# jinggqu/NextGen-UIA

Hardware: AMD Instinct MI355X
Metric: images/sec fwd+bwd BiomedCLIP+Mona bs=256 (higher is better)
Workload: dtype bf16

## Files before the change

include/uia_hip.h:

```cpp
#ifndef UIA_HIP_H
#define UIA_HIP_H
#include <stddef.h>
#include <stdint.h>

#ifdef __cplusplus
extern "C" {
#endif

enum { UIA_F32 = 0, UIA_BF16 = 1 };
enum { UIA_ACT_NONE = 0, UIA_ACT_GELU = 1, UIA_ACT_QUICKGELU = 2, UIA_ACT_RELU = 3 };
enum { UIA_MASK_NONE = 0, UIA_MASK_CAUSAL = 1, UIA_MASK_KEYPAD = 2 };
enum { UIA_MONA_BASELINE = 0, UIA_MONA_NOISE_AWARE = 1, UIA_MONA_FREQ_ENHANCED = 2, UIA_MONA_HYBRID = 3 };

const char* uia_last_error(void);
int uia_version(void);

typedef struct uia_gemm_desc {
    const void* A; int64_t lda;
    const void* W; int64_t ldw;
    int32_t M, N, K;
    float alpha;
    const float* bias;
    int32_t act;
    int32_t dact;
    const void* aux_in; int64_t ldaux_in;
    void* aux_out; int64_t ldaux_out;
    const float* resid; int64_t ldr;
    int32_t resid_mod, resid_row_off;
    const void* residT; int64_t ldrT;
    int32_t out_group;
    void* outT; int64_t ldo;
    float* out32; int64_t ldo32;
    int32_t w_kblocked;
    const void* resid_ln_stats;
    const float* resid_ln_w;
    const float* resid_ln_b;
    int64_t* rowsum_out;
    const int64_t* lnfold_sums;
    const float* lnfold_colsum;
    int32_t lnfold_dim; float lnfold_eps;
    int32_t resid_ln_dim; float resid_ln_eps;
    int64_t a_kb_rows;
    int64_t outT_kb_rows;
    int32_t* ln_flag;
    float ln_flag_limit;
    int32_t drop_where;
    float drop_p;
    uint64_t drop_seed;
    void* a_drop_out;
    float* splitk_ws;
    const void* A2;
    int64_t lda2;
    int32_t K2;
    int32_t a2_group_cols;
    int64_t a2_group_stride;
    const int8_t* resid_lo8;
    int64_t ld_resid_lo;
    int64_t residT_kb_rows;
    int8_t* out_lo8;
    int64_t ld_out_lo;
    int64_t resid_lo_kb_rows;
    int64_t out_lo_kb_rows;
} uia_gemm_desc;
int uia_gemm(void* stream, int dtype, const uia_gemm_desc* d, int tile_cfg );

int uia_wgrad(void* stream, int dtype, int M, int I, int J, const void* A, int64_t lda, const void* B, int64_t ldb,
              float alpha, float* dW, float* dbias_A);
int uia_wgrad_ex(void* stream, int dtype, int M, int I, int J, const void* A, int64_t lda, const void* B, int64_t ldb,
                 float alpha, float* dW, int64_t ldw, int i_valid, int j_valid, float* dbias_A);
int uia_wgrad_drop(void* stream, int dtype, int M, int I, int J, const void* A, int64_t lda, const void* B, int64_t ldb,
                   float alpha, float* dW, int64_t ldw, int i_valid, int j_valid, float drop_p, uint64_t seed, int64_t drop_ld, int drop_col0);
typedef struct uia_wgrad_group_desc {
    int32_t n, M, I, J;
    const void* A[4];
    const void* B[4];
    float* dW[4];
    float* dbias_A[4];
    int64_t lda, ldb, ldw;
    int32_t i_valid, j_valid;
    float alpha, drop_p;
    uint64_t drop_seed[4];
    int64_t drop_ld;
    int32_t drop_col0, reserved;
} uia_wgrad_group_desc;
int uia_wgrad_group(void* stream, int dtype, const uia_wgrad_group_desc* d);

typedef struct uia_attn_desc {
    const void *q, *k, *v; int64_t ld_qkv;
    void* out; int64_t ldo;
    float* lse;
    const int32_t* keylen;
    int32_t B, H, L, dh;
    int32_t mask_kind;
    float scale;
    const void* dout; int64_t lddo;
    void *dq, *dk, *dv; int64_t ld_dqkv;
    const int32_t* cu_seqlens;
    int64_t out_kb_rows;
    int64_t dqkv_kb_rows;
} uia_attn_desc;
int uia_attn_fwd(void* stream, int dtype, const uia_attn_desc* d);
int uia_attn_bwd(void* stream, int dtype, const uia_attn_desc* d);
int uia_attn_bwd_cfg(void* stream, int dtype, const uia_attn_desc* d, int cfg);

int uia_attn_fwd_long(void* stream, int dtype, const uia_attn_desc* d);

int uia_attn_bwd_cls(void* stream, int dtype, const uia_attn_desc* d);

int uia_attn_fwd_cls(void* stream, int dtype, const uia_attn_desc* d);
int uia_attn_bwd_cls_rows(void* stream, int dtype, const uia_attn_desc* d);

int uia_layernorm_fwd(void* stream, int dtype, int M, int D, int64_t ldx, const float* x, const float* gamma, const float* beta,
                      float eps, void* yT, float* y32);
int uia_layernorm_fwd_stats(void* stream, int dtype, int M, int D, int64_t ldx, const float* x, const float* gamma, const float* beta,
                            float eps, void* yT, float* y32, float* stats);
#define UIA_POOL_SLICES 32
int uia_ln_mean_rows(void* stream, int B, int L, int row0, int n, int D, int64_t ldx, const float* x, const float* gamma, const float* beta,
                     float eps, float* ws, float* out, int64_t ldo);
int uia_layernorm_bwd(void* stream, int dtype, int M, int D, int64_t ldx, const void* dy, const float* x, const float* gamma,
                      float eps, const float* dres, float* dx32, void* dxT);
int uia_layernorm_bwd3(void* stream, int dtype, int M, int D, int64_t ldx, const void* dy, const float* x, const void* x_hi, const int8_t* x_lo, int64_t x_kb_rows,
                       const float* gamma, float eps, const float* dres, const void* dres_hi, const int8_t* dres_lo, int64_t dres_kb_rows, float* dx32, void* dxT,
                       int8_t* dx_lo);
int uia_layernorm_bwd_periodic(void* stream, int dtype, int M, int D, const void* dy, const float* x, const void* x_hi, const int8_t* x_lo, int64_t x_kb_rows,
                               const float* gamma, float eps, const float* dres_rows, int period, float* dx32, void* dxT, int8_t* dx_lo);

typedef struct uia_mona_spatial_desc {
    int32_t variant, B, h, w, bott;
    const void* t;
    void* d;
    const float *conv1_w, *conv1_b, *conv2_w, *conv2_b, *conv3_w, *conv3_b;
    const float *proj_w, *proj_b;
    const float* freq;
    const float *ne1_w, *ne1_b, *ne3_w, *ne3_b;
    float p_drop; uint64_t seed; const uint8_t* keep_mask;
    const void* dd;
    void* dt;
    float *g_conv1_w, *g_conv1_b, *g_conv2_w, *g_conv2_b, *g_conv3_w, *g_conv3_b, *g_proj_w, *g_proj_b, *g_freq,
          *g_ne1_w, *g_ne1_b, *g_ne3_w, *g_ne3_b;
    float* ws;
} uia_mona_spatial_desc;
size_t uia_mona_spatial_workspace_bytes(int B);
int uia_mona_pre_fwd(void* stream, int dtype, int M, int D, const float* x, const float* norm_w, const float* norm_b,
                     const float* gamma, const float* gammax, float eps, void* u);
int uia_mona_pre_fwd_t(void* stream, int dtype, int M, int D, const float* x, const float* norm_w, const float* norm_b, const float* gamma, const float* gammax,
                       float eps, void* u, const void* w1, int64_t ldw1, const float* b1, void* t, int64_t ldt);
int uia_mona_pre_bwd(void* stream, int dtype, int M, int D, const void* du, const float* x, const float* dy,
                     const float* norm_w, const float* norm_b, const float* gamma, const float* gammax, float eps,
                     float* dx32, void* dxT, float* g_gamma, float* g_gammax, float* g_norm_w, float* g_norm_b, float* ws,
                     int64_t dxT_kb_rows);
int uia_mona_pre_bwd_du(void* stream, int dtype, int M, int D, const void* dt, int64_t ldt, const void* w1t, int64_t ldw1, const float* x, const float* dy,
                        const float* norm_w, const float* norm_b, const float* gamma, const float* gammax, float eps,
                        float* dx32, void* dxT, float* g_gamma, float* g_gammax, float* g_norm_w, float* g_norm_b, float* ws, int64_t dxT_kb_rows);
int uia_mona_pre_bwd_du3(void* stream, int dtype, int M, int D, const void* dt, int64_t ldt, const void* w1t, int64_t ldw1, const float* x, const void* dy_hi, const int8_t* dy_lo,
                         const float* norm_w, const float* norm_b, const float* gamma, const float* gammax, float eps, void* dxT, int8_t* dx_lo, float* g_gamma,
                         float* g_gammax, float* g_norm_w, float* g_norm_b, float* ws, int64_t dxT_kb_rows);
size_t uia_mona_pre_bwd_workspace_bytes(int M, int D);
int uia_mona_spatial_fwd(void* stream, int dtype, const uia_mona_spatial_desc* d);
int uia_mona_spatial_bwd(void* stream, int dtype, const uia_mona_spatial_desc* d);
int uia_mona_cls_bwd(void* stream, int dtype, int B, int ntok, const void* dd, const void* t, int64_t ldt, void* dt, float p_drop, uint64_t seed,
                     const uint8_t* keep_mask);
int uia_mona_cls_fwd(void* stream, int dtype, int B, int ntok, const void* t, int64_t ldt, void* d, float p_drop, uint64_t seed, const uint8_t* keep_mask);

typedef struct uia_mona_fused_desc {
    uia_mona_spatial_desc sp;
    int32_t D; float eps;
    const float* x;
    const float *norm_w, *norm_b, *gamma, *gammax;
    const void* w1; const float* b1;
    const void* w2; const float* b2;
    float* y32;
    void* yT; int64_t yT_kb_rows;
    int64_t* rowsum_out;
    int32_t* ln_flag;
    void* u_out;
    void* t_out;
} uia_mona_fused_desc;
int uia_mona_fused_supported(int dtype, int D, int h, int w, int bott);
int uia_mona_fused_fwd(void* stream, int dtype, const uia_mona_fused_desc* d);

typedef struct uia_lora_rank_desc {
    int32_t M, N, nsrc;
    float alpha;
    const void* Q; int64_t ldq, q_stride;
    const void* W[3]; int64_t ldw;
    void* out; int64_t ldo;
    float drop_p;
    uint64_t seed[3];
} uia_lora_rank_desc;
int uia_lora_rank_update(void* stream, int dtype, const uia_lora_rank_desc* d);

typedef struct uia_ln_lora_desc {
    int32_t M, D, nsrc;
    float eps;
    const float* x; int64_t ldx;
    const float *gamma, *beta;
    void* h;
    const void* A[3]; int64_t lda;
    void* T; int64_t t_stride;
    float drop_p;
    uint64_t seed[3];
} uia_ln_lora_desc;
int uia_ln_lora_down(void* stream, int dtype, const uia_ln_lora_desc* d);

int uia_upsample_bilinear_fwd(void* stream, int B, int C, int h, int w, int H, int W, const float* src, int64_t ld, float* dst);
int uia_upsample_bilinear_bwd(void* stream, int B, int C, int h, int w, int H, int W, const float* ddst, float* dsrc, int64_t ld);
int uia_segment_mean_fwd(void* stream, int B, int n, int C, const float* x, int64_t ld, float* out);
int uia_segment_mean_bwd(void* stream, int B, int n, int C, const float* dout, float* dx, int64_t ld);
size_t uia_dicece_workspace_bytes(int B);
int uia_dicece_fwd_bwd(void* stream, int B, int C, int HW, const float* logits, const float* label, float smooth_nr, float smooth_dr,
                       float* ws, float* loss, float* dlogits);
size_t uia_focal_workspace_bytes(int N, int C);
int uia_focal_fwd_bwd(void* stream, int N, int C, const float* logits, const int64_t* labels, float gamma, float alpha, void* ws, size_t ws_bytes,
                      float* loss, float* dlogits);
size_t uia_binary_cls_stats_workspace_bytes(int N);
int uia_binary_cls_stats(void* stream, int N, const float* p1, const int64_t* labels, const int64_t* perm, void* ws, size_t ws_bytes, double* record);
size_t uia_surface_distances_workspace_bytes(int B, int H, int W);
int uia_surface_distances(void* stream, int B, int H, int W, const float* logits, const float* label, float percentile, void* ws, size_t ws_bytes,
                          double* hd, double* asd);
enum { UIA_SEG_LABEL_U8 = 0, UIA_SEG_LABEL_F32 = 1 };
int uia_seg_viz_form(int S, int label_dtype, const void* logits, const void* images, const void* labels, const void* mask_rgb, const void* overlay_rgb,
                     const void* pred);
int uia_seg_viz(void* stream, int B, int C, int Ci, int S, const float* logits, const float* images, const void* labels, int label_dtype,
                uint8_t* mask_rgb, uint8_t* overlay_rgb, uint8_t* pred);
size_t uia_retrieval_workspace_bytes(int N, int E);
int uia_retrieval_ranks(void* stream, int N, int E, const float* img, const float* txt, int normalize, void* ws, size_t ws_bytes,
                        int32_t* gt_i2t, int32_t* eq_i2t, int32_t* gt_t2i, int32_t* eq_t2i);
size_t uia_retrieval_stats_workspace_bytes(int N);
int uia_retrieval_stats(void* stream, int N, const int32_t* gt, int nk, const int32_t* k_values, void* ws, size_t ws_bytes, double* record);
size_t uia_retrieval_topk_workspace_bytes(int Q, int N, int E, int K);
int uia_retrieval_topk_splits(int Q, int N);
int uia_retrieval_topk(void* stream, int Q, int N, int E, int K, const float* queries, const float* gallery, int normalize, int splits, void* ws,
                       size_t ws_bytes, int32_t* idx, float* score);
int uia_zero_shot_score(void* stream, int N, int T, int E, int C, const int32_t* class_off, const float* img, const float* prompts, float* logits, int64_t ld,
                        int64_t row, float* probs, float* img_n);
size_t uia_binary_roc_curve_workspace_bytes(int N);
int uia_binary_roc_curve(void* stream, int N, const float* p1, const int64_t* labels, const int64_t* perm, void* ws, size_t ws_bytes, int32_t* count,
                         double* fpr, double* tpr, float* thr);

size_t uia_augment_workspace_bytes(int B, int S);
int uia_augment_batch(void* stream, int B, int S, const float* images, const uint8_t* masks, const int32_t* programs, void* ws, size_t ws_bytes,
                      float* out_images, uint8_t* out_masks);

int uia_augment_gather(void* stream, int N, int B, int S, int src_dtype, const void* images, const uint8_t* masks, const int32_t* programs, void* ws,
                       size_t ws_bytes, float* out_images, uint8_t* out_masks);

int uia_cast(void* stream, int dtype, size_t n, const float* src, void* dst, float scale);
int uia_transpose_cast(void* stream, int dtype, int rows, int cols, const float* src, void* dst);

typedef struct uia_pack_desc {
    const float* src;
    void* row;
    void* row_kb;
    void* tr;
    void* tr_kb;
    int32_t rows, cols;
    int32_t rows_pad, cols_pad;
    float scale;
    int32_t reserved_;
} uia_pack_desc;
int uia_pack_weights(void* stream, int dtype, int n, const uia_pack_desc* descs_device, int max_elems);
int uia_im2col(void* stream, int dtype, int B, int C, int H, int W, int P, const float* img, void* out);
int uia_im2col_padded(void* stream, int dtype, int B, int C, int H, int W, int P, const float* img, void* cols, int64_t ldo);
int uia_fill_cls(void* stream, int B, int N, int D, const float* cls, const float* pos0, float* x);
// ... 94 lines not shown
```

nextgen-uia_amd/csrc/capi.cpp:

```cpp
#include "uia_kernels.h"

void uia_set_error(const char* fmt, ...);
#define NEED(ptr, name) do { if (!(ptr)) { uia_set_error("%s: null descriptor", name); return -1; } } while (0)

extern "C" {

int uia_version(void) { return 100; }

int uia_gemm(void* stream, int dtype, const uia_gemm_desc* d, int tile_cfg) {
    NEED(d, "uia_gemm");
    return uia_gemm_launch((hipStream_t)stream, dtype, *d, tile_cfg);
}
int uia_lora_rank_update(void* stream, int dtype, const uia_lora_rank_desc* d) {
    NEED(d, "uia_lora_rank_update");
    return uia_lora_rank_update_launch((hipStream_t)stream, dtype, *d);
}
int uia_ln_lora_down(void* stream, int dtype, const uia_ln_lora_desc* d) {
    NEED(d, "uia_ln_lora_down");
    return uia_ln_lora_down_launch((hipStream_t)stream, dtype, *d);
}
int uia_wgrad(void* stream, int dtype, int M, int I, int J, const void* A, int64_t lda, const void* B, int64_t ldb, float alpha, float* dW, float* dbias_A) {
    return uia_wgrad_launch((hipStream_t)stream, dtype, M, I, J, A, lda, B, ldb, alpha, dW, dbias_A);
}
int uia_wgrad_ex(void* stream, int dtype, int M, int I, int J, const void* A, int64_t lda, const void* B, int64_t ldb, float alpha, float* dW, int64_t ldw,
                 int i_valid, int j_valid, float* dbias_A) {
    if (ldw <= 0) { uia_set_error("uia_wgrad_ex: ldw=%lld must be positive", (long long)ldw); return -1; }
    return uia_wgrad_launch((hipStream_t)stream, dtype, M, I, J, A, lda, B, ldb, alpha, dW, dbias_A, ldw, i_valid, j_valid);
}
int uia_wgrad_group(void* stream, int dtype, const uia_wgrad_group_desc* d) {
    if (!d) { uia_set_error("uia_wgrad_group: null descriptor"); return -1; }
    if (d->n < 1 || d->n > 4) { uia_set_error("uia_wgrad_group: n=%d outside 1..4", d->n); return -1; }
    if (d->ldw <= 0) { uia_set_error("uia_wgrad_group: ldw=%lld must be positive", (long long)d->ldw); return -1; }
    float* dW[4];
    float* db[4];
    for (int g = 0; g < 4; ++g) { dW[g] = d->dW[g]; db[g] = d->dbias_A[g]; }
    if (d->drop_p > 0.f) for (int g = 0; g < d->n; ++g) if (db[g]) { uia_set_error("uia_wgrad_group: dbias with dropout on B is not a form of the kernel"); return -1; }
    return uia_wgrad_group_launch((hipStream_t)stream, dtype, d->n, d->M, d->I, d->J, d->A, (long)d->lda, d->B, (long)d->ldb, d->alpha, dW, db, (long)d->ldw, d->i_valid, d->j_valid,
                                  d->drop_p, d->drop_seed, (long)d->drop_ld, d->drop_col0);
}
int uia_wgrad_drop(void* stream, int dtype, int M, int I, int J, const void* A, int64_t lda, const void* B, int64_t ldb, float alpha, float* dW, int64_t ldw,
                   int i_valid, int j_valid, float drop_p, uint64_t seed, int64_t drop_ld, int drop_col0) {
    if (ldw <= 0) { uia_set_error("uia_wgrad_drop: ldw=%lld must be positive", (long long)ldw); return -1; }
    if (!(drop_p > 0.f)) { uia_set_error("uia_wgrad_drop: drop_p=%f must be in (0, 1); uia_wgrad_ex is the form without dropout", (double)drop_p); return -1; }
    return uia_wgrad_launch((hipStream_t)stream, dtype, M, I, J, A, lda, B, ldb, alpha, dW, nullptr, ldw, i_valid, j_valid, drop_p, seed, drop_ld, drop_col0);
}
int uia_attn_fwd(void* stream, int dtype, const uia_attn_desc* d) {
    NEED(d, "uia_attn_fwd");
    return uia_attn_fwd_launch((hipStream_t)stream, dtype, *d);
}
int uia_attn_fwd_long(void* stream, int dtype, const uia_attn_desc* d) {
    NEED(d, "uia_attn_fwd_long");
    return uia_attn_fwd_long_launch((hipStream_t)stream, dtype, *d);
}
int uia_attn_bwd(void* stream, int dtype, const uia_attn_desc* d) {
    NEED(d, "uia_attn_bwd");
    return uia_attn_bwd_launch((hipStream_t)stream, dtype, *d, 0);
}
int uia_attn_bwd_cfg(void* stream, int dtype, const uia_attn_desc* d, int cfg) {
    NEED(d, "uia_attn_bwd_cfg");
    return uia_attn_bwd_launch((hipStream_t)stream, dtype, *d, cfg);
}
int uia_layernorm_fwd(void* stream, int dtype, int M, int D, int64_t ldx, const float* x, const float* gamma, const float* beta, float eps, void* yT, float* y32) {
    return uia_layernorm_fwd_launch((hipStream_t)stream, dtype, M, D, ldx, x, gamma, beta, eps, yT, y32, nullptr);
}
int uia_layernorm_fwd_stats(void* stream, int dtype, int M, int D, int64_t ldx, const float* x, const float* gamma, const float* beta, float eps, void* yT, float* y32,
                            float* stats) {
    return uia_layernorm_fwd_launch((hipStream_t)stream, dtype, M, D, ldx, x, gamma, beta, eps, yT, y32, stats);
}
int uia_layernorm_bwd(void* stream, int dtype, int M, int D, int64_t ldx, const void* dy, const float* x, const float* gamma, float eps, const float* dres, float* dx32, void* dxT) {
    return uia_layernorm_bwd_launch((hipStream_t)stream, dtype, M, D, ldx, dy, x, gamma, eps, dres, dx32, dxT);
}
int uia_layernorm_bwd3(void* stream, int dtype, int M, int D, int64_t ldx, const void* dy, const float* x, const void* x_hi, const int8_t* x_lo, int64_t x_kb_rows,
                       const float* gamma, float eps, const float* dres, const void* dres_hi, const int8_t* dres_lo, int64_t dres_kb_rows, float* dx32, void* dxT,
                       int8_t* dx_lo) {
    return uia_layernorm_bwd3_launch((hipStream_t)stream, dtype, M, D, ldx, dy, x, x_hi, x_lo, (long)x_kb_rows, gamma, eps, dres, dres_hi, dres_lo, (long)dres_kb_rows, dx32, dxT,
                                     dx_lo);
}
int uia_layernorm_bwd_periodic(void* stream, int dtype, int M, int D, const void* dy, const float* x, const void* x_hi, const int8_t* x_lo, int64_t x_kb_rows,
                               const float* gamma, float eps, const float* dres_rows, int period, float* dx32, void* dxT, int8_t* dx_lo) {
    return uia_layernorm_bwd_periodic_launch((hipStream_t)stream, dtype, M, D, dy, x, x_hi, x_lo, (long)x_kb_rows, gamma, eps, dres_rows, period, dx32, dxT, dx_lo);
}
int uia_attn_bwd_cls(void* stream, int dtype, const uia_attn_desc* d) {
    NEED(d, "uia_attn_bwd_cls");
    return uia_attn_bwd_cls_launch((hipStream_t)stream, dtype, *d);
}
int uia_attn_bwd_cls_rows(void* stream, int dtype, const uia_attn_desc* d) {
    NEED(d, "uia_attn_bwd_cls_rows");
    return uia_attn_bwd_cls_launch((hipStream_t)stream, dtype, *d, true);
}
int uia_attn_fwd_cls(void* stream, int dtype, const uia_attn_desc* d) {
    NEED(d, "uia_attn_fwd_cls");
    return uia_attn_fwd_cls_launch((hipStream_t)stream, dtype, *d);
}
int uia_mona_cls_fwd(void* stream, int dtype, int B, int ntok, const void* t, int64_t ldt, void* d, float p_drop, uint64_t seed, const uint8_t* keep_mask) {
    return uia_mona_cls_fwd_launch((hipStream_t)stream, dtype, B, ntok, t, (long)ldt, d, p_drop, seed, keep_mask);
}
int uia_rows3_to_f32(void* stream, int rows, int D, int64_t stride_rows, const void* hi, int64_t ldhi, int64_t hi_kb_rows, const int8_t* lo, int64_t ldlo, float* dst) {
    return uia_rows3_to_f32_launch((hipStream_t)stream, rows, D, (long)stride_rows, hi, (long)ldhi, (long)hi_kb_rows, lo, (long)ldlo, dst);
}
int uia_mona_cls_bwd(void* stream, int dtype, int B, int ntok, const void* dd, const void* t, int64_t ldt, void* dt, float p_drop, uint64_t seed, const uint8_t* keep_mask) {
    return uia_mona_cls_bwd_launch((hipStream_t)stream, dtype, B, ntok, dd, t, (long)ldt, dt, p_drop, seed, keep_mask);
}
int uia_copy_rows(void* stream, int rows, int64_t row_bytes, const void* src, int64_t src_stride_bytes, void* dst) {
    return uia_copy_rows_launch((hipStream_t)stream, rows, (long)row_bytes, src, (long)src_stride_bytes, dst);
}
int uia_cast(void* stream, int dtype, size_t n, const float* src, void* dst, float scale) { return uia_cast_launch((hipStream_t)stream, dtype, n, src, dst, scale); }
int uia_transpose_cast(void* stream, int dtype, int rows, int cols, const float* src, void* dst) { return uia_transpose_cast_launch((hipStream_t)stream, dtype, rows, cols, src, dst); }
int uia_pack_weights(void* stream, int dtype, int n, const uia_pack_desc* descs_device, int max_elems) { return uia_pack_weights_launch((hipStream_t)stream, dtype, n, descs_device, max_elems); }
int uia_im2col(void* stream, int dtype, int B, int C, int H, int W, int P, const float* img, void* out) { return uia_im2col_launch((hipStream_t)stream, dtype, B, C, H, W, P, img, out); }
int uia_fill_cls(void* stream, int B, int N, int D, const float* cls, const float* pos0, float* x) { return uia_fill_cls_launch((hipStream_t)stream, B, N, D, cls, pos0, x); }
int uia_embed(void* stream, int rows, int L, int D, int vocab, int max_pos, const int64_t* ids, const float* table, const float* pos, const float* type0, float* out) {
    return uia_embed_launch((hipStream_t)stream, rows, L, D, vocab, max_pos, ids, table, pos, type0, out);
}
int uia_gather_rows(void* stream, int n, int D, const float* src, const int64_t* idx, float* dst) { return uia_gather_rows_launch((hipStream_t)stream, n, D, src, idx, dst); }

int uia_mona_pre_fwd(void* stream, int dtype, int M, int D, const float* x, const float* norm_w, const float* norm_b, const float* gamma,
                     const float* gammax, float eps, void* u) {
    return uia_mona_pre_fwd_launch((hipStream_t)stream, dtype, M, D, x, norm_w, norm_b, gamma, gammax, eps, u);
}
int uia_mona_pre_bwd(void* stream, int dtype, int M, int D, const void* du, const float* x, const float* dy, const float* norm_w,
                     const float* norm_b, const float* gamma, const float* gammax, float eps, float* dx32, void* dxT, float* g_gamma,
                     float* g_gammax, float* g_norm_w, float* g_norm_b, float* ws, int64_t dxT_kb_rows) {
    return uia_mona_pre_bwd_launch((hipStream_t)stream, dtype, M, D, du, x, dy, norm_w, norm_b, gamma, gammax, eps, dx32, dxT, g_gamma, g_gammax,
                                   g_norm_w, g_norm_b, ws, (long)dxT_kb_rows);
}
int uia_mona_pre_fwd_t(void* stream, int dtype, int M, int D, const float* x, const float* norm_w, const float* norm_b, const float* gamma, const float* gammax,
                       float eps, void* u, const void* w1, int64_t ldw1, const float* b1, void* t, int64_t ldt) {
    return uia_mona_pre_fwd_t_launch((hipStream_t)stream, dtype, M, D, x, norm_w, norm_b, gamma, gammax, eps, u, w1, (long)ldw1, b1, t, (long)ldt);
}
int uia_mona_pre_bwd_du(void* stream, int dtype, int M, int D, const void* dt, int64_t ldt, const void* w1t, int64_t ldw1, const float* x, const float* dy,
                        const float* norm_w, const float* norm_b, const float* gamma, const float* gammax, float eps, float* dx32, void* dxT, float* g_gamma,
                        float* g_gammax, float* g_norm_w, float* g_norm_b, float* ws, int64_t dxT_kb_rows) {
    if (!dt || !w1t) { uia_set_error("uia_mona_pre_bwd_du: null dt / w1t"); return -1; }
    return uia_mona_pre_bwd_launch((hipStream_t)stream, dtype, M, D, nullptr, x, dy, norm_w, norm_b, gamma, gammax, eps, dx32, dxT, g_gamma, g_gammax,
                                   g_norm_w, g_norm_b, ws, (long)dxT_kb_rows, dt, (long)ldt, w1t, (long)ldw1);
}
int uia_mona_pre_bwd_du3(void* stream, int dtype, int M, int D, const void* dt, int64_t ldt, const void* w1t, int64_t ldw1, const float* x, const void* dy_hi, const int8_t* dy_lo,
                         const float* norm_w, const float* norm_b, const float* gamma, const float* gammax, float eps, void* dxT, int8_t* dx_lo, float* g_gamma,
                         float* g_gammax, float* g_norm_w, float* g_norm_b, float* ws, int64_t dxT_kb_rows) {
    if (!dt || !w1t || !dy_hi || !dy_lo || !dx_lo) { uia_set_error("uia_mona_pre_bwd_du3: null dt / w1t / dy_hi / dy_lo / dx_lo"); return -1; }
    return uia_mona_pre_bwd_launch((hipStream_t)stream, dtype, M, D, nullptr, x, nullptr, norm_w, norm_b, gamma, gammax, eps, nullptr, dxT, g_gamma, g_gammax,
                                   g_norm_w, g_norm_b, ws, (long)dxT_kb_rows, dt, (long)ldt, w1t, (long)ldw1, dy_hi, dy_lo, dx_lo);
}
size_t uia_mona_pre_bwd_workspace_bytes(int M, int D) { return uia_mona_pre_bwd_ws_floats(M, D) * sizeof(float); }
int uia_mona_spatial_fwd(void* stream, int dtype, const uia_mona_spatial_desc* d) {
    NEED(d, "uia_mona_spatial_fwd");
    return uia_mona_spatial_fwd_launch((hipStream_t)stream, dtype, *d);
}
int uia_mona_spatial_bwd(void* stream, int dtype, const uia_mona_spatial_desc* d) {
    NEED(d, "uia_mona_spatial_bwd");
    return uia_mona_spatial_bwd_launch((hipStream_t)stream, dtype, *d);
}
int uia_mona_fused_fwd(void* stream, int dtype, const uia_mona_fused_desc* d) {
    NEED(d, "uia_mona_fused_fwd");
    return uia_mona_fused_fwd_launch((hipStream_t)stream, dtype, *d);
}

size_t uia_infonce_workspace_bytes(int B, int E) { return uia_infonce_workspace_floats(B, E) * sizeof(float); }
int uia_infonce_fwd_bwd(void* stream, int B, int E, const float* img, const float* txt, float inv_temp, float grad_scale, float* loss,
                        float* dimg, float* dtxt, void* workspace, size_t workspace_bytes) {
    return uia_infonce_launch((hipStream_t)stream, B, E, img, txt, inv_temp, grad_scale, loss, dimg, dtxt, (float*)workspace, workspace_bytes / sizeof(float));
}
int uia_adamw_clip_step(void* stream, size_t n, float* p, const float* g, float* m, float* v, float lr, float beta1, float beta2, float eps,
                        float weight_decay, float max_norm, int step, float grad_scale, float* ws2) {
    return uia_adamw_clip_launch((hipStream_t)stream, n, p, g, m, v, lr, beta1, beta2, eps, weight_decay, max_norm, step, grad_scale, ws2);
}
int uia_grad_accum_guarded(void* stream, size_t n, float* acc, float* mb, const float* loss, float* stats, int32_t* ctl, uint8_t* ok_log, int64_t log_index) {
    return uia_grad_accum_guarded_launch((hipStream_t)stream, n, acc, mb, loss, stats, (int*)ctl, ok_log, (long)log_index);
}
int uia_adamw_clip_step_guarded(void* stream, size_t n, float* p, float* acc, float* m, float* v, float lr, float lr_min, int t_max, float beta1, float beta2,
                                float eps, float weight_decay, float max_norm, float grad_scale, float skip_scale, float* ws8, int32_t* ctl) {
    return uia_adamw_clip_guarded_launch((hipStream_t)stream, n, p, acc, m, v, lr, lr_min, t_max, beta1, beta2, eps, weight_decay, max_norm, grad_scale, skip_scale, ws8, (int*)ctl);
}

int uia_dropout(void* stream, int dtype, size_t n, const void* src, void* dst, float p, uint64_t seed, int accumulate) {
    return uia_dropout_launch((hipStream_t)stream, dtype, n, src, dst, p, seed, accumulate);
}
int uia_colsum(void* stream, int dtype, int M, int N, const void* A, int64_t lda, float* out) {
    return uia_colsum_launch((hipStream_t)stream, dtype, M, N, A, lda, out);
}

int uia_layernorm_bwd_affine(void* stream, int dtype, int M, int D, const void* dy, const float* x, const float* gamma, float eps, const float* dres,
                             float* dx32, float* g_gamma, float* g_beta) {
    return uia_layernorm_bwd_affine_launch((hipStream_t)stream, dtype, M, D, dy, x, gamma, eps, dres, dx32, g_gamma, g_beta);
}
int uia_film_fwd(void* stream, int B, int N, int C, const float* x, const float* mul, const float* add, float* y) { return uia_film_fwd_launch((hipStream_t)stream, B, N, C, x, mul, add, y); }
int uia_film_bwd(void* stream, int B, int N, int C, const float* dy, const float* x, const float* mul, float* dx, float* dmul, float* dadd) {
    return uia_film_bwd_launch((hipStream_t)stream, B, N, C, dy, x, mul, dx, dmul, dadd);
}
int uia_im2col3x3(void* stream, int dtype, int B, int h, int w, int C, int ntok, int tok_off, const float* x, void* cols) {
    return uia_im2col3x3_launch((hipStream_t)stream, dtype, B, h, w, C, ntok, tok_off, x, cols);
}
int uia_col2im3x3(void* stream, int dtype, int B, int h, int w, int C, int ntok, int tok_off, const void* dcols, float* dx) {
    return uia_col2im3x3_launch((hipStream_t)stream, dtype, B, h, w, C, ntok, tok_off, dcols, dx);
}
int uia_unshuffle(void* stream, int dtype, int B, int h, int w, int k1, int k2, const void* tmp, int64_t ld, float bias, float* out) {
    return uia_unshuffle_launch((hipStream_t)stream, dtype, B, h, w, k1, k2, tmp, ld, bias, out);
}
int uia_shuffle(void* stream, int dtype, int B, int h, int w, int k1, int k2, const float* dout, void* dtmp, int64_t ld) {
    return uia_shuffle_launch((hipStream_t)stream, dtype, B, h, w, k1, k2, dout, dtmp, ld);
}
int uia_act_bwd(void* stream, int dtype, size_t n, const void* dy, const void* y, int act, void* out) { return uia_act_bwd_launch((hipStream_t)stream, dtype, n, dy, y, act, out); }

size_t uia_mona_spatial_workspace_bytes(int B) { return uia_mona_spatial_ws_floats(B) * sizeof(float); }

int uia_upsample_bilinear_fwd(void* stream, int B, int C, int h, int w, int H, int W, const float* src, int64_t ld, float* dst) {
    return uia_upsample_bilinear_launch((hipStream_t)stream, false, B, C, h, w, H, W, src, dst, (long)ld);
}
int uia_upsample_bilinear_bwd(void* stream, int B, int C, int h, int w, int H, int W, const float* ddst, float* dsrc, int64_t ld) {
    return uia_upsample_bilinear_launch((hipStream_t)stream, true, B, C, h, w, H, W, ddst, dsrc, (long)ld);
}
int uia_segment_mean_fwd(void* stream, int B, int n, int C, const float* x, int64_t ld, float* out) {
    return uia_segment_mean_launch((hipStream_t)stream, false, B, n, C, x, out, (long)ld);
}
int uia_segment_mean_bwd(void* stream, int B, int n, int C, const float* dout, float* dx, int64_t ld) {
    return uia_segment_mean_launch((hipStream_t)stream, true, B, n, C, dout, dx, (long)ld);
}

size_t uia_dicece_workspace_bytes(int B) { return uia_dicece_ws_floats(B) * sizeof(float); }
int uia_dicece_fwd_bwd(void* stream, int B, int C, int HW, const float* logits, const float* label, float smooth_nr, float smooth_dr,
                       float* ws, float* loss, float* dlogits) {
    return uia_dicece_launch((hipStream_t)stream, B, C, HW, logits, label, smooth_nr, smooth_dr, ws, loss, dlogits);
}

size_t uia_focal_workspace_bytes(int N, int C) { return uia_focal_ws_bytes(N, C); }
int uia_focal_fwd_bwd(void* stream, int N, int C, const float* logits, const int64_t* labels, float gamma, float alpha, void* ws, size_t ws_bytes,
                      float* loss, float* dlogits) {
    return uia_focal_launch((hipStream_t)stream, N, C, logits, labels, gamma, alpha, ws, ws_bytes, loss, dlogits);
}
size_t uia_binary_cls_stats_workspace_bytes(int N) { return uia_binary_cls_stats_ws_bytes(N); }
int uia_binary_cls_stats(void* stream, int N, const float* p1, const int64_t* labels, const int64_t* perm, void* ws, size_t ws_bytes, double* record) {
    return uia_binary_cls_stats_launch((hipStream_t)stream, N, p1, labels, perm, ws, ws_bytes, record);
}

size_t uia_surface_distances_workspace_bytes(int B, int H, int W) { return uia_surface_ws_bytes(B, H, W); }
int uia_surface_distances(void* stream, int B, int H, int W, const float* logits, const float* label, float percentile, void* ws, size_t ws_bytes,
                          double* hd, double* asd) {
    return uia_surface_launch((hipStream_t)stream, B, H, W, logits, label, percentile, ws, ws_bytes, hd, asd);
}

int uia_seg_viz(void* stream, int B, int C, int Ci, int S, const float* logits, const float* images, const void* labels, int label_dtype,
                uint8_t* mask_rgb, uint8_t* overlay_rgb, uint8_t* pred) {
    return uia_seg_viz_launch((hipStream_t)stream, B, C, Ci, S, logits, images, labels, label_dtype, mask_rgb, overlay_rgb, pred);
}

size_t uia_retrieval_workspace_bytes(int N, int E) { return uia_retrieval_ranks_ws_bytes(N, E); }
// ... 138 lines not shown
```

nextgen-uia_amd/csrc/uia_kernels.h:

```cpp
#pragma once
#include <hip/hip_runtime.h>
#include <stddef.h>
#include <stdint.h>

#include "../../include/uia_hip.h"

typedef uia_gemm_desc UiaGemmParams;
typedef uia_attn_desc UiaAttnParams;

int uia_gemm_launch(hipStream_t stream, int dtype, const UiaGemmParams& p, int cfg);
int uia_attn_fwd_launch(hipStream_t stream, int dtype, const UiaAttnParams& p);
int uia_attn_fwd_long_launch(hipStream_t stream, int dtype, const UiaAttnParams& p);
int uia_attn_bwd_launch(hipStream_t stream, int dtype, const UiaAttnParams& p, int cfg = 0);
int uia_layernorm_fwd_launch(hipStream_t stream, int dtype, int M, int D, long ldx, const float* x, const float* gamma, const float* beta,
                             float eps, void* yT, float* y32, float* stats);
int uia_layernorm_bwd_launch(hipStream_t stream, int dtype, int M, int D, long ldx, const void* dy, const float* x, const float* gamma, float eps,
                             const float* dres, float* dx32, void* dxT);
int uia_layernorm_bwd3_launch(hipStream_t stream, int dtype, int M, int D, long ldx, const void* dy, const float* x, const void* x_hi, const int8_t* x_lo,
                              long x_kb_rows, const float* gamma, float eps, const float* dres, const void* dres_hi, const int8_t* dres_lo, long dres_kb_rows,
                              float* dx32, void* dxT, int8_t* dx_lo);
int uia_layernorm_bwd_periodic_launch(hipStream_t stream, int dtype, int M, int D, const void* dy, const float* x, const void* x_hi, const int8_t* x_lo, long x_kb_rows,
                                      const float* gamma, float eps, const float* dres_rows, int period, float* dx32, void* dxT, int8_t* dx_lo);
int uia_attn_bwd_cls_launch(hipStream_t stream, int dtype, const UiaAttnParams& p, bool compact = false);
int uia_attn_fwd_cls_launch(hipStream_t stream, int dtype, const UiaAttnParams& p);
int uia_mona_cls_fwd_launch(hipStream_t stream, int dtype, int B, int ntok, const void* t, long ldt, void* d, float p_drop, uint64_t seed, const uint8_t* keep_mask);
int uia_rows3_to_f32_launch(hipStream_t stream, int rows, int D, long stride_rows, const void* hi, long ldhi, long hi_kb_rows, const int8_t* lo, long ldlo, float* dst);
int uia_mona_cls_bwd_launch(hipStream_t stream, int dtype, int B, int ntok, const void* dd, const void* t, long ldt, void* dt, float p_drop, uint64_t seed,
                            const uint8_t* keep_mask);
int uia_copy_rows_launch(hipStream_t stream, int rows, long row_bytes, const void* src, long src_stride_bytes, void* dst);
int uia_lora_rank_update_launch(hipStream_t stream, int dtype, const uia_lora_rank_desc& p);
int uia_ln_lora_down_launch(hipStream_t stream, int dtype, const uia_ln_lora_desc& p);
int uia_cast_launch(hipStream_t stream, int dtype, size_t n, const float* src, void* dst, float scale);
int uia_transpose_cast_launch(hipStream_t stream, int dtype, int rows, int cols, const float* src, void* dst);
int uia_pack_weights_launch(hipStream_t stream, int dtype, int n, const uia_pack_desc* descs_device, int max_elems);
int uia_im2col_launch(hipStream_t stream, int dtype, int B, int C, int H, int W, int P, const float* img, void* out);
int uia_fill_cls_launch(hipStream_t stream, int B, int N, int D, const float* cls, const float* pos0, float* x);
int uia_embed_launch(hipStream_t stream, int rows, int L, int D, int vocab, int max_pos, const int64_t* ids, const float* table, const float* pos, const float* type0, float* out);
int uia_gather_rows_launch(hipStream_t stream, int n, int D, const float* src, const int64_t* idx, float* dst);
int uia_wgrad_group_launch(hipStream_t stream, int dtype, int n, int M, int I, int J, const void* const* A, long lda, const void* const* B, long ldb, float alpha,
                            float* const* dW, float* const* dbias, long ldw, int i_valid, int j_valid, float drop_p, const uint64_t* drop_seed, long drop_ld, int drop_col0);
int uia_wgrad_launch(hipStream_t stream, int dtype, int M, int I, int J, const void* A, long lda, const void* B, long ldb, float alpha, float* dW, float* dbias,
                     long ldw = 0, int i_valid = 0, int j_valid = 0, float drop_p = 0.f, uint64_t drop_seed = 0, long drop_ld = 0, int drop_col0 = 0);
int uia_mona_pre_fwd_launch(hipStream_t stream, int dtype, int M, int D, const float* x, const float* nw, const float* nb, const float* gamma,
                            const float* gammax, float eps, void* u);
int uia_mona_pre_fwd_t_launch(hipStream_t stream, int dtype, int M, int D, const float* x, const float* nw, const float* nb, const float* gamma,
                              const float* gammax, float eps, void* u, const void* w1, long ldw1, const float* b1, void* t, long ldt);
int uia_mona_pre_bwd_launch(hipStream_t stream, int dtype, int M, int D, const void* du, const float* x, const float* dy, const float* nw,
                            const float* nb, const float* gamma, const float* gammax, float eps, float* dx32, void* dxT, float* g_gamma,
                            float* g_gammax, float* g_nw, float* g_nb, float* ws, long dxT_kb_rows, const void* dt = nullptr, long ldt = 0,
                            const void* w1t = nullptr, long ldw1 = 0, const void* dy_hi = nullptr, const int8_t* dy_lo = nullptr, int8_t* dx_lo = nullptr);
size_t uia_mona_pre_bwd_ws_floats(int M, int D);
int uia_mona_spatial_fwd_launch(hipStream_t stream, int dtype, const uia_mona_spatial_desc& p);
int uia_mona_spatial_bwd_launch(hipStream_t stream, int dtype, const uia_mona_spatial_desc& p);
int uia_mona_fused_fwd_launch(hipStream_t stream, int dtype, const uia_mona_fused_desc& q);
size_t uia_infonce_workspace_floats(int B, int E);
int uia_infonce_launch(hipStream_t stream, int B, int E, const float* img, const float* txt, float inv_temp, float grad_scale, float* loss,
                       float* dimg, float* dtxt, float* ws, size_t ws_floats);
int uia_adamw_clip_launch(hipStream_t stream, size_t n, float* p, const float* g, float* m, float* v, float lr, float beta1, float beta2,
                          float eps, float weight_decay, float max_norm, int step, float grad_scale, float* ws);
int uia_grad_accum_guarded_launch(hipStream_t stream, size_t n, float* acc, float* mb, const float* loss, float* stats, int* ctl, unsigned char* ok_log, long log_index);
int uia_adamw_clip_guarded_launch(hipStream_t stream, size_t n, float* p, float* acc, float* m, float* v, float lr, float lr_min, int t_max, float beta1,
                                  float beta2, float eps, float weight_decay, float max_norm, float grad_scale, float skip_scale, float* ws8, int* ctl);
int uia_dropout_launch(hipStream_t stream, int dtype, size_t n, const void* src, void* dst, float p, uint64_t seed, int accumulate);
int uia_colsum_launch(hipStream_t stream, int dtype, int M, int N, const void* A, long lda, float* out);
int uia_attn_small_launch(hipStream_t stream, int dtype, const UiaAttnParams& p, bool bwd);
bool uia_attn_dh16_ok(int dtype, const UiaAttnParams& p);
int uia_attn_dh16_launch(hipStream_t stream, const UiaAttnParams& p, bool bwd);
int uia_layernorm_bwd_affine_launch(hipStream_t stream, int dtype, int M, int D, const void* dy, const float* x, const float* gamma, float eps,
                                    const float* dres, float* dx32, float* g_gamma, float* g_beta);
int uia_film_fwd_launch(hipStream_t stream, int B, int N, int C, const float* x, const float* mul, const float* add, float* y);
int uia_film_bwd_launch(hipStream_t stream, int B, int N, int C, const float* dy, const float* x, const float* mul, float* dx, float* dmul, float* dadd);
int uia_im2col3x3_launch(hipStream_t stream, int dtype, int B, int h, int w, int C, int ntok, int tok_off, const float* x, void* cols);
int uia_col2im3x3_launch(hipStream_t stream, int dtype, int B, int h, int w, int C, int ntok, int tok_off, const void* dcols, float* dx);
int uia_unshuffle_launch(hipStream_t stream, int dtype, int B, int h, int w, int k1, int k2, const void* tmp, long ld, float bias, float* out);
int uia_shuffle_launch(hipStream_t stream, int dtype, int B, int h, int w, int k1, int k2, const float* dout, void* dtmp, long ld);
int uia_act_bwd_launch(hipStream_t stream, int dtype, size_t n, const void* dy, const void* y, int act, void* out);
size_t uia_mona_spatial_ws_floats(int B);
int uia_upsample_bilinear_launch(hipStream_t stream, bool bwd, int B, int C, int h, int w, int H, int W, const float* in, float* out, long ld);
int uia_segment_mean_launch(hipStream_t stream, bool bwd, int B, int n, int C, const float* in, float* out, long ld);
size_t uia_dicece_ws_floats(int B);
int uia_dicece_launch(hipStream_t stream, int B, int C, int HW, const float* logits, const float* label, float nr, float dr, float* ws, float* loss, float* dlogits);
size_t uia_focal_ws_bytes(int N, int C);
int uia_focal_launch(hipStream_t stream, int N, int C, const float* logits, const int64_t* labels, float gamma, float alpha, void* ws, size_t ws_bytes,
                     float* loss, float* dlogits);
size_t uia_binary_cls_stats_ws_bytes(int N);
int uia_binary_cls_stats_launch(hipStream_t stream, int N, const float* p1, const int64_t* labels, const int64_t* perm, void* ws, size_t ws_bytes,
                                double* record);
size_t uia_surface_ws_bytes(int B, int H, int W);
int uia_surface_launch(hipStream_t stream, int B, int H, int W, const float* logits, const float* label, float percentile, void* ws, size_t ws_bytes,
                       double* hd, double* asd);
int uia_seg_viz_launch(hipStream_t stream, int B, int C, int Ci, int S, const float* logits, const float* images, const void* labels, int label_dtype,
                       uint8_t* mask_rgb, uint8_t* overlay_rgb, uint8_t* pred);
size_t uia_retrieval_ranks_ws_bytes(int N, int E);
int uia_retrieval_ranks_launch(hipStream_t stream, int N, int E, const float* img, const float* txt, int normalize, void* ws, size_t ws_bytes,
                               int32_t* gt_i2t, int32_t* eq_i2t, int32_t* gt_t2i, int32_t* eq_t2i);
size_t uia_retrieval_stats_ws_bytes(int N);
int uia_retrieval_stats_launch(hipStream_t stream, int N, const int32_t* gt, int nk, const int32_t* k_values, void* ws, size_t ws_bytes, double* record);
size_t uia_retrieval_topk_ws_bytes(int Q, int N, int E, int K);
int uia_retrieval_topk_rule(int Q, int N);
int uia_retrieval_topk_launch(hipStream_t stream, int Q, int N, int E, int K, const float* queries, const float* gallery, int normalize, int splits, void* ws,
                              size_t ws_bytes, int32_t* idx, float* score);
int uia_zero_shot_score_launch(hipStream_t stream, int N, int T, int E, int C, const int32_t* class_off, const float* img, const float* prompts, float* logits,
                               long ld, long row, float* probs, float* img_n);
size_t uia_binary_roc_curve_ws_bytes(int N);
int uia_binary_roc_curve_launch(hipStream_t stream, int N, const float* p1, const int64_t* labels, const int64_t* perm, void* ws, size_t ws_bytes,
                                int32_t* count, double* fpr, double* tpr, float* thr);
size_t uia_augment_ws_bytes(int B, int S);
int uia_augment_batch_launch(hipStream_t stream, int B, int S, const float* images, const uint8_t* masks, const int32_t* programs, void* ws, size_t ws_bytes,
                             float* out_images, uint8_t* out_masks);
int uia_augment_gather_launch(hipStream_t stream, int N, int B, int S, int src_dtype, const void* images, const uint8_t* masks, const int32_t* programs,
                              void* ws, size_t ws_bytes, float* out_images, uint8_t* out_masks);
int uia_im2col_padded_launch(hipStream_t stream, int dtype, int B, int C, int H, int W, int P, const float* img, void* out, long ldo);
int uia_embed_bwd_launch(hipStream_t stream, int rows, int D, int vocab, const int64_t* ids, const float* dx, float* dtable, long pad_id);
int uia_embed_packed_launch(hipStream_t stream, int rows, int D, int vocab, int max_pos, const int64_t* ids, const int64_t* pos_idx, const float* table, const float* pos, const float* type0, float* out);
int uia_ln_mean_rows_launch(hipStream_t stream, int B, int L, int row0, int n, int D, long ldx, const float* x, const float* gamma, const float* beta,
                            float eps, float* ws, float* out, long ldo);
int uia_conv_igemm_launch(hipStream_t stream, int dtype, int mode, int B, int H, int W, int C1, int C2, const void* x1, const void* x2, int N, int N1,
                          const void* w, const float* bias, void* y1, void* y2);
int uia_conv_wgrad_splits(int mode, int B, int H, int W, int C1, int C2, int N);
int uia_conv_wgrad_launch(hipStream_t stream, int dtype, int mode, int B, int H, int W, int C1, int C2, const void* x1, const void* x2, int N,
                          const void* dy, float* ws, float* dw);
int uia_bn_fwd_launch(hipStream_t stream, int dtype, int training, long M, int C, const void* y, const float* gamma, const float* beta,
                      float* run_mean, float* run_var, int64_t* nbt, float momentum, float eps, float* ws, float* mean, float* invstd,
                      float* scale, float* shift, int relu, void* out);
int uia_bn_relu_bwd_launch(hipStream_t stream, int dtype, long M, int C, const void* y, const void* dout, const float* scale, const float* shift,
                           const float* mean, const float* invstd, const float* gamma, float* ws, float* dgamma, float* dbeta, void* dy);
int uia_colsum_ordered_launch(hipStream_t stream, int dtype, long M, int C, const void* y, float* ws, float* out);
int uia_conv_igemm_form(int mode, int C1, int C2, int N, int N1);
int uia_conv_wgrad_form(int mode, int C1, int C2, int N);
int uia_bn_act_fwd_launch(hipStream_t stream, int dtype, int training, long M, int C, const void* y, const float* gamma, const float* beta,
                          float* run_mean, float* run_var, int64_t* nbt, float momentum, float eps, float* ws, float* mean, float* invstd,
                          float* scale, float* shift, float slope, void* out, float drop_p, uint64_t seed, const uint8_t* keep_mask);
int uia_bn_act_bwd_launch(hipStream_t stream, int dtype, long M, int C, const void* y, const void* dout, const float* scale, const float* shift,
                          const float* mean, const float* invstd, const float* gamma, float* ws, float* dgamma, float* dbeta, void* dy,
                          float slope, float drop_p, uint64_t seed, const uint8_t* keep_mask);
int uia_maxpool2_launch(hipStream_t stream, int dtype, int backward, int B, int H, int W, int C, const void* x, const void* dy, void* out);
int uia_conv_strided_launch(hipStream_t stream, int dtype, int dgrad, int B, int H, int W, int C, int k, int s, const void* x, int N, const void* w,
                            void* y);
int uia_conv_strided_wgrad_splits(int B, int H, int W, int C, int k, int s, int N);
int uia_conv_strided_form(int dgrad, int C, int N, int k, int s);
int uia_conv_strided_wgrad_form(int C, int N, int k, int s);
int uia_conv_strided_wgrad_launch(hipStream_t stream, int dtype, int B, int H, int W, int C, int k, int s, const void* x, int N, const void* dy,
                                  float* ws, float* dw);
int uia_maxpool3s2_launch(hipStream_t stream, int dtype, int backward, int B, int H, int W, int C, const void* x, const void* dy, void* out);
int uia_avgpool_launch(hipStream_t stream, int dtype, int backward, int B, int H, int W, int C, const void* x, float* pooled, void* dx);
int uia_nchw_to_nhwc_launch(hipStream_t stream, int dtype, int B, int Cin, int H, int W, int Cout, int rep, const float* x, void* out);
int uia_add2_launch(hipStream_t stream, int dtype, long n, const void* a, const void* b, void* out);
int uia_bn_add_relu_fwd_launch(hipStream_t stream, int dtype, int training, long M, int C, const void* y, const void* r, const float* gamma,
                               const float* beta, float* run_mean, float* run_var, int64_t* nbt, float momentum, float eps, float* ws, float* mean,
                               float* invstd, float* scale, float* shift, void* out);
int uia_bn_add_relu_bwd_launch(hipStream_t stream, int dtype, long M, int C, const void* y, const void* out, const void* dout, const float* mean,
                               const float* invstd, const float* gamma, float* ws, float* dgamma, float* dbeta, void* dy, void* dr);
int uia_upsample_ac_launch(hipStream_t stream, int dtype, int backward, int B, int H, int W, int C, int f, const void* in, void* out);
int uia_resize_aa_launch(hipStream_t stream, int dtype, int backward, int B, int C, int Hi, int Wi, int Ho, int Wo, const void* x, float* tmp, float* out,
                         const float* dout, void* dx);
```

nextgen-uia_amd/uia_hip/_lib.py:

```python
import ctypes as C
import os
import re

import torch

_HERE = os.path.dirname(os.path.abspath(__file__))
LIB_PATH = os.environ.get("UIA_HIP_LIB") or os.path.join(_HERE, "libuia_hip.so")

F32, BF16 = 0, 1
ACT_NONE, ACT_GELU, ACT_QUICKGELU, ACT_RELU = 0, 1, 2, 3
MASK_NONE, MASK_CAUSAL, MASK_KEYPAD = 0, 1, 2
MONA_VARIANTS = {"baseline": 0, "noise_aware": 1, "freq_enhanced": 2, "hybrid": 3}

vp, i32, i64, f32, sz = C.c_void_p, C.c_int32, C.c_int64, C.c_float, C.c_size_t


class PackDesc(C.Structure):
    _fields_ = [("src", vp), ("row", vp), ("row_kb", vp), ("tr", vp), ("tr_kb", vp), ("rows", i32), ("cols", i32),
                ("rows_pad", i32), ("cols_pad", i32), ("scale", f32), ("reserved_", i32)]


class GemmDesc(C.Structure):
    _fields_ = [("A", vp), ("lda", i64), ("W", vp), ("ldw", i64), ("M", i32), ("N", i32), ("K", i32), ("alpha", f32),
                ("bias", vp), ("act", i32), ("dact", i32), ("aux_in", vp), ("ldaux_in", i64), ("aux_out", vp), ("ldaux_out", i64),
                ("resid", vp), ("ldr", i64), ("resid_mod", i32), ("resid_row_off", i32), ("residT", vp), ("ldrT", i64),
                ("out_group", i32), ("outT", vp), ("ldo", i64), ("out32", vp), ("ldo32", i64), ("w_kblocked", i32),
                ("resid_ln_stats", vp), ("resid_ln_w", vp), ("resid_ln_b", vp),
                ("rowsum_out", vp), ("lnfold_sums", vp), ("lnfold_colsum", vp), ("lnfold_dim", i32), ("lnfold_eps", f32),
                ("resid_ln_dim", i32), ("resid_ln_eps", f32), ("a_kb_rows", i64), ("outT_kb_rows", i64), ("ln_flag", vp), ("ln_flag_limit", f32),
                ("drop_where", i32), ("drop_p", f32), ("drop_seed", C.c_uint64), ("a_drop_out", vp), ("splitk_ws", vp),
                ("A2", vp), ("lda2", i64), ("K2", i32), ("a2_group_cols", i32), ("a2_group_stride", i64),
                ("resid_lo8", vp), ("ld_resid_lo", i64), ("residT_kb_rows", i64), ("out_lo8", vp), ("ld_out_lo", i64),
                ("resid_lo_kb_rows", i64), ("out_lo_kb_rows", i64)]


class AttnDesc(C.Structure):
    _fields_ = [("q", vp), ("k", vp), ("v", vp), ("ld_qkv", i64), ("out", vp), ("ldo", i64), ("lse", vp), ("keylen", vp),
                ("B", i32), ("H", i32), ("L", i32), ("dh", i32), ("mask_kind", i32), ("scale", f32),
                ("dout", vp), ("lddo", i64), ("dq", vp), ("dk", vp), ("dv", vp), ("ld_dqkv", i64), ("cu_seqlens", vp),
                ("out_kb_rows", i64), ("dqkv_kb_rows", i64)]


class MonaSpatialDesc(C.Structure):
    _fields_ = [("variant", i32), ("B", i32), ("h", i32), ("w", i32), ("bott", i32),
                ("t", vp), ("d", vp),
                ("conv1_w", vp), ("conv1_b", vp), ("conv2_w", vp), ("conv2_b", vp), ("conv3_w", vp), ("conv3_b", vp),
                ("proj_w", vp), ("proj_b", vp), ("freq", vp), ("ne1_w", vp), ("ne1_b", vp), ("ne3_w", vp), ("ne3_b", vp),
                ("p_drop", f32), ("seed", C.c_uint64), ("keep_mask", vp),
                ("dd", vp), ("dt", vp),
                ("g_conv1_w", vp), ("g_conv1_b", vp), ("g_conv2_w", vp), ("g_conv2_b", vp), ("g_conv3_w", vp), ("g_conv3_b", vp),
                ("g_proj_w", vp), ("g_proj_b", vp), ("g_freq", vp), ("g_ne1_w", vp), ("g_ne1_b", vp), ("g_ne3_w", vp), ("g_ne3_b", vp), ("ws", vp)]


class WgradGroupDesc(C.Structure):
    _fields_ = [("n", C.c_int32), ("M", C.c_int32), ("I", C.c_int32), ("J", C.c_int32), ("A", C.c_void_p * 4), ("B", C.c_void_p * 4), ("dW", C.c_void_p * 4),
                ("dbias_A", C.c_void_p * 4), ("lda", C.c_int64), ("ldb", C.c_int64), ("ldw", C.c_int64), ("i_valid", C.c_int32), ("j_valid", C.c_int32),
                ("alpha", C.c_float), ("drop_p", C.c_float), ("drop_seed", C.c_uint64 * 4), ("drop_ld", C.c_int64), ("drop_col0", C.c_int32), ("reserved", C.c_int32)]


class LoraRankDesc(C.Structure):
    _fields_ = [("M", i32), ("N", i32), ("nsrc", i32), ("alpha", f32), ("Q", vp), ("ldq", i64), ("q_stride", i64), ("W", vp * 3), ("ldw", i64),
                ("out", vp), ("ldo", i64), ("drop_p", f32), ("seed", C.c_uint64 * 3)]


class LnLoraDesc(C.Structure):
    _fields_ = [("M", i32), ("D", i32), ("nsrc", i32), ("eps", f32), ("x", vp), ("ldx", i64), ("gamma", vp), ("beta", vp), ("h", vp), ("A", vp * 3), ("lda", i64),
                ("T", vp), ("t_stride", i64), ("drop_p", f32), ("seed", C.c_uint64 * 3)]


class MonaFusedDesc(C.Structure):
    _fields_ = [("sp", MonaSpatialDesc), ("D", i32), ("eps", f32), ("x", vp), ("norm_w", vp), ("norm_b", vp), ("gamma", vp), ("gammax", vp),
                ("w1", vp), ("b1", vp), ("w2", vp), ("b2", vp), ("y32", vp), ("yT", vp), ("yT_kb_rows", i64), ("rowsum_out", vp), ("ln_flag", vp),
                ("u_out", vp), ("t_out", vp)]


PROTOTYPES = {
    "uia_last_error": (C.c_char_p, []),
    "uia_version": (C.c_int, []),
    "uia_gemm": (C.c_int, [vp, C.c_int, C.POINTER(GemmDesc), C.c_int]),
    "uia_wgrad": (C.c_int, [vp, C.c_int, C.c_int, C.c_int, C.c_int, vp, i64, vp, i64, f32, vp, vp]),
    "uia_wgrad_drop": (C.c_int, [vp, C.c_int, C.c_int, C.c_int, C.c_int, vp, i64, vp, i64, f32, vp, i64, C.c_int, C.c_int, f32, C.c_uint64, i64, C.c_int]),
    "uia_wgrad_group": (C.c_int, [vp, C.c_int, vp]),
    "uia_wgrad_ex": (C.c_int, [vp, C.c_int, C.c_int, C.c_int, C.c_int, vp, i64, vp, i64, f32, vp, i64, C.c_int, C.c_int, vp]),
    "uia_attn_fwd": (C.c_int, [vp, C.c_int, C.POINTER(AttnDesc)]),
    "uia_attn_fwd_long": (C.c_int, [vp, C.c_int, C.POINTER(AttnDesc)]),
    "uia_attn_bwd": (C.c_int, [vp, C.c_int, C.POINTER(AttnDesc)]),
    "uia_attn_bwd_cfg": (C.c_int, [vp, C.c_int, C.POINTER(AttnDesc), C.c_int]),
    "uia_layernorm_fwd": (C.c_int, [vp, C.c_int, C.c_int, C.c_int, i64, vp, vp, vp, f32, vp, vp]),
    "uia_layernorm_fwd_stats": (C.c_int, [vp, C.c_int, C.c_int, C.c_int, i64, vp, vp, vp, f32, vp, vp, vp]),
    "uia_ln_mean_rows": (C.c_int, [vp, C.c_int, C.c_int, C.c_int, C.c_int, C.c_int, i64, vp, vp, vp, f32, vp, vp, i64]),
    "uia_conv_igemm": (C.c_int, [vp, C.c_int, C.c_int, C.c_int, C.c_int, C.c_int, C.c_int, C.c_int, vp, vp, C.c_int, C.c_int, vp, vp, vp, vp]),
    "uia_conv_wgrad_splits": (C.c_int, [C.c_int, C.c_int, C.c_int, C.c_int, C.c_int, C.c_int, C.c_int]),
    "uia_conv_wgrad": (C.c_int, [vp, C.c_int, C.c_int, C.c_int, C.c_int, C.c_int, C.c_int, C.c_int, vp, vp, C.c_int, vp, vp, vp]),
    "uia_conv_igemm_form": (C.c_int, [C.c_int, C.c_int, C.c_int, C.c_int, C.c_int]),
    "uia_conv_wgrad_form": (C.c_int, [C.c_int, C.c_int, C.c_int, C.c_int]),
    "uia_bn_act_fwd": (C.c_int, [vp, C.c_int, C.c_int, i64, C.c_int, vp, vp, vp, vp, vp, vp, f32, f32, vp, vp, vp, vp, vp, f32, vp, f32, C.c_uint64, vp]),
    "uia_bn_act_bwd": (C.c_int, [vp, C.c_int, i64, C.c_int, vp, vp, vp, vp, vp, vp, vp, vp, vp, vp, vp, f32, f32, C.c_uint64, vp]),
    "uia_maxpool2_fwd": (C.c_int, [vp, C.c_int, C.c_int, C.c_int, C.c_int, C.c_int, vp, vp]),
    "uia_maxpool2_bwd": (C.c_int, [vp, C.c_int, C.c_int, C.c_int, C.c_int, C.c_int, vp, vp, vp]),
    "uia_conv_strided": (C.c_int, [vp, C.c_int, C.c_int, C.c_int, C.c_int, C.c_int, C.c_int, C.c_int, C.c_int, vp, C.c_int, vp, vp]),
    "uia_conv_strided_wgrad_splits": (C.c_int, [C.c_int, C.c_int, C.c_int, C.c_int, C.c_int, C.c_int, C.c_int]),
    "uia_conv_strided_form": (C.c_int, [C.c_int, C.c_int, C.c_int, C.c_int, C.c_int]),
    "uia_conv_strided_wgrad_form": (C.c_int, [C.c_int, C.c_int, C.c_int, C.c_int]),
    "uia_conv_strided_wgrad": (C.c_int, [vp, C.c_int, C.c_int, C.c_int, C.c_int, C.c_int, C.c_int, C.c_int, vp, C.c_int, vp, vp, vp]),
    "uia_maxpool3s2_fwd": (C.c_int, [vp, C.c_int, C.c_int, C.c_int, C.c_int, C.c_int, vp, vp]),
    "uia_maxpool3s2_bwd": (C.c_int, [vp, C.c_int, C.c_int, C.c_int, C.c_int, C.c_int, vp, vp, vp]),
    "uia_bn_add_relu_fwd": (C.c_int, [vp, C.c_int, C.c_int, i64, C.c_int, vp, vp, vp, vp, vp, vp, vp, f32, f32, vp, vp, vp, vp, vp, vp]),
    "uia_bn_add_relu_bwd": (C.c_int, [vp, C.c_int, i64, C.c_int, vp, vp, vp, vp, vp, vp, vp, vp, vp, vp, vp]),
    "uia_avgpool_fwd": (C.c_int, [vp, C.c_int, C.c_int, C.c_int, C.c_int, C.c_int, vp, vp]),
    "uia_avgpool_bwd": (C.c_int, [vp, C.c_int, C.c_int, C.c_int, C.c_int, C.c_int, vp, vp]),
    "uia_nchw_to_nhwc": (C.c_int, [vp, C.c_int, C.c_int, C.c_int, C.c_int, C.c_int, C.c_int, C.c_int, vp, vp]),
    "uia_add2": (C.c_int, [vp, C.c_int, i64, vp, vp, vp]),
    "uia_bn_fwd": (C.c_int, [vp, C.c_int, C.c_int, i64, C.c_int, vp, vp, vp, vp, vp, vp, f32, f32, vp, vp, vp, vp, vp, C.c_int, vp]),
    "uia_bn_relu_bwd": (C.c_int, [vp, C.c_int, i64, C.c_int, vp, vp, vp, vp, vp, vp, vp, vp, vp, vp, vp]),
    "uia_colsum_ordered": (C.c_int, [vp, C.c_int, i64, C.c_int, vp, vp, vp]),
    "uia_upsample_ac": (C.c_int, [vp, C.c_int, C.c_int, C.c_int, C.c_int, C.c_int, C.c_int, C.c_int, vp, vp]),
    "uia_resize_aa": (C.c_int, [vp, C.c_int, C.c_int, C.c_int, C.c_int, C.c_int, C.c_int, C.c_int, C.c_int, vp, vp, vp, vp, vp]),
    "uia_layernorm_bwd": (C.c_int, [vp, C.c_int, C.c_int, C.c_int, i64, vp, vp, vp, f32, vp, vp, vp]),
    "uia_ln_lora_down": (C.c_int, [vp, C.c_int, C.POINTER(LnLoraDesc)]),
    "uia_lora_rank_update": (C.c_int, [vp, C.c_int, C.POINTER(LoraRankDesc)]),
    "uia_layernorm_bwd3": (C.c_int, [vp, C.c_int, C.c_int, C.c_int, i64, vp, vp, vp, vp, i64, vp, f32, vp, vp, vp, i64, vp, vp, vp]),
    "uia_mona_pre_fwd": (C.c_int, [vp, C.c_int, C.c_int, C.c_int, vp, vp, vp, vp, vp, f32, vp]),
    "uia_mona_pre_bwd": (C.c_int, [vp, C.c_int, C.c_int, C.c_int, vp, vp, vp, vp, vp, vp, vp, f32, vp, vp, vp, vp, vp, vp, vp, i64]),
    "uia_mona_pre_fwd_t": (C.c_int, [vp, C.c_int, C.c_int, C.c_int, vp, vp, vp, vp, vp, f32, vp, vp, i64, vp, vp, i64]),
    "uia_mona_pre_bwd_du": (C.c_int, [vp, C.c_int, C.c_int, C.c_int, vp, i64, vp, i64, vp, vp, vp, vp, vp, vp, f32, vp, vp, vp, vp, vp, vp, vp, i64]),
    "uia_mona_pre_bwd_du3": (C.c_int, [vp, C.c_int, C.c_int, C.c_int, vp, i64, vp, i64, vp, vp, vp, vp, vp, vp, vp, f32, vp, vp, vp, vp, vp, vp, vp, i64]),
    "uia_mona_pre_bwd_workspace_bytes": (sz, [C.c_int, C.c_int]),
    "uia_mona_spatial_fwd": (C.c_int, [vp, C.c_int, C.POINTER(MonaSpatialDesc)]),
    "uia_mona_spatial_bwd": (C.c_int, [vp, C.c_int, C.POINTER(MonaSpatialDesc)]),
    "uia_mona_spatial_workspace_bytes": (sz, [C.c_int]),
    "uia_mona_fused_supported": (C.c_int, [C.c_int, C.c_int, C.c_int, C.c_int, C.c_int]),
    "uia_mona_fused_fwd": (C.c_int, [vp, C.c_int, C.POINTER(MonaFusedDesc)]),
    "uia_upsample_bilinear_fwd": (C.c_int, [vp, C.c_int, C.c_int, C.c_int, C.c_int, C.c_int, C.c_int, vp, C.c_int64, vp]),
    "uia_upsample_bilinear_bwd": (C.c_int, [vp, C.c_int, C.c_int, C.c_int, C.c_int, C.c_int, C.c_int, vp, vp, C.c_int64]),
    "uia_segment_mean_fwd": (C.c_int, [vp, C.c_int, C.c_int, C.c_int, vp, C.c_int64, vp]),
    "uia_segment_mean_bwd": (C.c_int, [vp, C.c_int, C.c_int, C.c_int, vp, vp, C.c_int64]),
    "uia_dicece_workspace_bytes": (sz, [C.c_int]),
    "uia_dicece_fwd_bwd": (C.c_int, [vp, C.c_int, C.c_int, C.c_int, vp, vp, C.c_float, C.c_float, vp, vp, vp]),
    "uia_focal_workspace_bytes": (sz, [C.c_int, C.c_int]),
    "uia_focal_fwd_bwd": (C.c_int, [vp, C.c_int, C.c_int, vp, vp, f32, f32, vp, sz, vp, vp]),
    "uia_binary_cls_stats_workspace_bytes": (sz, [C.c_int]),
    "uia_binary_cls_stats": (C.c_int, [vp, C.c_int, vp, vp, vp, vp, sz, vp]),
    "uia_surface_distances_workspace_bytes": (sz, [C.c_int, C.c_int, C.c_int]),
    "uia_surface_distances": (C.c_int, [vp, C.c_int, C.c_int, C.c_int, vp, vp, f32, vp, sz, vp, vp]),
    "uia_seg_viz_form": (C.c_int, [C.c_int, C.c_int, vp, vp, vp, vp, vp, vp]),
    "uia_seg_viz": (C.c_int, [vp, C.c_int, C.c_int, C.c_int, C.c_int, vp, vp, vp, C.c_int, vp, vp, vp]),
    "uia_retrieval_workspace_bytes": (sz, [C.c_int, C.c_int]),
    "uia_retrieval_ranks": (C.c_int, [vp, C.c_int, C.c_int, vp, vp, C.c_int, vp, sz, vp, vp, vp, vp]),
    "uia_retrieval_stats_workspace_bytes": (sz, [C.c_int]),
    "uia_retrieval_stats": (C.c_int, [vp, C.c_int, vp, C.c_int, vp, vp, sz, vp]),
    "uia_retrieval_topk_workspace_bytes": (sz, [C.c_int, C.c_int, C.c_int, C.c_int]),
    "uia_retrieval_topk_splits": (C.c_int, [C.c_int, C.c_int]),
    "uia_retrieval_topk": (C.c_int, [vp, C.c_int, C.c_int, C.c_int, C.c_int, vp, vp, C.c_int, C.c_int, vp, sz, vp, vp]),
    "uia_zero_shot_score": (C.c_int, [vp, C.c_int, C.c_int, C.c_int, C.c_int, vp, vp, vp, vp, C.c_int64, C.c_int64, vp, vp]),
    "uia_binary_roc_curve_workspace_bytes": (sz, [C.c_int]),
    "uia_binary_roc_curve": (C.c_int, [vp, C.c_int, vp, vp, vp, vp, sz, vp, vp, vp, vp]),
    "uia_augment_workspace_bytes": (sz, [C.c_int, C.c_int]),
    "uia_augment_batch": (C.c_int, [vp, C.c_int, C.c_int, vp, vp, vp, vp, sz, vp, vp]),
    "uia_augment_gather": (C.c_int, [vp, C.c_int, C.c_int, C.c_int, C.c_int, vp, vp, vp, vp, sz, vp, vp]),
    "uia_infonce_workspace_bytes": (sz, [C.c_int, C.c_int]),
    "uia_infonce_fwd_bwd": (C.c_int, [vp, C.c_int, C.c_int, vp, vp, f32, f32, vp, vp, vp, vp, sz]),
    "uia_adamw_clip_step": (C.c_int, [vp, sz, vp, vp, vp, vp, f32, f32, f32, f32, f32, f32, C.c_int, f32, vp]),
    "uia_grad_accum_guarded": (C.c_int, [vp, sz, vp, vp, vp, vp, vp, vp, i64]),
    "uia_adamw_clip_step_guarded": (C.c_int, [vp, sz, vp, vp, vp, vp, f32, f32, C.c_int, f32, f32, f32, f32, f32, f32, f32, vp, vp]),
    "uia_comm_unique_id_bytes": (C.c_int, []),
    "uia_comm_get_unique_id": (C.c_int, [vp, C.c_int]),
    "uia_comm_init": (C.c_int, [C.c_int, C.c_int, vp, C.c_int]),
    "uia_comm_world": (C.c_int, []),
    "uia_comm_initialised": (C.c_int, []),
    "uia_allreduce_sum": (C.c_int, [vp, C.c_int, vp, sz]),
    "uia_allgather": (C.c_int, [vp, C.c_int, vp, vp, sz]),
    "uia_comm_destroy": (C.c_int, []),
    "uia_dropout": (C.c_int, [vp, C.c_int, sz, vp, vp, f32, C.c_uint64, C.c_int]),
    "uia_colsum": (C.c_int, [vp, C.c_int, C.c_int, C.c_int, vp, i64, vp]),
    "uia_layernorm_bwd_affine": (C.c_int, [vp, C.c_int, C.c_int, C.c_int, vp, vp, vp, f32, vp, vp, vp, vp]),
    "uia_film_fwd": (C.c_int, [vp, C.c_int, C.c_int, C.c_int, vp, vp, vp, vp]),
    "uia_film_bwd": (C.c_int, [vp, C.c_int, C.c_int, C.c_int, vp, vp, vp, vp, vp, vp]),
    "uia_im2col3x3": (C.c_int, [vp, C.c_int, C.c_int, C.c_int, C.c_int, C.c_int, C.c_int, C.c_int, vp, vp]),
    "uia_col2im3x3": (C.c_int, [vp, C.c_int, C.c_int, C.c_int, C.c_int, C.c_int, C.c_int, C.c_int, vp, vp]),
    "uia_unshuffle": (C.c_int, [vp, C.c_int, C.c_int, C.c_int, C.c_int, C.c_int, C.c_int, vp, i64, f32, vp]),
    "uia_shuffle": (C.c_int, [vp, C.c_int, C.c_int, C.c_int, C.c_int, C.c_int, C.c_int, vp, vp, i64]),
    "uia_act_bwd": (C.c_int, [vp, C.c_int, sz, vp, vp, C.c_int, vp]),
    "uia_cast": (C.c_int, [vp, C.c_int, sz, vp, vp, f32]),
    "uia_transpose_cast": (C.c_int, [vp, C.c_int, C.c_int, C.c_int, vp, vp]),
    "uia_pack_weights": (C.c_int, [vp, C.c_int, C.c_int, vp, C.c_int]),
    "uia_im2col": (C.c_int, [vp, C.c_int, C.c_int, C.c_int, C.c_int, C.c_int, C.c_int, vp, vp]),
    "uia_im2col_padded": (C.c_int, [vp, C.c_int, C.c_int, C.c_int, C.c_int, C.c_int, C.c_int, vp, vp, C.c_int64]),
    "uia_fill_cls": (C.c_int, [vp, C.c_int, C.c_int, C.c_int, vp, vp, vp]),
    "uia_embed": (C.c_int, [vp, C.c_int, C.c_int, C.c_int, C.c_int, C.c_int, vp, vp, vp, vp, vp]),
    "uia_embed_bwd": (C.c_int, [vp, C.c_int, C.c_int, C.c_int, vp, vp, vp, C.c_int64]),
    "uia_embed_packed": (C.c_int, [vp, C.c_int, C.c_int, C.c_int, C.c_int, vp, vp, vp, vp, vp, vp]),
    "uia_gather_rows": (C.c_int, [vp, C.c_int, C.c_int, vp, vp, vp]),
    "uia_copy_rows": (C.c_int, [vp, C.c_int, i64, vp, i64, vp]),
    "uia_attn_bwd_cls": (C.c_int, [vp, C.c_int, C.POINTER(AttnDesc)]),
    "uia_mona_cls_bwd": (C.c_int, [vp, C.c_int, C.c_int, C.c_int, vp, vp, i64, vp, f32, C.c_uint64, vp]),
    "uia_attn_fwd_cls": (C.c_int, [vp, C.c_int, C.POINTER(AttnDesc)]),
    "uia_attn_bwd_cls_rows": (C.c_int, [vp, C.c_int, C.POINTER(AttnDesc)]),
    "uia_mona_cls_fwd": (C.c_int, [vp, C.c_int, C.c_int, C.c_int, vp, i64, vp, f32, C.c_uint64, vp]),
    "uia_rows3_to_f32": (C.c_int, [vp, C.c_int, C.c_int, i64, vp, i64, i64, vp, i64, vp]),
    "uia_layernorm_bwd_periodic": (C.c_int, [vp, C.c_int, C.c_int, C.c_int, vp, vp, vp, vp, i64, vp, f32, vp, C.c_int, vp, vp, vp]),
}

_lib = None
_BLOCKING = ("uia_comm_init", "uia_comm_destroy", "uia_comm_get_unique_id")


class UiaError(RuntimeError):
    pass


def lib():
    global _lib
    if _lib is None:
        if not os.path.exists(LIB_PATH):
            raise UiaError(f"{LIB_PATH} not built: run `make -C nextgen-uia_amd/csrc` (hipcc --offload-arch=gfx950). "
                           "There is no CPU fallback for the uia hot path.")
        release = os.environ.get("UIA_CTYPES_RELEASE_GIL", "0") == "1"
        handle = (C.CDLL if release else C.PyDLL)(LIB_PATH)
        blocking = C.CDLL(LIB_PATH)
        _one_copy_of("librccl")
        _one_copy_of("libamdhip64")
        for name, (res, args) in PROTOTYPES.items():
            fn = getattr(blocking if name in _BLOCKING else handle, name)
            fn.restype, fn.argtypes = res, args
            if name in _BLOCKING:
                setattr(handle, name, fn)
        _lib = handle
    return _lib


def _one_copy_of(stem):
    try:
        pat = re.compile(r"^" + re.escape(stem) + r"\.so(\.\d+)*$")
        paths = {line.split()[-1] for line in open("/proc/self/maps") if pat.match(os.path.basename(line.split()[-1]) if line.split() else "")}
    except OSError:
        return
    real = {os.path.realpath(p) for p in paths}
    if len(real) > 1:
        raise UiaError(f"two copies of {stem} are loaded ({sorted(real)}): import torch before uia_hip so that libuia_hip.so binds to PyTorch's runtime")


def check(rc, what=""):
    if rc != 0:
        raise UiaError(f"{what} failed (rc={rc}): {lib().uia_last_error().decode()}")
```

nextgen-uia_amd/uia_hip/functional.py:

```python
import math
import os
import weakref

import time

import torch

from . import handoff, ops
from ._lib import UiaError
from .handoff import (ClsGrad, Resid3, _g3_partner_feeds, cls_grad_of, fwd3_of, grad3_decode, grad3_of, grad_resid3_enabled, hook_free, linear_chain,
                      publish_cls_grad, publish_fwd3, publish_grad3, publish_rows, publish_t_copy, set_cls_grad, set_grad_resid3, t_copy_of, take_rows, zero_sums,
                      cls_only, set_cls_forward, take_cls_forward)
from .handoff import clear as clear_t_copies

_STATE = {"dtype": torch.bfloat16, "seed": 0x5EED, "calls": 0, "fwd_resid3": os.environ.get("UIA_FWD_RESID3", "1") != "0"}


def set_compute_dtype(dt):
    assert dt in (torch.bfloat16, torch.float32)
    _STATE["dtype"] = dt


def compute_dtype():
    return _STATE["dtype"]


def set_deferred_text_ln(flag):
    _STATE["text_ln_deferred"] = bool(flag)


def set_block_resid3(flag):
    _STATE["block_resid3"] = bool(flag)


def set_fwd_resid3(flag):
    _STATE["fwd_resid3"] = bool(flag)


def set_text_resid3(flag):
    _STATE["text_resid3"] = bool(flag)


def set_ln_fold(flag):
    _STATE["ln_fold"] = bool(flag)


def set_deterministic(flag):
    _STATE["deterministic"] = bool(flag)
    ops.TAIL_SPLIT_K = not flag


def ln_fold_enabled(dt, rows=None):
    return dt != torch.float32 and _STATE.get("ln_fold", True) and (rows is None or rows > _STATE.get("ln_fold_min_rows", 2048))


class LnFoldRangeError(FloatingPointError):
    """A GEMM that left row sums for a folded LayerNorm saw a non-finite or out-of-range partial sum: the LayerNorm statistics of that
    row — and everything downstream of it — are wrong."""


_FOLD_POLL = {}
_FOLD_REPORTED = {}


POLL_LAG = max(1, int(os.environ.get("UIA_POLL_LAG", "2")))


def reset_ln_flag(device=None):
    dev = torch.device("cuda", torch.cuda.current_device()) if device is None else torch.device(device)
    key = dev.index if dev.index is not None else torch.cuda.current_device()
    _FOLD_POLL.pop(key, None)
    _FOLD_REPORTED.pop(key, None)
    if key in ops._LN_FLAG:
        ops._LN_FLAG[key].zero_()


def poll_ln_flag(device=None, sync=False):
    dev = torch.device("cuda", torch.cuda.current_device()) if device is None else torch.device(device)
    key = dev.index if dev.index is not None else torch.cuda.current_device()
    flag = ops._LN_FLAG.get(key)
    if flag is None:
        return 0
    seen = 0
    pending = _FOLD_POLL.setdefault(key, [])
    while pending and (sync or len(pending) >= POLL_LAG):
        prev = pending.pop(0)
        t0 = time.perf_counter()
        prev[1].synchronize()
        _STATE["gpu_wait_s"] = _STATE.get("gpu_wait_s", 0.0) + time.perf_counter() - t0
        seen |= int(prev[0][0])
    host = torch.empty(1, dtype=torch.int32, pin_memory=True)
    host.copy_(flag, non_blocking=True)
    ev = torch.cuda.Event()
    ev.record()
    if sync:
        ev.synchronize()
        seen |= int(host[0])
    else:
        pending.append((host, ev))
    seen &= ~_FOLD_REPORTED.get(key, 0) | 2
    _FOLD_REPORTED[key] = _FOLD_REPORTED.get(key, 0) | (seen & 1)
    if seen & 2:
        raise LnFoldRangeError("uia_hip: a LayerNorm row sum was non-finite or out of the fixed-point range (|Σ| or Σ² >= 5e8 in one column "
                               "block): the activations have diverged; the statistics of that row are not valid")
    if seen & 1 and _STATE.get("ln_fold", True):
        import warnings
        warnings.warn(f"uia_hip: LayerNorm fold switched off: a row with |mean| / std > {ops.LN_FLAG_LIMIT} would lose bf16 precision as a raw "
                      "GEMM operand; the LayerNorm kernels are used from the next forward on")
        set_ln_fold(False)
    return seen


def set_fp32_heads(flag):
    _STATE["fp32_heads"] = bool(flag)


def head_dtype():
    return torch.float32 if _STATE.get("fp32_heads", True) else compute_dtype()


def set_unpad_text(flag):
    _STATE["unpad_text"] = bool(flag)


def set_dropout_seed(seed):
    _STATE["seed"], _STATE["calls"] = int(seed), 0


def _next_seed():
    _STATE["calls"] += 1
    return (_STATE["seed"] * 0x9E3779B97F4A7C15 + _STATE["calls"] * 0xD1B54A32D192ED03) & 0xFFFFFFFFFFFFFFFF


class _PackedParam:
    __slots__ = ("ref", "version", "epoch", "dt", "row", "row_kb", "tr", "tr_kb", "fwd", "bwd", "src_ptr", "pads", "extra")

    def __init__(self, p, dt, pads=None):
        R, Cc = p.shape
        RP, CP = pads if pads is not None else (R, Cc)
        g = 64 // torch.empty(0, dtype=dt).element_size()
        mk = (lambda *shape: torch.zeros(shape, device=p.device, dtype=dt)) if pads is not None else (lambda *shape: torch.empty(shape, device=p.device, dtype=dt))
        self.ref, self.version, self.epoch, self.dt, self.src_ptr, self.pads = weakref.ref(p), -1, -1, dt, 0, pads
        self.extra = []
        self.row, self.tr = mk(RP, CP), mk(CP, RP)
        self.row_kb = mk(CP // g, RP, g) if CP % g == 0 else None
        self.tr_kb = mk(RP // g, CP, g) if RP % g == 0 else None
        self.fwd, self.bwd = ops.PackedW(self.row, self.row_kb), ops.PackedW(self.tr, self.tr_kb)

    def entries(self):
        src = self.ref().detach()
        ent = (src, self.row, self.row_kb, self.tr, self.tr_kb)
        out = [ent if self.pads is None else ent + ((self.pads[0], self.pads[1], 1.0),)]
        for view, rp, cp, scale in self.extra:
            out.append((src, None, ops.RawDest(view), None, None, (rp, cp, scale)))
        return out


class WeightCache:
    PACK_MAX_ELEMS = 1 << 20

    def __init__(self):
        self._c = {}
        self.epoch = 0
        self._packed = {}
        self._ext_of = {}
# ... 272 lines not shown
        P = dict(zip(names, params))
        B, N, D = x.shape
        dt, bott = u.dtype, t.shape[1]
        dy = cg.rows32
        dy_t = dy if dt == torch.float32 else (cg.rows_t if cg.rows_t is not None else t_copy_of(dy, dt))
        direct = ctx.direct_params is not None and all(_is_flat_grad(p) for p in ctx.direct_params)
        G = ({k: p.grad for k, p in zip(names, ctx.direct_params)} if direct
             else {k: torch.zeros_like(v, dtype=torch.float32) for k, v in P.items()})
        cls_rows = lambda a: a.view(B, N * a.shape[1])[:, :a.shape[1]]
        side = _wgrad_side_stream(x.device) if _STATE.get("wgrad_side_stream", False) else None
        w2t = WEIGHTS.get(P["project2.weight"], dt, transpose=True)
        dd = _empty((B, bott), dt, x)
        _wgrad_beside(side, lambda: ops.gemm(dy_t, w2t, out_t=dd), dy_t, cls_rows(d), G["project2.weight"], G["project2.bias"])
        dtt = _empty((B, bott), dt, x)
        ops.mona_cls_bwd(B, ntok or N, dd, t, dtt, p_drop=p_drop, seed=seed, keep_mask=keep_mask, t_rows=bool(ntok))
        w1t = WEIGHTS.get(P["project1.weight"], dt, transpose=True)
        fuse_du = x.is_cuda and ops.mona_pre_bwd_du_ok(B, D, bott, dt)
        du = None if fuse_du else _empty((B, D), dt, x)
        _wgrad_beside(side, None if fuse_du else (lambda: ops.gemm(dtt, w1t, out_t=du)), dtt, cls_rows(u), G["project1.weight"], G["project1.bias"])
        need_dx = ctx.needs_input_grad[0]
        x_cls = x.view(B, D) if ntok else ops.copy_rows(x.view(B * N, D), N, _empty((B, D), torch.float32, x))
        dx = _empty((B, D), torch.float32, x) if need_dx else None
        dx_t = _empty((B, D), dt, x) if (need_dx and dt != torch.float32) else None
        w1t_rows = (dtt, w1t.row if isinstance(w1t, ops.PackedW) else w1t) if fuse_du else None
        ops.mona_pre_bwd(du, x_cls, dy if need_dx else None, P["norm.weight"], P["norm.bias"], P["gamma"], P["gammax"], dx, dx_t,
                         G["gamma"], G["gammax"], G["norm.weight"], G["norm.bias"], dt_w1t=w1t_rows)
        if need_dx and ntok:
            dx = dx.view(B, 1, D)
            publish_t_copy(dx, dx_t.view(B, 1, D) if dx_t is not None else None)
        elif need_dx:
            dx = publish_cls_grad(x.shape, x.device, dx, dx_t) if ctx.cls_ok else ClsGrad(dx, dx_t, N).decode()
        grads = tuple(None if direct else (G[k] if ctx.needs_input_grad[7 + i] else None) for i, k in enumerate(names))
        return (dx, None, None, None, None, None, None) + grads

    @staticmethod
    def backward(ctx, dy):
        if getattr(ctx, "rows_ntok", 0):
            dy = dy.contiguous()
            B, _, D = dy.shape
            dt = ctx.saved_tensors[1].dtype
            return MonaFn.backward_cls(ctx, ClsGrad(dy.view(B, D), t_copy_of(dy, dt).view(B, D) if dt != torch.float32 else None, ctx.rows_ntok))
        cg = cls_grad_of(dy)
        if cg is not None:
            return MonaFn.backward_cls(ctx, cg)
        variant, hw, p_drop, seed, names, has_mask = ctx.meta
        x, u, t, d, keep_mask, *params = ctx.saved_tensors
        keep_mask = keep_mask if has_mask else None
        P = dict(zip(names, params))
        B, N, D = x.shape
        h, w = hw
        M, dt = B * N, u.dtype
        bott = t.shape[1]
        g3 = grad3_of(dy)
        fuse_du = x.is_cuda and ops.mona_pre_bwd_du_ok(M, D, bott, dt)
        if g3 is not None and ops.is_kb(g3.hi):
            dy, g3 = g3.decode().view(B, N, D), None
        if g3 is not None:
            dy_t = g3.hi.view(M, D)
        else:
            dy = dy.contiguous()
            dy_t = t_copy_of(dy, dt).view(M, D)
        direct = ctx.direct_params is not None and all(_is_flat_grad(p) for p in ctx.direct_params)
        G = ({k: p.grad for k, p in zip(names, ctx.direct_params)} if direct
             else {k: torch.zeros_like(v, dtype=torch.float32) for k, v in P.items()})
        w2t = WEIGHTS.get(P["project2.weight"], dt, transpose=True)
        dd = _empty((M, bott), dt, x)
        side = _wgrad_side_stream(x.device) if _STATE.get("wgrad_side_stream", False) else None
        _wgrad_beside(side, lambda: ops.gemm(dy_t, w2t, out_t=dd), dy_t, d, G["project2.weight"], G["project2.bias"])
        sp = {_SPATIAL_MAP[k]: v.detach().contiguous() for k, v in P.items() if k in _SPATIAL_MAP}
        sg = {_SPATIAL_MAP[k]: G[k] for k in P if k in _SPATIAL_MAP}
        dtt = _empty((M, bott), dt, x)
        ops.mona_spatial_bwd(variant, B, h, w, t, sp, dd, dtt, sg, p_drop=p_drop, seed=seed, keep_mask=keep_mask)
        w1t = WEIGHTS.get(P["project1.weight"], dt, transpose=True)
        du = None if fuse_du else _empty((M, D), dt, x)
        _wgrad_beside(side, None if fuse_du else (lambda: ops.gemm(dtt, w1t, out_t=du)), dtt, u, G["project1.weight"], G["project1.bias"])
        need_dx = ctx.needs_input_grad[0]
        dx_t = _act(M, D, dt, x, 4 * D) if (need_dx and dt != torch.float32) else None
        w1t_rows = (dtt, w1t.row if isinstance(w1t, ops.PackedW) else w1t) if fuse_du else None
        if need_dx and g3 is not None and fuse_du and getattr(ctx, "g3_out", False):
            dlo = torch.empty(M, D, device=x.device, dtype=torch.int8)
            ops.mona_pre_bwd(None, x, g3, P["norm.weight"], P["norm.bias"], P["gamma"], P["gammax"], None, dx_t,
                             G["gamma"], G["gammax"], G["norm.weight"], G["norm.bias"], dt_w1t=w1t_rows, dx_lo=dlo)
            dx = publish_grad3(x.shape, x.device, dx_t, dlo)
        else:
            if need_dx and g3 is not None:
                dy = g3.decode().view(B, N, D)
            dx = torch.empty_like(x) if need_dx else None
            ops.mona_pre_bwd(du, x, dy if need_dx else None, P["norm.weight"], P["norm.bias"], P["gamma"], P["gammax"], dx, dx_t,
                             G["gamma"], G["gammax"], G["norm.weight"], G["norm.bias"], dt_w1t=w1t_rows)
            if need_dx:
                publish_t_copy(dx, dx_t)
        grads = tuple(None if direct else (G[k] if ctx.needs_input_grad[7 + i] else None) for i, k in enumerate(names))
        return (dx, None, None, None, None, None, None) + grads


def _wgrad_beside(side, dgrad, a, b, dw, db):
    if side is not None:
        side.wait_stream(torch.cuda.current_stream())
        with torch.cuda.stream(side):
            ops.wgrad(a, b, dw, db)
        a.record_stream(side)
        b.record_stream(side)
    if dgrad is not None:
        dgrad()
    if side is None:
        ops.wgrad(a, b, dw, db)


_WGRAD_SIDE = {}


def _wgrad_side_stream(device):
    key = device.index if device.index is not None else torch.cuda.current_device()
    if key not in _WGRAD_SIDE:
        _WGRAD_SIDE[key] = torch.cuda.Stream(device=device)
    return _WGRAD_SIDE[key]


def set_wgrad_side_stream(flag):
    _STATE["wgrad_side_stream"] = bool(flag)


def join_side_streams():
    cur = torch.cuda.current_stream()
    for st in _WGRAD_SIDE.values():
        cur.wait_stream(st)


DIRECT_TRAIN = True


def _is_flat_grad(p):
    g = p.grad
    return (getattr(p, "_uia_flat_grad", False) and g is not None and g.dtype == torch.float32 and g.is_contiguous() and g.shape == p.shape
            and g.device == p.device)


def mona_apply(x_bnd, module_params, variant, hw, p_drop, training, keep_mask=None):
    names = tuple(k for k in MONA_PARAM_ORDER if k in module_params)
    pd = p_drop if (training or keep_mask is not None) else 0.0
    params = [module_params[k] for k in names]
    direct = torch.is_grad_enabled() and all(p.requires_grad and _is_flat_grad(p) for p in params)
    return MonaFn.apply(x_bnd, variant, tuple(hw), pd, keep_mask, names, direct, *params)


class BlockSpec:

    def __init__(self, heads, eps, act, ln1, qkv, proj, ln2, fc1, fc2, mask=None, publish_out=False):
        self.heads, self.eps, self.act, self.mask = heads, eps, act, mask
        self.publish_out = publish_out
        self.ln1, self.qkv, self.proj, self.ln2, self.fc1, self.fc2 = ln1, qkv, proj, ln2, fc1, fc2


ATTN_SINGLE_PASS_MAX = 272


class VitBlockFn(torch.autograd.Function):

    @staticmethod
    def forward(ctx, x, spec):
        B, N, D = x.shape
        M, dt = B * N, compute_dtype()
        if N > ATTN_SINGLE_PASS_MAX and (ctx.needs_input_grad[0] or spec.mask is not None):
            raise UiaError(f"vit_block: {N} tokens exceed the {ATTN_SINGLE_PASS_MAX} of the attention backward; sequences this long run forward-only "
                           "(frozen tower under torch.no_grad()), unmasked" if ctx.needs_input_grad[0] else
                           f"vit_block: {N} tokens with a mask: the long attention forward takes no mask")
        x3 = fwd3_of(x)
        like = x3.lo if x3 is not None else x
        if x3 is None:
            x = x.contiguous()
            x2d = x.view(M, D)
        train = ctx.needs_input_grad[0]
        fold = ln_fold_enabled(dt, M)
        if x3 is not None:
            assert fold and dt == torch.bfloat16, "a three-byte forward token reached a block that cannot take it"
            rows = (x3.hi, x3.sums)
        else:
            rows = take_rows(x, dt) if fold else None
        qkv = _empty((M, 3 * D), dt, like)
        if rows is not None:
            wq, cq, bq = WEIGHTS.get_lnfold(spec.qkv[0], spec.qkv[1], spec.ln1[0], spec.ln1[1], dt)
            xin_t, sums0 = rows
            if not ops.is_kb(xin_t):
                xin_t = xin_t.view(M, D)
            ops.gemm(xin_t, wq, bias=bq, out_t=qkv, lnfold=(sums0, cq, D, spec.eps))
            h1 = _act(M, D, dt, like, spec.fc1[0].shape[0]) if x3 is not None else xin_t
        else:
            h1 = _empty((M, D), dt, x)
            ops.layernorm_fwd(x2d, spec.ln1[0], spec.ln1[1], spec.eps, y_t=h1)
            ops.gemm(h1, WEIGHTS.get(spec.qkv[0], dt), bias=spec.qkv[1], out_t=qkv)
        if handoff.take_last_block_cls() and spec.mask is None and 1 < N <= ATTN_SINGLE_PASS_MAX and D == 64 * spec.heads and like.is_cuda:
            return VitBlockFn._forward_cls(ctx, x, x3, qkv, spec, (B, N, D), dt, train)
        if N > ATTN_SINGLE_PASS_MAX:
            a = _empty((M, D), dt, like)
            ops.attn_fwd_long(qkv[:, :D], qkv[:, D:2 * D], qkv[:, 2 * D:], a, B, spec.heads, N)
            lse = None
        else:
            a = _attn_act(M, D, dt, like, D) if D == 64 * spec.heads else _empty((M, D), dt, like)
            lse = torch.empty(B, spec.heads, N, device=like.device, dtype=torch.float32) if train else None
            ops.attn_fwd(qkv[:, :D], qkv[:, D:2 * D], qkv[:, 2 * D:], a, B, spec.heads, N, lse=lse, mask=spec.mask)
        F = spec.fc1[0].shape[0]
        f = _act(M, F, dt, like, D)
        pre = _empty((M, F), dt, like) if train else None
        r3 = fold and _STATE.get("block_resid3", False) and dt == torch.bfloat16 and M > 2048
        x1 = None if r3 else torch.empty(M, D, device=like.device, dtype=torch.float32)
        lo1 = torch.empty(M, D, device=like.device, dtype=torch.int8) if r3 else None
        if fold:
            sums1 = zero_sums(M, like.device)
            h1 = _as_act(h1, M, D, dt, F) if x3 is None else h1
            resx = dict(resid3=x3.resid3) if x3 is not None else dict(resid=x2d)
            ops.gemm(a, WEIGHTS.get(spec.proj[0], dt), bias=spec.proj[1], out32=x1, out_t=h1, out_lo=lo1, rowsum=sums1, **resx)
            w1, c1, b1 = WEIGHTS.get_lnfold(spec.fc1[0], spec.fc1[1], spec.ln2[0], spec.ln2[1], dt)
            ops.gemm(h1, w1, bias=b1, act=spec.act, aux_out=pre, out_t=f, lnfold=(sums1, c1, D, spec.eps))
        else:
            ops.gemm(a, WEIGHTS.get(spec.proj[0], dt), bias=spec.proj[1], resid=x2d, out32=x1)
            h1 = _as_act(h1, M, D, dt, 0)
            ops.layernorm_fwd(x1, spec.ln2[0], spec.ln2[1], spec.eps, y_t=h1)
            ops.gemm(h1, WEIGHTS.get(spec.fc1[0], dt), bias=spec.fc1[1], act=spec.act, aux_out=pre, out_t=f)
        x2 = torch.empty(B, N, D, device=like.device, dtype=torch.float32)
        res1 = dict(resid3=Resid3(h1, lo1)) if r3 else dict(resid=x1)
        if fold and spec.publish_out:
            sums2 = zero_sums(M, like.device)
            h2 = _act(M, D, dt, like, 3 * D) if r3 else _as_act(h1, M, D, dt, 3 * D)
            ops.gemm(f, WEIGHTS.get(spec.fc2[0], dt), bias=spec.fc2[1], out32=x2.view(M, D), out_t=h2, rowsum=sums2, **res1)
            publish_rows(x2, h2, sums2)
        else:
            ops.gemm(f, WEIGHTS.get(spec.fc2[0], dt), bias=spec.fc2[1], out32=x2.view(M, D), **res1)
        if train:
            saved, ctx.layout = handoff.save_layout(x3.resid3 if x3 is not None else x, qkv, a, lse, Resid3(h1, lo1) if r3 else x1, pre)
            ctx.save_for_backward(*saved)
            ctx.xshape = (B, N, D)
            ctx.spec = spec
            ctx.g3_out = dt == torch.bfloat16 and _g3_partner_feeds(x)
            ctx.cls_ok = spec.mask is None and N <= ATTN_SINGLE_PASS_MAX and D == 64 * spec.heads and not r3 and handoff.cls_grad_enabled()
        return x2

    @staticmethod
    def _forward_cls(ctx, x, x3, qkv, spec, shape, dt, train):
        B, N, D = shape
        like = qkv
        a = _empty((B, D), dt, like)
        lse = torch.empty(B, spec.heads, device=like.device, dtype=torch.float32) if train else None
        ops.attn_fwd_cls(qkv[:, :D], qkv[:, D:2 * D], qkv[:, 2 * D:], a, B, spec.heads, N, lse=lse)
        x_cls = torch.empty(B, D, device=like.device, dtype=torch.float32)
        if x3 is not None:
            ops.rows3_to_f32(x3.hi, x3.lo, N, x_cls)
        else:
            ops.copy_rows(x.view(B * N, D), N, x_cls)
        x1 = torch.empty(B, D, device=like.device, dtype=torch.float32)
        M = B * N
        wp = WEIGHTS.get(spec.proj[0], dt)
        ops.gemm(a, wp, bias=spec.proj[1], resid=x_cls, out32=x1, tile_cfg=_rows_tile_cfg(M, wp, like, dt, out32=True, resid=True))
        h2 = _empty((B, D), dt, like)
        ops.layernorm_fwd(x1, spec.ln2[0], spec.ln2[1], spec.eps, y_t=h2)
        F = spec.fc1[0].shape[0]
        f = _empty((B, F), dt, like)
        pre = _empty((B, F), dt, like) if train else None
        w1, w2 = WEIGHTS.get(spec.fc1[0], dt), WEIGHTS.get(spec.fc2[0], dt)
        ops.gemm(h2, w1, bias=spec.fc1[1], act=spec.act, aux_out=pre, out_t=f, tile_cfg=_rows_tile_cfg(M, w1, like, dt, act=True, aux_out=train, out_t=True))
        x2 = torch.empty(B, 1, D, device=like.device, dtype=torch.float32)
        ops.gemm(f, w2, bias=spec.fc2[1], resid=x1, out32=x2.view(B, D), tile_cfg=_rows_tile_cfg(M, w2, like, dt, out32=True, resid=True))
        if train:
            saved, ctx.layout = handoff.save_layout(x3.resid3 if x3 is not None else x, qkv, a, lse, x1, pre)
            ctx.save_for_backward(*saved)
            ctx.xshape = (B, N, D)
            ctx.spec = spec
            ctx.g3_out = dt == torch.bfloat16 and _g3_partner_feeds(x)
            ctx.cls_ok = False
            ctx.cls_fwd = True
        handoff.cls_rows_out(True)
        return x2

    @staticmethod
    def backward_cls(ctx, cg):
        compact = getattr(ctx, "cls_fwd", False)
        xin, qkv, a, lse, x1, pre = handoff.restore_layout(ctx.saved_tensors, ctx.layout)
        x3_in = isinstance(xin, Resid3)
        x = xin.lo if x3_in else xin
        spec = ctx.spec
        B, N, D = ctx.xshape
        M, dt = B * N, qkv.dtype
        F = pre.shape[1]
        dy = cg.rows32
        dy_t = dy if dt == torch.float32 else (cg.rows_t if cg.rows_t is not None else t_copy_of(dy, dt))
        pre_cls = pre if compact else ops.copy_rows(pre, N, _empty((B, F), dt, x))
        dpre = _empty((B, F), dt, x)
        ops.gemm(dy_t, WEIGHTS.get(spec.fc2[0], dt, transpose=True), dact=spec.act, aux_in=pre_cls, out_t=dpre)
        dh = _empty((B, D), dt, x)
        ops.gemm(dpre, WEIGHTS.get(spec.fc1[0], dt, transpose=True), out_t=dh)
        x1_cls = x1 if compact else ops.copy_rows(x1, N, _empty((B, D), torch.float32, x))
        dx1 = _empty((B, D), torch.float32, x)
        dx1_t = _empty((B, D), dt, x) if dt != torch.float32 else dx1
        ops.layernorm_bwd(dh, x1_cls, spec.ln2[0], spec.eps, dres=dy, dx32=dx1, dx_t=dx1_t if dt != torch.float32 else None)
        da = dh
        ops.gemm(dx1_t, WEIGHTS.get(spec.proj[0], dt, transpose=True), out_t=da)
        dqkv = _attn_act(M, 3 * D, dt, x, D)
        if ops.is_kb(dqkv):
            ops.attn_bwd_cls(qkv[:, :D], qkv[:, D:2 * D], qkv[:, 2 * D:], a, da, lse, dqkv, None, None, B, spec.heads, N, rows=compact)
        else:
            ops.attn_bwd_cls(qkv[:, :D], qkv[:, D:2 * D], qkv[:, 2 * D:], a, da, lse, dqkv[:, :D], dqkv[:, D:2 * D], dqkv[:, 2 * D:], B, spec.heads, N, rows=compact)
        dh1 = _empty((M, D), dt, x)
        ops.gemm(dqkv, WEIGHTS.get(spec.qkv[0], dt, transpose=True), out_t=dh1)
        xrows = xin if x3_in else x.view(M, D)
        if getattr(ctx, "g3_out", False):
            dx_t = _empty((M, D), dt, x)
            dlo = torch.empty(M, D, device=x.device, dtype=torch.int8)
            ops.layernorm_bwd_periodic(dh1, xrows, spec.ln1[0], spec.eps, dx1, N, dx_t=dx_t, dx_lo=dlo)
            return publish_grad3((B, N, D), x.device, dx_t, dlo), None
        dx = torch.empty(B, N, D, device=x.device, dtype=torch.float32)
        if dt == torch.float32:
            ops.layernorm_bwd_periodic(dh1, xrows, spec.ln1[0], spec.eps, dx1, N, dx32=dx.view(M, D))
            return dx, None
        dx_t = _empty((M, D), dt, x)
        ops.layernorm_bwd(dh1, xrows, spec.ln1[0], spec.eps, dres=ClsGrad(dx1, None, N).decode().view(M, D), dx32=dx.view(M, D), dx_t=dx_t)
        publish_t_copy(dx, dx_t)
        return dx, None

    @staticmethod
    def backward(ctx, dx2):
        if getattr(ctx, "cls_fwd", False):
            dx2 = dx2.contiguous()
            B, N, D = ctx.xshape
            dt = ctx.saved_tensors[-1].dtype
            return VitBlockFn.backward_cls(ctx, ClsGrad(dx2.view(B, D), t_copy_of(dx2, dt).view(B, D) if dt != torch.float32 else None, N))
        cg = cls_grad_of(dx2)
        if cg is not None:
            if getattr(ctx, "cls_ok", False):
                return VitBlockFn.backward_cls(ctx, cg)
            dx2 = cg.decode()
        g3 = grad3_of(dx2)
        xin, qkv, a, lse, x1, pre = handoff.restore_layout(ctx.saved_tensors, ctx.layout)
        x3_in, r3 = isinstance(xin, Resid3), isinstance(x1, Resid3)
        x = xin.lo if x3_in else xin
        spec = ctx.spec
        B, N, D = ctx.xshape
        M, dt = B * N, qkv.dtype
        F = pre.shape[1]
        if g3 is not None:
            dx2_t = g3.hi if ops.is_kb(g3.hi) else g3.hi.view(M, D)
            dres2 = Resid3(dx2_t, g3.lo)
        else:
            dx2 = dx2.contiguous()
            dx2_t = t_copy_of(dx2, dt, allow_kb=True)
            if not ops.is_kb(dx2_t):
                dx2_t = dx2_t.view(M, D)
            dres2 = dx2.view(M, D)
        g3_mode = g3 is not None or getattr(ctx, "g3_out", False)
        dpre = _act(M, F, dt, x, D)
        ops.gemm(dx2_t, WEIGHTS.get(spec.fc2[0], dt, transpose=True), dact=spec.act, aux_in=pre, out_t=dpre)
        dh = _empty((M, D), dt, x)
        ops.gemm(dpre, WEIGHTS.get(spec.fc1[0], dt, transpose=True), out_t=dh)
        del dpre
        if r3 or g3_mode:
            dx1_t = _empty((M, D), dt, x)
            dlo1 = torch.empty(M, D, device=x.device, dtype=torch.int8)
            ops.layernorm_bwd(dh, x1, spec.ln2[0], spec.eps, dres=dres2, dx_t=dx1_t, dx_lo=dlo1)
            dx1 = Resid3(dx1_t, dlo1)
        else:
            dx1 = torch.empty_like(x1)
            dx1_t = _empty((M, D), dt, x) if dt != torch.float32 else dx1
            ops.layernorm_bwd(dh, x1, spec.ln2[0], spec.eps, dres=dres2, dx32=dx1, dx_t=dx1_t if dt != torch.float32 else None)
        da = dh
        ops.gemm(dx1_t, WEIGHTS.get(spec.proj[0], dt, transpose=True), out_t=da)
        dqkv = _attn_act(M, 3 * D, dt, x, D) if D == 64 * spec.heads else _empty((M, 3 * D), dt, x)
        if ops.is_kb(dqkv):
            ops.attn_bwd(qkv[:, :D], qkv[:, D:2 * D], qkv[:, 2 * D:], a, da, lse, dqkv, None, None, B, spec.heads, N, mask=spec.mask)
        else:
            ops.attn_bwd(qkv[:, :D], qkv[:, D:2 * D], qkv[:, 2 * D:], a, da, lse, dqkv[:, :D], dqkv[:, D:2 * D], dqkv[:, 2 * D:], B, spec.heads, N, mask=spec.mask)
        ops.gemm(dqkv, WEIGHTS.get(spec.qkv[0], dt, transpose=True), out_t=da)
        dx_t = _empty((M, D), dt, x) if dt != torch.float32 else None
        xrows = xin if x3_in else x.view(M, D)
        if getattr(ctx, "g3_out", False):
            dlo = torch.empty(M, D, device=x.device, dtype=torch.int8)
            ops.layernorm_bwd(da, xrows, spec.ln1[0], spec.eps, dres=dx1, dx_t=dx_t, dx_lo=dlo)
            return publish_grad3((B, N, D), x.device, dx_t, dlo), None
        dx = torch.empty(B, N, D, device=x.device, dtype=torch.float32)
        ops.layernorm_bwd(da, xrows, spec.ln1[0], spec.eps, dres=dx1, dx32=dx.view(M, D), dx_t=dx_t)
        publish_t_copy(dx, dx_t)
        return dx, None


def vit_block(x, spec):
    return VitBlockFn.apply(x, spec)


class LnResidual:
    __slots__ = ("raw", "stats", "w", "b", "dim", "eps", "hi", "lo")

    def __init__(self, raw, stats, w, b, dim=None, eps=None, hi=None, lo=None):
        self.raw, self.stats, self.w, self.b = raw, stats, w, b
        self.dim, self.eps = dim, eps
        self.hi, self.lo = hi, lo

    def gemm_kw(self):
        if self.lo is not None:
            return dict(resid3=Resid3(self.hi, self.lo), resid_ln=(self.stats, self.w, self.b, self.dim, self.eps))
        if self.stats is None:
            return dict(resid=self.raw)
        if self.dim is None:
            return dict(resid=self.raw, resid_ln=(self.stats, self.w, self.b))
        return dict(resid=self.raw, resid_ln=(self.stats, self.w, self.b, self.dim, self.eps))


def _post_ln(raw, w, b, eps, x_t, stats_buf=None):
    if _STATE.get("text_ln_deferred", True):
        stats = stats_buf if stats_buf is not None else torch.empty(raw.shape[0], 2, device=raw.device, dtype=torch.float32)
        ops.layernorm_fwd(raw, w, b, eps, y_t=x_t, stats=stats)
        return LnResidual(raw, stats, w, b)
    ops.layernorm_fwd(raw, w, b, eps, y_t=x_t, y32=raw)
    return LnResidual(raw, None, w, b)


def post_ln_embed(e32, ln, x_t):
    return _post_ln(e32, ln.weight, ln.bias, ln.eps, x_t)


def _res_cls_rows(res, L, B, D, eps):
    rows = torch.empty(B, D, device=res.w.device, dtype=torch.float32)
    if res.lo is not None:
        ops.rows3_to_f32(res.hi, res.lo, L, rows)
    else:
        ops.copy_rows(res.raw.view(-1, D), L, rows)
        if res.stats is None:
            return rows
    ops.layernorm_fwd(rows, res.w, res.b, res.eps if res.eps is not None else eps, y32=rows)
    return rows


def post_ln_layer_cls_ok(x_t, heads, L, cu_seqlens=None):
    D = x_t.cols if ops.is_kb(x_t) else x_t.shape[1]
    return cu_seqlens is None and D == 64 * heads and 1 < L <= 288 and x_t.is_cuda and not (x_t.dtype != torch.float32 and _STATE.get("text_resid_t", False))


def _post_ln_layer_cls(res, qkv, L, B, heads, P, keylen, eps, D, dt):
    a = _empty((B, D), dt, qkv)
    ops.attn_fwd_cls(qkv[:, :D], qkv[:, D:2 * D], qkv[:, 2 * D:], a, B, heads, L, mask="keypad", keylen=keylen)
    r = _res_cls_rows(res, L, B, D, eps)
    s_a = torch.empty(B, D, device=qkv.device, dtype=torch.float32)
    M = B * L
    wo = WEIGHTS.get(P["attention.output.dense.weight"], dt)
    ops.gemm(a, wo, bias=P["attention.output.dense.bias"], resid=r, out32=s_a, tile_cfg=_rows_tile_cfg(M, wo, qkv, dt, out32=True, resid=True))
    h = _empty((B, D), dt, qkv)
    ops.layernorm_fwd(s_a, P["attention.output.LayerNorm.weight"], P["attention.output.LayerNorm.bias"], eps, y_t=h, y32=s_a)
    F = P["intermediate.dense.weight"].shape[0]
    f = _empty((B, F), dt, qkv)
    w1, w2 = WEIGHTS.get(P["intermediate.dense.weight"], dt), WEIGHTS.get(P["output.dense.weight"], dt)
    ops.gemm(h, w1, bias=P["intermediate.dense.bias"], act="gelu", out_t=f, tile_cfg=_rows_tile_cfg(M, w1, qkv, dt, act=True, out_t=True))
    ops.gemm(f, w2, bias=P["output.dense.bias"], resid=s_a, out32=r, tile_cfg=_rows_tile_cfg(M, w2, qkv, dt, out32=True, resid=True))
    ops.layernorm_fwd(r, P["output.LayerNorm.weight"], P["output.LayerNorm.bias"], eps, y_t=h, y32=r)
    return LnResidual(r, None, P["output.LayerNorm.weight"], P["output.LayerNorm.bias"]), h


def post_ln_layer(res, x_t, L, B, heads, P, keylen, eps=1e-12, cu_seqlens=None, fold_sums=None, fold_out=False, cls_only=False):
    kb_in = ops.is_kb(x_t)
    M, D = (x_t.rows, x_t.cols) if kb_in else x_t.shape
    dt = x_t.dtype
    t_resid = dt != torch.float32 and _STATE.get("text_resid_t", False)
    fold = fold_sums is not None and ln_fold_enabled(dt, M) and not t_resid
    qkv = _empty((M, 3 * D), dt, x_t)
    if res.dim is not None:
        wq, cq, bq = WEIGHTS.get_lnfold(P["_qkv_raw"][0], P["_qkv_raw"][1], res.w, res.b, dt)
        ops.gemm(x_t, wq, bias=bq, out_t=qkv, lnfold=(res.stats, cq, D, res.eps))
    else:
        ops.gemm(x_t, P["_qkv_w"](dt), bias=P["_qkv_b"], out_t=qkv)
    if cls_only:
        return _post_ln_layer_cls(res, qkv, L, B, heads, P, keylen, eps, D, dt)
    a = _attn_act(M, D, dt, x_t, D) if (D == 64 * heads and cu_seqlens is None) else _empty((M, D), dt, x_t)
    if cu_seqlens is not None:
        ops.attn_fwd(qkv[:, :D], qkv[:, D:2 * D], qkv[:, 2 * D:], a, B, heads, L, cu_seqlens=cu_seqlens)
    else:
        ops.attn_fwd(qkv[:, :D], qkv[:, D:2 * D], qkv[:, 2 * D:], a, B, heads, L, mask="keypad", keylen=keylen)
    del qkv
    F = P["intermediate.dense.weight"].shape[0]
    f = _act(M, F, dt, x_t, D)
    r3 = fold and _STATE.get("text_resid3", True) and dt == torch.bfloat16 and M > 2048
    if fold:
        lw_a, lb_a = P["attention.output.LayerNorm.weight"], P["attention.output.LayerNorm.bias"]
        s_a_t = _act(M, D, dt, x_t, F)
        if r3:
            lo_a = torch.empty(M, D, device=x_t.device, dtype=torch.int8)
            ops.gemm(a, WEIGHTS.get(P["attention.output.dense.weight"], dt), bias=P["attention.output.dense.bias"], out_t=s_a_t, out_lo=lo_a,
                     rowsum=fold_sums[0], **res.gemm_kw())
            res_a = LnResidual(None, fold_sums[0], lw_a, lb_a, D, eps, hi=s_a_t, lo=lo_a)
        else:
            s_a = torch.empty(M, D, device=x_t.device, dtype=torch.float32)
            ops.gemm(a, WEIGHTS.get(P["attention.output.dense.weight"], dt), bias=P["attention.output.dense.bias"], out32=s_a, out_t=s_a_t,
                     rowsum=fold_sums[0], **res.gemm_kw())
            res_a = LnResidual(s_a, fold_sums[0], lw_a, lb_a, D, eps)
        w1, c1, b1 = WEIGHTS.get_lnfold(P["intermediate.dense.weight"], P["intermediate.dense.bias"], lw_a, lb_a, dt)
        ops.gemm(s_a_t, w1, bias=b1, act="gelu", out_t=f, lnfold=(fold_sums[0], c1, D, eps))
        if not r3:
            del s_a_t
    else:
        s_a = torch.empty(M, D, device=x_t.device, dtype=torch.float32)
        ops.gemm(a, WEIGHTS.get(P["attention.output.dense.weight"], dt), bias=P["attention.output.dense.bias"], out32=s_a,
                 **(dict(resid_t=x_t) if t_resid else res.gemm_kw()))
        x_t = _as_act(x_t, M, D, dt, 0)
        res_a = _post_ln(s_a, P["attention.output.LayerNorm.weight"], P["attention.output.LayerNorm.bias"], eps, x_t)
        ops.gemm(x_t, WEIGHTS.get(P["intermediate.dense.weight"], dt), bias=P["intermediate.dense.bias"], act="gelu", out_t=f)
    s_o = res.raw if res.raw is not None else torch.empty(M, D, device=x_t.device, dtype=torch.float32)
    if fold and fold_out:
        x_t = _as_act(x_t, M, D, dt, 3 * D)
        if r3:
            lo_o = res.lo if res.lo is not None else torch.empty(M, D, device=x_t.device, dtype=torch.int8)
            ops.gemm(f, WEIGHTS.get(P["output.dense.weight"], dt), bias=P["output.dense.bias"], out_t=x_t, out_lo=lo_o, rowsum=fold_sums[1],
                     **res_a.gemm_kw())
            return LnResidual(None, fold_sums[1], P["output.LayerNorm.weight"], P["output.LayerNorm.bias"], D, eps, hi=x_t, lo=lo_o), x_t
        ops.gemm(f, WEIGHTS.get(P["output.dense.weight"], dt), bias=P["output.dense.bias"], out32=s_o, out_t=x_t, rowsum=fold_sums[1],
                 **res_a.gemm_kw())
        return LnResidual(s_o, fold_sums[1], P["output.LayerNorm.weight"], P["output.LayerNorm.bias"], D, eps), x_t
    ops.gemm(f, WEIGHTS.get(P["output.dense.weight"], dt), bias=P["output.dense.bias"], out32=s_o,
             **(dict(resid_t=x_t) if t_resid else res_a.gemm_kw()))
    stats_buf = res.stats if (res.dim is None and res.stats is not None) else None
    x_t = _as_act(x_t, M, D, dt, 0)
    return _post_ln(s_o, P["output.LayerNorm.weight"], P["output.LayerNorm.bias"], eps, x_t, stats_buf=stats_buf), x_t


_GRAY_W = {}


def gray_conv_weight(conv_w):
    if conv_w.requires_grad:
        raise NotImplementedError("one-channel input through a TRAINABLE patch embedding: widen the batch instead (src.datasets.segmentation.as_model_input)")
    key = id(conv_w)
    hit = _GRAY_W.get(key)
    sig = (conv_w._version, conv_w.data_ptr(), conv_w.dtype, conv_w.device)
    if hit is None or hit[0] != sig or hit[2]() is not conv_w:
        import weakref
        hit = _GRAY_W[key] = (sig, conv_w.detach().float().sum(dim=1, keepdim=True).contiguous(), weakref.ref(conv_w))
    return hit[1]


class PatchEmbedFn(torch.autograd.Function):

    @staticmethod
    def forward(ctx, images, conv_w, conv_b, cls, pos, patch):
        dt = compute_dtype()
        B, C, H, W = images.shape
        G = (H // patch) * (W // patch)
        D = conv_w.shape[0]
        K = C * patch * patch
        gran = 64 if dt == torch.bfloat16 else 32
        Kp = (K + gran - 1) // gran * gran
        cols = _empty((B * G, Kp), dt, images)
        ops.im2col(images.contiguous().float(), cols, patch)
        x = torch.empty(B, G + 1, D, device=images.device, dtype=torch.float32)
        pos2d = pos.detach().reshape(G + 1, D).contiguous()
        ops.gemm(cols, WEIGHTS.get(conv_w, dt, pad_cols_to=Kp), bias=conv_b, resid=pos2d, resid_mod=G, resid_row_off=1, out_group=G, out32=x.view(-1, D))
        ops.fill_cls(x, cls.detach().reshape(D).contiguous(), pos2d[0])
        return x

    @staticmethod
    def backward(ctx, g):
        return None, None, None, None, None, None


class ClsHeadFn(torch.autograd.Function):

    @staticmethod
    def forward(ctx, x, ln_w, ln_b, eps, w, w_is_in_out=False):
        B, N, D = x.shape
        dt = head_dtype()
        x = x.contiguous()
        h = _empty((B, D), dt, x)
        ops.layernorm_fwd(x, ln_w, ln_b, eps, y_t=h, rows=B, ldx=N * D)
        E = w.shape[1] if w_is_in_out else w.shape[0]
        feat = torch.empty(B, E, device=x.device, dtype=torch.float32)
        ops.gemm(h, WEIGHTS.get(w, dt, transpose=w_is_in_out), out32=feat)
        ctx.save_for_backward(x, ln_w)
        ctx.meta = (eps, w, w_is_in_out, dt)
        ctx.cls_out = handoff.takes_cls_grad(x, in_chain=False)
        return feat

    @staticmethod
    def backward(ctx, dfeat):
        x, ln_w = ctx.saved_tensors
        eps, w, w_is_in_out, hdt = ctx.meta
        B, N, D = x.shape
        dt = compute_dtype()
        df = t_copy_of(dfeat.contiguous(), hdt)
        dh = _empty((B, D), hdt, x)
        E = df.shape[1]
        if E % 64:
            Ep = (E + 63) // 64 * 64
            dfp = df.new_zeros(B, Ep)
            dfp[:, :E] = df
            df = dfp
            wt = WEIGHTS.get(w, hdt, transpose=not w_is_in_out, **({"pad_cols_to": Ep} if w_is_in_out else {"pad_rows_to": Ep}))
        else:
            wt = WEIGHTS.get(w, hdt, transpose=not w_is_in_out)
        ops.gemm(df, wt, out_t=dh)
        if hdt != dt:
            dh_t = _empty((B, D), dt, x)
            ops.cast(dh, dh_t)
            dh = dh_t
        if getattr(ctx, "cls_out", False):
            x_cls = ops.copy_rows(x.view(B * N, D), N, _empty((B, D), torch.float32, x))
            rows32 = _empty((B, D), torch.float32, x)
            rows_t = _empty((B, D), dt, x) if dt != torch.float32 else None
            ops.layernorm_bwd(dh, x_cls, ln_w, eps, dx32=rows32, dx_t=rows_t)
            return publish_cls_grad(x.shape, x.device, rows32, rows_t), None, None, None, None, None
        dx = torch.zeros_like(x)
        dx_t = torch.zeros(B * N, D, device=x.device, dtype=dt) if dt != torch.float32 else None
        ops.layernorm_bwd(dh, x, ln_w, eps, dx32=dx, dx_t=dx_t, rows=B, ldx=N * D)
        publish_t_copy(dx, dx_t)
        return dx, None, None, None, None, None


class LayerNormFn(torch.autograd.Function):

    @staticmethod
# ... 1077 lines not shown
```

nextgen-uia_amd/uia_hip/handoff.py:

```python
from typing import NamedTuple

import torch

from . import ops

_STATE = {"chain_depth": 0, "fwd3_next_plain": False, "grad_resid3": False, "cls_grad": True,
          "cls_forward": True, "cls_decl": False, "cls_last": False, "cls_rows": False}


class Resid3(NamedTuple):
    hi: object
    lo: torch.Tensor

    def decode(self):
        return ops.three_byte_to_float(self.hi, self.lo).contiguous()


class Fwd3(NamedTuple):
    hi: object
    lo: torch.Tensor
    sums: torch.Tensor

    @property
    def resid3(self):
        return Resid3(self.hi, self.lo)


class ClsGrad(NamedTuple):
    rows32: torch.Tensor
    rows_t: object
    tokens: int

    def decode(self):
        B, D = self.rows32.shape
        dense = self.rows32.new_zeros(B, self.tokens, D)
        dense[:, 0] = self.rows32
        return dense


def save_layout(*values):
    tensors, tags = [], []
    for v in values:
        three = isinstance(v, Resid3)
        hi = v.hi if three else v
        kb = ops.is_kb(hi)
        tensors.append(hi.t if kb else hi)
        if three:
            tensors.append(v.lo)
        tags.append(("3" if three else "") + ("kb" if kb else "rows"))
    return tensors, tuple(tags)


def restore_layout(tensors, tags):
    it, out = iter(tensors), []
    for tag in tags:
        hi = next(it)
        if tag.endswith("kb"):
            hi = ops.KBlocked(hi)
        out.append(Resid3(hi, next(it)) if tag[0] == "3" else hi)
    return out


class TokenRegistry:

    def __init__(self, size):
        self.size, self._pools, self._live = size, {}, {}

    def publish(self, shape, device, payload):
        key = (device.type, device.index if device.index is not None else (torch.cuda.current_device() if device.type == "cuda" else 0))
        pool = self._pools.get(key)
        if pool is None:
            pool = self._pools[key] = [torch.full((self.size,), float("nan"), device=device, dtype=torch.float32), 0]
        i = pool[1]
        pool[1] = (i + 1) % self.size
        tok = pool[0][i:i + 1].view((1,) * len(shape)).expand(shape)
        if len(self._live) >= self.size:
            self._live.clear()
        self._live[tok.data_ptr()] = (payload, tok.numel())
        return tok

    def take(self, t):
        if not self._live or t.dim() == 0 or any(st != 0 for st, n in zip(t.stride(), t.shape) if n > 1):
            return None
        payload, numel = self._live.pop(t.data_ptr(), (None, 0))
        return payload if numel == t.numel() else None

    def clear(self):
        self._live.clear()


GRAD3 = TokenRegistry(64)
FWD3 = TokenRegistry(256)
CLSG = TokenRegistry(64)
_G3_VIEWS = ("PermuteBackward0", "ViewBackward0", "UnsafeViewBackward0", "TransposeBackward0", "AliasBackward0", "ReshapeAliasBackward0")
_G3_PARTNERS = ("MonaFnBackward", "VitBlockFnBackward")


def publish_grad3(shape, device, hi, lo):
    return GRAD3.publish(shape, device, Resid3(hi, lo))


def grad3_of(g):
    return GRAD3.take(g)


def grad3_decode(hi, lo):
    return Resid3(hi, lo).decode()


def publish_fwd3(shape, device, hi, lo, sums):
    return FWD3.publish(shape, device, Fwd3(hi, lo, sums))


def fwd3_of(x):
    return FWD3.take(x)


def publish_cls_grad(shape, device, rows32, rows_t):
    return CLSG.publish(shape, device, ClsGrad(rows32, rows_t, shape[1]))


def cls_grad_of(g):
    return CLSG.take(g)


def set_cls_grad(flag):
    _STATE["cls_grad"] = bool(flag)


def cls_grad_enabled():
    return _STATE["cls_grad"] and _STATE["grad_resid3"]


def set_grad_resid3(flag):
    _STATE["grad_resid3"] = bool(flag)


def grad_resid3_enabled():
    return _STATE["grad_resid3"]


class linear_chain:

    def __enter__(self):
        _STATE["chain_depth"] += 1
        return self

    def __exit__(self, *exc):
        _STATE["chain_depth"] -= 1
        _STATE["fwd3_next_plain"] = False
        _STATE["cls_last"] = _STATE["cls_rows"] = False
        return False

    @staticmethod
    def last_block_cls(flag):
        _STATE["cls_last"] = bool(flag)

    @staticmethod
    def next_is_plain_block(flag):
        _STATE["fwd3_next_plain"] = bool(flag)


def fwd3_consumer_ahead():
    return _STATE["fwd3_next_plain"] and _STATE["chain_depth"] > 0


def take_last_block_cls():
    flag = _STATE["cls_last"] and _STATE["chain_depth"] > 0
    _STATE["cls_last"] = False
    return flag


def cls_rows_out(flag):
    _STATE["cls_rows"] = bool(flag)


def take_cls_rows():
    flag = _STATE["cls_rows"] and _STATE["chain_depth"] > 0
    _STATE["cls_rows"] = False
    return flag


class cls_only:

    def __enter__(self):
        _STATE["cls_decl"] = True
        return self

    def __exit__(self, *exc):
        _STATE["cls_decl"] = False
        return False


def take_cls_forward():
    flag = _STATE["cls_decl"] and _STATE["cls_forward"]
    _STATE["cls_decl"] = False
    return flag


def cls_declared():
    return _STATE["cls_decl"]


def set_cls_forward(flag):
    _STATE["cls_forward"] = bool(flag)


def hook_free(*modules):
    import torch.nn.modules.module as _mm
    if _mm._global_forward_hooks or _mm._global_forward_pre_hooks or _mm._global_backward_hooks or getattr(_mm, "_global_backward_pre_hooks", None) \
            or getattr(_mm, "_global_forward_hooks_always_called", None):
        return False
    for mod in modules:
        for m in mod.modules():
            if m._forward_hooks or m._forward_pre_hooks or m._backward_hooks or getattr(m, "_backward_pre_hooks", None):
                return False
    return True


def partner_node(x, in_chain=True):
    if not _STATE["grad_resid3"] or (in_chain and _STATE["chain_depth"] <= 0):
        return None
    fn = x.grad_fn
    for _ in range(8):
        if fn is None:
            return None
        name = type(fn).__name__
        if name in _G3_PARTNERS:
            return fn
        if name not in _G3_VIEWS or len(fn.next_functions) != 1:
            return None
        fn = fn.next_functions[0][0]
    return None


def _g3_partner_feeds(x):
    return partner_node(x) is not None


def takes_cls_grad(x, in_chain=True):
    return cls_grad_enabled() and bool(getattr(partner_node(x, in_chain), "cls_ok", False))


_T_COPIES = {}


def publish_t_copy(g32, g_t):
    if g_t is not None and g_t.dtype != torch.float32:
        if len(_T_COPIES) >= 256:
            _T_COPIES.clear()
        _T_COPIES[g32.data_ptr()] = (g32, g32._version, g_t)


def t_copy_of(g32, dt, allow_kb=False):
    if dt == torch.float32:
        return g32
    hit = _T_COPIES.pop(g32.data_ptr(), None)
    if hit is not None:
        src, version, g_t = hit
        if (src.shape == g32.shape and src.stride() == g32.stride() and version == g32._version
                and src.untyped_storage().data_ptr() == g32.untyped_storage().data_ptr() and g_t.dtype == dt and (allow_kb or not ops.is_kb(g_t))):
            return g_t
    out = torch.empty(g32.shape, device=g32.device, dtype=dt)
    ops.cast(g32.contiguous(), out)
    return out


_SUMS_ARENA = {}


def zero_sums(M, device, stream=None):
    key = ops.raw_stream() if stream is None else stream
    a = _SUMS_ARENA.get(key)
    if a is None or a[0].shape[1] != M or a[0].device != device or a[1] >= a[0].shape[0]:
        a = [torch.zeros(48, M, 2, device=device, dtype=torch.int64), 0]
        _SUMS_ARENA[key] = a
    a[1] += 1
    return a[0][a[1] - 1]


_ROWS = {}


def publish_rows(x32, x_t, sums, stream=None):
    _ROWS[ops.raw_stream() if stream is None else stream] = (x32, x32._version, x_t, sums)


def take_rows(x32, dt, stream=None):
    hit = _ROWS.pop(ops.raw_stream() if stream is None else stream, None)
    if hit is not None:
        src, version, x_t, sums = hit
        if (src.data_ptr() == x32.data_ptr() and src.numel() == x32.numel() and version == x32._version
                and src.untyped_storage().data_ptr() == x32.untyped_storage().data_ptr() and x32.is_contiguous() and x_t.dtype == dt):
            return x_t, sums
    return None


def clear():
    _T_COPIES.clear()
    _ROWS.clear()
    _SUMS_ARENA.clear()
    GRAD3.clear()
    FWD3.clear()
    CLSG.clear()
```

nextgen-uia_amd/uia_hip/ops.py:

```python
import ctypes as C
from typing import NamedTuple

import torch

from . import _lib
from ._lib import AttnDesc, GemmDesc, LnLoraDesc, LoraRankDesc, MonaFusedDesc, MonaSpatialDesc, PackDesc, UiaError, WgradGroupDesc, check, lib

_ACT = {None: 0, "none": 0, "gelu": 1, "quick_gelu": 2, "relu": 3}

GEMM_PROFILE = None


EPI_BIAS, EPI_AUX_OUT, EPI_GELU, EPI_DGELU, EPI_RESID, EPI_RESIDT, EPI_OUT32, EPI_OUTT, EPI_RESID_LN, EPI_GENERIC = 1, 2, 4, 8, 16, 32, 64, 128, 256, -1
EPI_QUICK = 2048
EPI_ROWSUM, EPI_LNFOLD = 512, 1024
EPI_RESID_LO, EPI_OUT_LO = 4096, 8192
_SPECIALISED = {EPI_BIAS | EPI_RESID | EPI_OUT32, EPI_BIAS | EPI_RESIDT | EPI_OUT32, EPI_BIAS | EPI_RESID | EPI_RESID_LN | EPI_OUT32, EPI_OUTT, EPI_BIAS | EPI_OUTT, EPI_BIAS | EPI_GELU | EPI_OUTT, EPI_DGELU | EPI_OUTT,
                EPI_BIAS | EPI_GELU | EPI_AUX_OUT | EPI_OUTT,
                EPI_QUICK | EPI_BIAS | EPI_GELU | EPI_OUTT, EPI_QUICK | EPI_DGELU | EPI_OUTT, EPI_QUICK | EPI_BIAS | EPI_GELU | EPI_AUX_OUT | EPI_OUTT,
                EPI_BIAS | EPI_RESID | EPI_OUT32 | EPI_OUTT | EPI_ROWSUM, EPI_BIAS | EPI_RESID | EPI_RESID_LN | EPI_OUT32 | EPI_OUTT | EPI_ROWSUM,
                EPI_BIAS | EPI_OUTT | EPI_LNFOLD, EPI_BIAS | EPI_GELU | EPI_OUTT | EPI_LNFOLD, EPI_BIAS | EPI_GELU | EPI_AUX_OUT | EPI_OUTT | EPI_LNFOLD,
                EPI_QUICK | EPI_BIAS | EPI_GELU | EPI_OUTT | EPI_LNFOLD, EPI_QUICK | EPI_BIAS | EPI_GELU | EPI_AUX_OUT | EPI_OUTT | EPI_LNFOLD,
                EPI_BIAS | EPI_RESID_LO | EPI_RESID_LN | EPI_OUTT | EPI_OUT_LO | EPI_ROWSUM,
                EPI_BIAS | EPI_RESID | EPI_OUTT | EPI_OUT_LO | EPI_ROWSUM, EPI_BIAS | EPI_RESID_LO | EPI_OUT32,
# ... 696 lines not shown


LORA_WGRAD_GROUP = True


def wgrad_group(a_list, b_list, dw_list, dbias_list=None, alpha=1.0, drop=None):
    n = len(a_list)
    a0, b0, w0 = a_list[0], b_list[0], dw_list[0]
    if not (1 <= n <= 4 and len(b_list) == n and len(dw_list) == n and a0.dtype == torch.bfloat16):
        raise UiaError("wgrad_group: 1..4 bf16 problems")
    lda, ldb = _rowmajor(a0, "a"), _rowmajor(b0, "b")
    M, I, J = a0.shape[0], a0.shape[1], b0.shape[1]
    d = WgradGroupDesc()
    d.n, d.M, d.I, d.J, d.lda, d.ldb, d.ldw = n, M, I, J, lda, ldb, w0.shape[1]
    d.i_valid, d.j_valid, d.alpha = w0.shape[0], w0.shape[1], alpha
    for g in range(n):
        a, b, w = a_list[g], b_list[g], dw_list[g]
        if (a.dtype != torch.bfloat16 or b.dtype != torch.bfloat16 or tuple(a.shape) != (M, I) or tuple(b.shape) != (M, J) or _rowmajor(a, "a") != lda or _rowmajor(b, "b") != ldb
                or w.dtype != torch.float32 or not w.is_contiguous() or w.shape != w0.shape or w.shape[0] > I or w.shape[1] > J):
            raise UiaError(f"wgrad_group: problem {g} does not have the shape / strides / dtypes of problem 0")
        d.A[g], d.B[g], d.dW[g] = a.data_ptr(), b.data_ptr(), w.data_ptr()
        db = dbias_list[g] if dbias_list is not None else None
        if db is not None:
            assert db.dtype == torch.float32 and db.numel() >= w.shape[0]
            d.dbias_A[g] = db.data_ptr()
    if drop is not None:
        p_, seeds = drop
        if ldb != J or (dbias_list is not None and any(x is not None for x in dbias_list)):
            raise UiaError("wgrad_group(drop=...): no bias, and each b must be the whole dropped tensor (contiguous rows)")
        d.drop_p, d.drop_ld, d.drop_col0 = float(p_), J, 0
        for g in range(n):
            d.drop_seed[g] = int(seeds[g]) & 0xFFFFFFFFFFFFFFFF
    check(lib().uia_wgrad_group(_stream(), _code(a0.dtype), C.byref(d)), "uia_wgrad_group")


def _attn_desc(q, k, v, out, lse, B, H, L, mask, keylen, scale, dh=None):
    d = AttnDesc()
    for t in (q, k, v):
        if t.stride(-1) != 1 or t.dtype != q.dtype:
            raise UiaError("attention operands must be unit-stride in the last dim and share a dtype")
    width = q.shape[-1]
    if width % H != 0 or (dh is not None and dh * H != width) or k.shape[-1] != width or v.shape[-1] != width:
        raise UiaError(f"attention: q / k / v are {q.shape[-1]} / {k.shape[-1]} / {v.shape[-1]} columns wide for {H} heads" + (f" of dim {dh}" if dh is not None else ""))
    dh = width // H
    if dh not in (16, 32, 64):
        raise UiaError(f"attention: head dim {dh} unsupported (16, 32 or 64): {width} columns over {H} heads")
    if not is_kb(out) and out.shape[-1] != width:
        raise UiaError(f"attention: out is {out.shape[-1]} columns wide, q / k / v {width}")
    d.q, d.k, d.v, d.ld_qkv = _p(q), _p(k), _p(v), q.stride(-2)
    assert k.stride(-2) == q.stride(-2) == v.stride(-2)
    if is_kb(out):
        rows, cols, d.out_kb_rows = _kb_dims(out, "attention out")
        if rows < B * L or cols != H * dh or dh != 64 or q.dtype != torch.bfloat16:
            raise UiaError(f"attention out (K-blocked {tuple(out.t.shape)}) must hold [{B * L}, {H * dh}] bf16 with head dim 64")
        d.out, d.ldo = _p(out.t), cols
    else:
        d.out, d.ldo = _p(out), out.stride(-2)
    d.lse = _p(lse)
    d.keylen = _p(keylen)
    d.B, d.H, d.L, d.dh = B, H, L, dh
    d.mask_kind = {"none": 0, None: 0, "causal": 1, "keypad": 2}[mask]
    d.scale = scale if scale is not None else dh ** -0.5
    return d


def attn_fwd(q, k, v, out, B, H, L, lse=None, mask=None, keylen=None, scale=None, dh=None, cu_seqlens=None):
    d = _attn_desc(q, k, v, out, lse, B, H, L, mask, keylen, scale, dh)
    if cu_seqlens is not None:
        assert cu_seqlens.dtype == torch.int32 and cu_seqlens.is_contiguous() and cu_seqlens.numel() == B + 1
        d.cu_seqlens = _p(cu_seqlens)
    check(lib().uia_attn_fwd(_stream(), _code(q.dtype), C.byref(d)), "uia_attn_fwd")


def attn_fwd_long(q, k, v, out, B, H, L, lse=None, scale=None):
    if is_kb(out):
        raise UiaError("attn_fwd_long: the output must be a row-major tensor, not K-blocked")
    d = _attn_desc(q, k, v, out, lse, B, H, L, None, None, scale)
    if d.dh != 64:
        raise UiaError(f"attn_fwd_long: head dim {d.dh}, only 64 is supported")
    check(lib().uia_attn_fwd_long(_stream(), _code(q.dtype), C.byref(d)), "uia_attn_fwd_long")


ATTN_BWD_CFG = 0


def attn_bwd(q, k, v, out, dout, lse, dq, dk, dv, B, H, L, mask=None, keylen=None, scale=None, dh=None, cfg=None):
    d = _attn_desc(q, k, v, out, lse, B, H, L, mask, keylen, scale, dh)
    dh = d.dh
    d.dout, d.lddo = _p(dout), dout.stride(-2)
    if is_kb(dq):
        rows, cols, d.dqkv_kb_rows = _kb_dims(dq, "attention dqkv")
        if rows < B * L or cols != 3 * H * dh or dh != 64 or q.dtype != torch.bfloat16 or dk is not None or dv is not None:
            raise UiaError(f"attention dqkv (K-blocked {tuple(dq.t.shape)}) must hold [{B * L}, {3 * H * dh}] bf16 with head dim 64, dk = dv = None")
        part = (H * dh // kb_group(q.dtype)) * d.dqkv_kb_rows * kb_group(q.dtype) * dq.t.element_size()
        d.dq, d.dk, d.dv, d.ld_dqkv = dq.t.data_ptr(), dq.t.data_ptr() + part, dq.t.data_ptr() + 2 * part, cols
    else:
        d.dq, d.dk, d.dv, d.ld_dqkv = _p(dq), _p(dk), _p(dv), dq.stride(-2)
        assert dk.stride(-2) == dq.stride(-2) == dv.stride(-2)
    cfg = ATTN_BWD_CFG if cfg is None else cfg
    if cfg:
        check(lib().uia_attn_bwd_cfg(_stream(), _code(q.dtype), C.byref(d), int(cfg)), "uia_attn_bwd_cfg")
    else:
        check(lib().uia_attn_bwd(_stream(), _code(q.dtype), C.byref(d)), "uia_attn_bwd")


def attn_bwd_cls(q, k, v, out, dout, lse, dq, dk, dv, B, H, L, mask=None, scale=None, rows=False):
    if mask not in (None, "none"):
        raise UiaError(f"attn_bwd_cls: mask {mask!r}: the CLS-query backward takes unmasked attention only")
    d = _attn_desc(q, k, v, out, lse, B, H, L, None, None, scale)
    if d.dh != 64:
        raise UiaError(f"attn_bwd_cls: head dim {d.dh}, only 64 is supported")
    if dout.dim() != 2 or dout.shape[0] != B or dout.shape[1] != H * 64 or dout.stride(1) != 1 or dout.dtype != q.dtype:
        raise UiaError(f"attn_bwd_cls: dout must be [{B}, {H * 64}] {q.dtype} rows (one per sequence), got {tuple(dout.shape)} {dout.dtype}")
    compact = bool(rows)
    if compact and (is_kb(out) or out.dim() != 2 or out.shape[0] != B or out.stride(1) != 1 or out.dtype != q.dtype):
        raise UiaError(f"attn_bwd_cls(rows=True): out must be [{B}, {H * 64}] {q.dtype} rows (one per sequence)")
    if lse is None or lse.dtype != torch.float32 or not lse.is_contiguous() or lse.numel() != (B * H if compact else B * H * L):
        raise UiaError(f"attn_bwd_cls: lse must be a contiguous fp32 [{B}, {H}, {L}] tensor ([{B}, {H}] beside a compact out)")
    d.dout, d.lddo = _p(dout), dout.stride(0)
    if is_kb(dq):
        rows, cols, d.dqkv_kb_rows = _kb_dims(dq, "attention dqkv")
        if rows < B * L or cols != 3 * H * 64 or q.dtype != torch.bfloat16 or dk is not None or dv is not None:
            raise UiaError(f"attention dqkv (K-blocked {tuple(dq.t.shape)}) must hold [{B * L}, {3 * H * 64}] bf16 with head dim 64, dk = dv = None")
        part = (H * 64 // kb_group(q.dtype)) * d.dqkv_kb_rows * kb_group(q.dtype) * dq.t.element_size()
        d.dq, d.dk, d.dv, d.ld_dqkv = dq.t.data_ptr(), dq.t.data_ptr() + part, dq.t.data_ptr() + 2 * part, cols
    else:
        for name, t in (("dq", dq), ("dk", dk), ("dv", dv)):
            if t.dtype != q.dtype or t.dim() != 2 or t.shape[0] < B * L or t.shape[1] != H * 64 or t.stride(1) != 1 or t.stride(0) != dq.stride(0):
                raise UiaError(f"attn_bwd_cls: {name} must be [{B * L}, {H * 64}] {q.dtype} rows sharing one row stride, got {tuple(t.shape)} {t.dtype}")
        d.dq, d.dk, d.dv, d.ld_dqkv = _p(dq), _p(dk), _p(dv), dq.stride(0)
    if compact:
        check(lib().uia_attn_bwd_cls_rows(_stream(), _code(q.dtype), C.byref(d)), "uia_attn_bwd_cls_rows")
    else:
        check(lib().uia_attn_bwd_cls(_stream(), _code(q.dtype), C.byref(d)), "uia_attn_bwd_cls")


def attn_fwd_cls(q, k, v, out, B, H, L, lse=None, mask=None, keylen=None, scale=None):
    if mask not in (None, "none", "keypad"):
        raise UiaError(f"attn_fwd_cls: mask {mask!r}: none or key padding only")
    if is_kb(out) or out.dim() != 2 or out.shape[0] != B or out.shape[1] != H * 64 or out.stride(1) != 1 or out.dtype != q.dtype:
        raise UiaError(f"attn_fwd_cls: out must be [{B}, {H * 64}] {q.dtype} rows (one per sequence)")
    if q.shape[0] < B * L:
        raise UiaError(f"attn_fwd_cls: q / k / v hold {q.shape[0]} rows, {B} sequences of {L} need {B * L}")
    if lse is not None and (lse.dtype != torch.float32 or not lse.is_contiguous() or lse.numel() != B * H):
        raise UiaError(f"attn_fwd_cls: lse must be a contiguous fp32 [{B}, {H}] tensor")
    if mask == "keypad" and (keylen is None or keylen.dtype != torch.int32 or not keylen.is_contiguous() or keylen.numel() != B):
        raise UiaError(f"attn_fwd_cls: key padding needs keylen int32 [{B}]")
    d = _attn_desc(q, k, v, out, lse, B, H, L, mask, keylen if mask == "keypad" else None, scale)
    if d.dh != 64:
        raise UiaError(f"attn_fwd_cls: head dim {d.dh}, only 64 is supported")
    check(lib().uia_attn_fwd_cls(_stream(), _code(q.dtype), C.byref(d)), "uia_attn_fwd_cls")


def rows3_to_f32(hi, lo, stride_rows, dst):
    rows, D = dst.shape
    if dst.dtype != torch.float32 or not dst.is_contiguous() or lo.dtype != torch.int8 or lo.dim() != 2 or lo.stride(1) != 1 or lo.shape[1] != D:
        raise UiaError(f"rows3_to_f32: dst fp32 contiguous [rows, D] and lo int8 [M, D] are required, got {tuple(dst.shape)} {dst.dtype} / {tuple(lo.shape)} {lo.dtype}")
    _require(rows > 0 and stride_rows > 0 and (rows - 1) * stride_rows < lo.shape[0], f"rows3_to_f32: {rows} rows {stride_rows} apart do not fit the {lo.shape[0]} rows of lo")
    if is_kb(hi):
        hrows, hcols, kb_rows = _kb_dims(hi, "rows3_to_f32 hi")
        _require(hi.dtype == torch.bfloat16 and hcols == D and (rows - 1) * stride_rows < hrows, "rows3_to_f32: the K-blocked hi plane must hold bf16 [M, D]")
        hp, ldhi = hi.t.data_ptr(), D
    else:
        _require(hi.dtype == torch.bfloat16 and hi.dim() == 2 and hi.stride(1) == 1 and hi.shape[1] == D and (rows - 1) * stride_rows < hi.shape[0],
                 "rows3_to_f32: the hi plane must hold bf16 [M, D] rows")
        hp, ldhi, kb_rows = hi.data_ptr(), hi.stride(0), 0
    check(lib().uia_rows3_to_f32(_stream(), rows, D, stride_rows, hp, ldhi, kb_rows, _p(lo), lo.stride(0), _p(dst)), "uia_rows3_to_f32")
    return dst


def layernorm_fwd(x, gamma, beta, eps, y_t=None, y32=None, rows=None, ldx=None, stats=None):
    D = gamma.numel()
    rows = x.numel() // D if rows is None else rows
    ldx = D if ldx is None else ldx
    dt = _code(y_t.dtype) if y_t is not None else _lib.F32
    if stats is not None:
        assert stats.dtype == torch.float32 and stats.is_contiguous() and stats.numel() >= 2 * rows
        check(lib().uia_layernorm_fwd_stats(_stream(), dt, rows, D, ldx, _p(x), _p(gamma), _p(beta), eps, _p(y_t), _p(y32), _p(stats)), "uia_layernorm_fwd_stats")
        return
    check(lib().uia_layernorm_fwd(_stream(), dt, rows, D, ldx, _p(x), _p(gamma), _p(beta), eps, _p(y_t), _p(y32)), "uia_layernorm_fwd")


POOL_SLICES = 32


def ln_mean_rows(x, gamma, beta, eps, row0, n, out=None):
    if x.dim() != 3 or x.dtype != torch.float32 or x.stride(-1) != 1 or x.stride(1) != x.shape[2] or x.stride(0) != x.shape[1] * x.shape[2]:
        raise UiaError("ln_mean_rows: x must be a contiguous fp32 [B, L, D] tensor")
    B, L, D = x.shape
    if out is None:
        out = torch.empty(B, D, device=x.device, dtype=torch.float32)
    if out.dtype != torch.float32 or out.stride(-1) != 1 or out.shape[-1] != D or out.shape[0] != B:
        raise UiaError("ln_mean_rows: out must be fp32 [B, D] with unit column stride")
    ws = torch.empty(B * POOL_SLICES * D, device=x.device, dtype=torch.float32)
    check(lib().uia_ln_mean_rows(_stream(), B, L, int(row0), int(n), D, D, _p(x), _p(gamma), _p(beta), float(eps), _p(ws), _p(out), out.stride(0)),
          "uia_ln_mean_rows")
    return out


def layernorm_bwd(dy, x, gamma, eps, dres=None, dx32=None, dx_t=None, rows=None, ldx=None, dx_lo=None):
    D = gamma.numel()
    rows = dy.numel() // D if rows is None else rows
    ldx = D if ldx is None else ldx
    if isinstance(x, tuple) or isinstance(dres, tuple) or dx_lo is not None:
        x_hi, x_lo = x if isinstance(x, tuple) else (None, None)
        r_hi, r_lo = dres if isinstance(dres, tuple) else (None, None)
        x_kb = r_kb = 0
        if is_kb(x_hi):
            kr, kc, x_kb = _kb_dims(x_hi, "layernorm_bwd x hi plane")
            if kr < rows or kc != D:
                raise UiaError(f"layernorm_bwd: K-blocked x hi plane {tuple(x_hi.t.shape)} does not hold [{rows}, {D}]")
            x_hi = x_hi.t
        if is_kb(r_hi):
            kr, kc, r_kb = _kb_dims(r_hi, "layernorm_bwd dres hi plane")
            if kr < rows or kc != D:
                raise UiaError(f"layernorm_bwd: K-blocked dres hi plane {tuple(r_hi.t.shape)} does not hold [{rows}, {D}]")
            r_hi = r_hi.t
        for name, t, dt_ in (("x hi", x_hi, torch.bfloat16), ("x lo", x_lo, torch.int8), ("dres hi", r_hi, torch.bfloat16), ("dres lo", r_lo, torch.int8), ("dx_lo", dx_lo, torch.int8)):
            if t is not None and (t.dtype != dt_ or not t.is_contiguous() or t.numel() < rows * D):
                raise UiaError(f"layernorm_bwd: {name} plane must be a contiguous {dt_} tensor of at least [{rows}, {D}], got {tuple(t.shape)} {t.dtype}")
        check(lib().uia_layernorm_bwd3(_stream(), _code(dy.dtype), rows, D, ldx, _p(dy), None if isinstance(x, tuple) else _p(x), _p(x_hi), _p(x_lo), x_kb, _p(gamma), eps,
                                       None if isinstance(dres, tuple) else _p(dres), _p(r_hi), _p(r_lo), r_kb, _p(dx32), _p(dx_t), _p(dx_lo)), "uia_layernorm_bwd3")
        return
    check(lib().uia_layernorm_bwd(_stream(), _code(dy.dtype), rows, D, ldx, _p(dy), _p(x), _p(gamma), eps, _p(dres), _p(dx32), _p(dx_t)), "uia_layernorm_bwd")


def layernorm_bwd_periodic(dy, x, gamma, eps, dres_rows, period, dx32=None, dx_t=None, dx_lo=None):
    D = gamma.numel()
    M = dy.numel() // D
    nrows = (M + period - 1) // period
    _dense(dres_rows, "layernorm_bwd_periodic: dres_rows", _F32, nrows * D, align=16)
    x_hi, x_lo = x if isinstance(x, tuple) else (None, None)
    x_kb = 0
    if is_kb(x_hi):
        kr, kc, x_kb = _kb_dims(x_hi, "layernorm_bwd_periodic x hi plane")
        if kr < M or kc != D:
            raise UiaError(f"layernorm_bwd_periodic: K-blocked x hi plane {tuple(x_hi.t.shape)} does not hold [{M}, {D}]")
        x_hi = x_hi.t
    for name, t, dt_ in (("dy", dy, dy.dtype), ("x", None if isinstance(x, tuple) else x, torch.float32), ("x hi", x_hi, torch.bfloat16), ("x lo", x_lo, torch.int8),
                         ("dx32", dx32, torch.float32), ("dx_t", dx_t, dy.dtype), ("dx_lo", dx_lo, torch.int8)):
        if t is not None and (t.dtype != dt_ or not t.is_contiguous() or t.numel() < M * D):
            raise UiaError(f"layernorm_bwd_periodic: {name} must be a contiguous {dt_} tensor of at least [{M}, {D}], got {tuple(t.shape)} {t.dtype}")
    check(lib().uia_layernorm_bwd_periodic(_stream(), _code(dy.dtype), M, D, _p(dy), None if isinstance(x, tuple) else _p(x), _p(x_hi), _p(x_lo), x_kb, _p(gamma), eps,
                                           _p(dres_rows), int(period), _p(dx32), _p(dx_t), _p(dx_lo)), "uia_layernorm_bwd_periodic")


def cast(src, dst, scale=1.0):
    _dense(src, "cast: src", _F32, align=16)
    _dense(dst, "cast: dst", _FT, src.numel(), align="v4")
    check(lib().uia_cast(_stream(), _code(dst.dtype), src.numel(), _p(src), _p(dst), scale), "uia_cast")


def transpose_cast(src, dst):
    _dense(src, "transpose_cast: src", _F32)
    _dense(dst, "transpose_cast: dst", _FT)
    _require(src.dim() == 2 and tuple(dst.shape) == (src.shape[1], src.shape[0]),
             f"transpose_cast: dst shape {tuple(dst.shape)} is not the transpose of src {tuple(src.shape)}")
    check(lib().uia_transpose_cast(_stream(), _code(dst.dtype), src.shape[0], src.shape[1], _p(src), _p(dst)), "uia_transpose_cast")


_PIN_RING, _PIN_SLOTS, _PIN_SLOT = {}, 512, 4096


def pack_table(entries, device):
    arr = (PackDesc * len(entries))()
    max_elems = 0
    for d, ent in zip(arr, entries):
        src, row, row_kb, tr, tr_kb = ent[:5]
        assert src.dtype == torch.float32 and src.dim() == 2 and src.is_contiguous()
        R, Cc = src.shape
        RP, CP, scale = ent[5] if len(ent) > 5 and ent[5] is not None else (R, Cc, 1.0)
        assert RP >= R and CP >= Cc
        d.src, d.rows, d.cols, d.rows_pad, d.cols_pad, d.scale = _p(src), R, Cc, RP, CP, float(scale)
        for name, t in (("row", row), ("row_kb", row_kb), ("tr", tr), ("tr_kb", tr_kb)):
            if isinstance(t, RawDest):
                assert t.view.device == src.device
                setattr(d, name, t.view.data_ptr())
            elif t is not None:
                assert t.is_contiguous() and t.numel() == RP * CP and t.device == src.device
                setattr(d, name, _p(t))
            if t is not None and name.endswith("_kb"):
                g = 64 // (t.view.element_size() if isinstance(t, RawDest) else t.element_size())
                k, kp = (Cc, CP) if name == "row_kb" else (R, RP)
                if -(-k // g) * g > kp:
                    raise UiaError(f"pack_table: {name} needs its K extent {kp} >= {k} rounded up to {g}")
        max_elems = max(max_elems, R * Cc)
    nbytes = C.sizeof(arr)
    dev = torch.device(device)
    if dev.type == "cuda" and nbytes <= _PIN_SLOT:
        key = dev.index if dev.index is not None else torch.cuda.current_device()
        ring = _PIN_RING.get(key)
        if ring is None:
            ring = _PIN_RING[key] = [torch.empty(_PIN_SLOTS, _PIN_SLOT, dtype=torch.uint8).pin_memory(), 0, [None] * _PIN_SLOTS]
        i = ring[1]
        slot = ring[0][i]
        ring[1] = (i + 1) % _PIN_SLOTS
        if ring[2][i] is not None:
            ring[2][i].synchronize()
        C.memmove(slot.data_ptr(), C.addressof(arr), nbytes)
        table = torch.empty(nbytes, dtype=torch.uint8, device=dev)
        table.copy_(slot[:nbytes], non_blocking=True)
        ev = torch.cuda.Event()
        ev.record()
        ring[2][i] = ev
        return table, len(entries), max_elems
    raw = torch.frombuffer(bytearray(bytes(arr)), dtype=torch.uint8).clone()
# ... 1109 lines not shown
```

Before: 6696.

## Fold CLS-only attention QKV projection into per-sequence reductions

Adds a cls_fold path for layers where only the CLS output row is needed. Instead of projecting all tokens to Q, K and V and running attention, it computes q for the CLS row, folds it through W_k into a score vector applied directly to the normalized inputs, and applies W_v after the softmax-weighted sum of inputs. The backward pass is folded the same way, producing dh1 without materializing dqkv. This removes the full QKV GEMMs over all tokens in the final layer, at the cost of new custom kernels with extra numerical-path complexity and restrictions on head count and sequence length.

```diff
diff --git a/include/uia_hip.h b/include/uia_hip.h
--- a/include/uia_hip.h
+++ b/include/uia_hip.h
@@ -110,6 +110,24 @@
 int uia_attn_fwd_cls(void* stream, int dtype, const uia_attn_desc* d);
 int uia_attn_bwd_cls_rows(void* stream, int dtype, const uia_attn_desc* d);
 
+typedef struct uia_cls_fold_desc {
+    const void* A; int64_t lda; int64_t a_kb_rows;
+    const void* W; const void* Wu;
+    const float* bias;
+    const void* ln_sums; const float* ln_colsum; float ln_eps;
+    float scale;
+    int32_t B, H, L, reserved;
+    const int32_t* keylen;
+    void* out; int64_t ldo;
+    float* q; float* p;
+    const void* dout; int64_t lddo;
+    void* dh1; int64_t ld_dh1;
+    void* ws; uint64_t ws_bytes;
+} uia_cls_fold_desc;
+size_t uia_cls_fold_workspace_bytes(int B, int H, int L);
+int uia_cls_fold_fwd(void* stream, const uia_cls_fold_desc* d);
+int uia_cls_fold_bwd(void* stream, const uia_cls_fold_desc* d);
+
 int uia_layernorm_fwd(void* stream, int dtype, int M, int D, int64_t ldx, const float* x, const float* gamma, const float* beta,
                       float eps, void* yT, float* y32);
 int uia_layernorm_fwd_stats(void* stream, int dtype, int M, int D, int64_t ldx, const float* x, const float* gamma, const float* beta,
diff --git a/nextgen-uia_amd/csrc/capi.cpp b/nextgen-uia_amd/csrc/capi.cpp
--- a/nextgen-uia_amd/csrc/capi.cpp
+++ b/nextgen-uia_amd/csrc/capi.cpp
@@ -92,6 +92,15 @@
     NEED(d, "uia_attn_fwd_cls");
     return uia_attn_fwd_cls_launch((hipStream_t)stream, dtype, *d);
 }
+size_t uia_cls_fold_workspace_bytes(int B, int H, int L) { return uia_cls_fold_ws_bytes(B, H, L); }
+int uia_cls_fold_fwd(void* stream, const uia_cls_fold_desc* d) {
+    NEED(d, "uia_cls_fold_fwd");
+    return uia_cls_fold_fwd_launch((hipStream_t)stream, *d);
+}
+int uia_cls_fold_bwd(void* stream, const uia_cls_fold_desc* d) {
+    NEED(d, "uia_cls_fold_bwd");
+    return uia_cls_fold_bwd_launch((hipStream_t)stream, *d);
+}
 int uia_mona_cls_fwd(void* stream, int dtype, int B, int ntok, const void* t, int64_t ldt, void* d, float p_drop, uint64_t seed, const uint8_t* keep_mask) {
     return uia_mona_cls_fwd_launch((hipStream_t)stream, dtype, B, ntok, t, (long)ldt, d, p_drop, seed, keep_mask);
 }
diff --git a/nextgen-uia_amd/csrc/cls_fold.hip b/nextgen-uia_amd/csrc/cls_fold.hip
--- /dev/null
+++ b/nextgen-uia_amd/csrc/cls_fold.hip
@@ -0,0 +1,582 @@
+#include "uia_common.h"
+#include "uia_kernels.h"
+
+namespace {
+
+struct FoldA {
+    const bf16_t* A;
+    long lda, kb_rows;
+};
+__device__ __forceinline__ const bf16_t* a_at(const FoldA& a, size_t row, int c) {
+    return a.kb_rows ? a.A + ((size_t)(c >> 5) * (size_t)a.kb_rows + row) * 32 + (c & 31) : a.A + row * (size_t)a.lda + c;
+}
+
+template <int VW> __device__ __forceinline__ void loadv(const bf16_t* p, float* o);
+template <> __device__ __forceinline__ void loadv<4>(const bf16_t* p, float* o) {
+    const bf16x4 v = *(const bf16x4*)p;
+    o[0] = (float)v[0]; o[1] = (float)v[1]; o[2] = (float)v[2]; o[3] = (float)v[3];
+}
+template <> __device__ __forceinline__ void loadv<2>(const bf16_t* p, float* o) {
+    const bf16x2 v = *(const bf16x2*)p;
+    o[0] = (float)v[0]; o[1] = (float)v[1];
+}
+template <> __device__ __forceinline__ void loadv<1>(const bf16_t* p, float* o) { o[0] = (float)*p; }
+template <int VW> struct RawV;
+template <> struct RawV<4> { bf16x4 v; };
+template <> struct RawV<2> { bf16x2 v; };
+template <> struct RawV<1> { bf16_t v; };
+__device__ __forceinline__ void rawload(const bf16_t* p, RawV<4>& r) { r.v = *(const bf16x4*)p; }
+__device__ __forceinline__ void rawload(const bf16_t* p, RawV<2>& r) { r.v = *(const bf16x2*)p; }
+__device__ __forceinline__ void rawload(const bf16_t* p, RawV<1>& r) { r.v = *p; }
+__device__ __forceinline__ void rawcvt(const RawV<4>& r, float* o) { o[0] = (float)r.v[0]; o[1] = (float)r.v[1]; o[2] = (float)r.v[2]; o[3] = (float)r.v[3]; }
+__device__ __forceinline__ void rawcvt(const RawV<2>& r, float* o) { o[0] = (float)r.v[0]; o[1] = (float)r.v[1]; }
+__device__ __forceinline__ void rawcvt(const RawV<1>& r, float* o) { o[0] = (float)r.v; }
+template <int VW> __device__ __forceinline__ void loadvf(const float* p, float* o) {
+#pragma unroll
+    for (int e = 0; e < VW; ++e) o[e] = p[e];
+}
+
+__device__ __forceinline__ float2 fold_row_ln(const void* sums, size_t row, int dim, float eps) {
+    if (!sums) return float2{1.f, 0.f};
+    const long long* s = (const long long*)sums + 2 * row;
+    const float s1 = (float)s[0] * (1.0f / 1073741824.0f), s2 = (float)s[1] * (1.0f / 1073741824.0f);
+    const float inv = 1.0f / (float)dim;
+    const float mean = s1 * inv;
+    const float var = fmaxf(fmaf(-mean, mean, s2 * inv), 0.0f);
+    const float rstd = rsqrtf(var + eps);
+    return float2{rstd, -mean * rstd};
+}
+
+template <int H> struct Cols {
+    static constexpr int VW = H % 4 == 0 ? 4 : (H % 2 == 0 ? 2 : 1), NT = H / VW, HP = (H + 3) / 4 * 4;
+    static __device__ __forceinline__ int col(int t, int lane) { return 64 * VW * t + VW * lane; }
+};
+
+template <int N> __device__ __forceinline__ float dot_n(const float (&a)[N], const float (&x)[N]) {
+    if constexpr (N % 2 == 0) {
+        f32x2 acc = {0.f, 0.f};
+#pragma unroll
+        for (int i = 0; i < N; i += 2) {
+            const f32x2 a2 = {a[i], a[i + 1]}, x2 = {x[i], x[i + 1]};
+            acc = __builtin_elementwise_fma(a2, x2, acc);
+        }
+        return acc[0] + acc[1];
+    } else {
+        float acc = 0.f;
+#pragma unroll
+        for (int i = 0; i < N; ++i) acc = fmaf(a[i], x[i], acc);
+        return acc;
+    }
+}
+template <int N> __device__ __forceinline__ void axpy_n(float c, const float (&x)[N], float (&acc)[N]) {
+    if constexpr (N % 2 == 0) {
+        const f32x2 c2 = {c, c};
+#pragma unroll
+        for (int i = 0; i < N; i += 2) {
+            const f32x2 x2 = {x[i], x[i + 1]}, a2 = {acc[i], acc[i + 1]};
+            const f32x2 r = __builtin_elementwise_fma(c2, x2, a2);
+            acc[i] = r[0];
+            acc[i + 1] = r[1];
+        }
+    } else {
+#pragma unroll
+        for (int i = 0; i < N; ++i) acc[i] = fmaf(c, x[i], acc[i]);
+    }
+}
+
+template <int N>
+__device__ __forceinline__ float wave_sum_pick(const float (&a)[N], int lane) {
+    float mine = 0.f;
+#pragma unroll
+    for (int h = 0; h < N; ++h) {
+        float v = a[h];
+        v += uia_dpp_quad_xor1(v);
+        v += uia_dpp_quad_xor2(v);
+        v += uia_dpp_half_mirror(v);
+        v += uia_dpp_row_mirror(v);
+        mine = (lane & 15) == h ? v : mine;
+    }
+    return rows_sum(mine);
+}
+
+struct FoldDotParams {
+    const bf16_t* W;
+    FoldA A;
+    const void* sums; float eps;
+    const float* v;
+    const float* ms;
+    const float* colsum;
+    const float* bias;
+    float alpha;
+    int B, L, src_a;
+    float* out32; bf16_t* outT; long ldo;
+};
+constexpr int FDOT_ROWS = 8, FDOT_BCHUNK = 8;
+
+template <int H>
+__global__ __launch_bounds__(256) void fold_dot_kernel(const FoldDotParams p) {
+    using C = Cols<H>;
+    constexpr int D = 64 * H;
+    const int lane = threadIdx.x & 63, wave = threadIdx.x >> 6;
+    const int n_first = blockIdx.x * 32 + wave * FDOT_ROWS, h = n_first >> 6;
+    float w[FDOT_ROWS][H];
+#pragma unroll
+    for (int r = 0; r < FDOT_ROWS; ++r)
+#pragma unroll
+        for (int t = 0; t < C::NT; ++t) loadv<C::VW>(p.W + (size_t)(n_first + r) * D + C::col(t, lane), &w[r][t * C::VW]);
+    const int n = n_first + (lane & 7);
+    const float cs = p.colsum ? p.colsum[n] : 0.f, bi = p.bias ? p.bias[n] : 0.f;
+    const int b_end = min(p.B, (int)(blockIdx.y + 1) * FDOT_BCHUNK);
+    auto fetch = [&](int b, float (&v)[H]) {
+        if (p.src_a) {
+#pragma unroll
+            for (int t = 0; t < C::NT; ++t) loadv<C::VW>(a_at(p.A, (size_t)b * p.L, C::col(t, lane)), &v[t * C::VW]);
+        } else {
+#pragma unroll
+            for (int t = 0; t < C::NT; ++t) loadvf<C::VW>(p.v + ((size_t)b * H + h) * D + C::col(t, lane), &v[t * C::VW]);
+        }
+    };
+    int b = blockIdx.y * FDOT_BCHUNK;
+    float vn[H];
+    if (b < b_end) fetch(b, vn);
+    for (; b < b_end; ++b) {
+        float v[H];
+#pragma unroll
+        for (int i = 0; i < H; ++i) v[i] = vn[i];
+        if (b + 1 < b_end) fetch(b + 1, vn);
+        float alpha = p.alpha, ms = 0.f;
+        if (p.src_a) {
+            const float2 st = fold_row_ln(p.sums, (size_t)b * p.L, D, p.eps);
+            alpha = st.x;
+            ms = st.y;
+        } else if (p.ms) {
+            ms = p.ms[(size_t)b * H + h];
+        }
+        float acc[FDOT_ROWS];
+#pragma unroll
+        for (int r = 0; r < FDOT_ROWS; ++r) acc[r] = dot_n<H>(w[r], v);
+        const float mine = wave_sum_pick<FDOT_ROWS>(acc, lane);
+        if (lane < FDOT_ROWS) {
+            const float r = p.src_a ? fmaf(mine, alpha, fmaf(ms, cs, bi)) : fmaf(alpha, fmaf(ms, cs, mine), bi);
+            if (p.out32) p.out32[(size_t)b * p.ldo + n] = r;
+            else p.outT[(size_t)b * p.ldo + n] = (bf16_t)r;
+        }
+    }
+}
+
+struct FoldHeadTParams {
+    const bf16_t* W;
+    const float* u32;
+    const bf16_t* uT; long ldu;
+    const float* colsum;
+    float* cout;
+    float* out;
+    int B;
+};
+constexpr int FHT_BT = 8, FHT_DU = 8;
+struct FoldHeadTBatch {
+    FoldHeadTParams p[3];
+};
+
+template <int H>
+__global__ __launch_bounds__(H * 16 < 64 ? 64 : H * 16) void fold_headT_kernel(const FoldHeadTBatch batch) {
+    constexpr int D = 64 * H;
+    const FoldHeadTParams& p = batch.p[blockIdx.z];
+    __shared__ __attribute__((aligned(16))) float u[64][FHT_BT];
+    const int tid = threadIdx.x, h = blockIdx.x, b0 = blockIdx.y * FHT_BT;
+    for (int i = tid; i < 64 * FHT_BT; i += blockDim.x) {
+        const int bb = i >> 6, d = i & 63, b = b0 + bb;
+        float val = 0.f;
+        if (b < p.B) val = p.u32 ? p.u32[(size_t)b * D + h * 64 + d] : (float)p.uT[(size_t)b * p.ldu + h * 64 + d];
+        u[d][bb] = val;
+    }
+    __syncthreads();
+    if (p.cout && tid < FHT_BT && b0 + tid < p.B) {
+        float c = 0.f;
+        for (int d = 0; d < 64; ++d) c = fmaf(u[d][tid], p.colsum[h * 64 + d], c);
+        p.cout[(size_t)(b0 + tid) * H + h] = c;
+    }
+    if (tid >= 16 * H) return;
+    const int c0 = 4 * tid;
+    float acc[FHT_BT][4];
+#pragma unroll
+    for (int bb = 0; bb < FHT_BT; ++bb)
+#pragma unroll
+        for (int e = 0; e < 4; ++e) acc[bb][e] = 0.f;
+    for (int d0 = 0; d0 < 64; d0 += FHT_DU) {
+        float w[FHT_DU][4];
+#pragma unroll
+        for (int dd = 0; dd < FHT_DU; ++dd) loadv<4>(p.W + (size_t)(h * 64 + d0 + dd) * D + c0, w[dd]);
+#pragma unroll
+        for (int dd = 0; dd < FHT_DU; ++dd)
+#pragma unroll
+            for (int g = 0; g < FHT_BT / 4; ++g) {
+                const f32x4 u4 = *(const f32x4*)&u[d0 + dd][4 * g];
+                const float uu[4] = {u4[0], u4[1], u4[2], u4[3]};
+#pragma unroll
+                for (int k = 0; k < 4; ++k) axpy_n<4>(uu[k], w[dd], acc[4 * g + k]);
+            }
+    }
+#pragma unroll
+    for (int bb = 0; bb < FHT_BT; ++bb)
+        if (b0 + bb < p.B) {
+            const f32x4 r = {acc[bb][0], acc[bb][1], acc[bb][2], acc[bb][3]};
+            *(f32x4*)(p.out + ((size_t)(b0 + bb) * H + h) * D + c0) = r;
+        }
+}
+
+struct FoldSeqParams {
+    FoldA A;
+    const void* sums; float eps;
+    const int32_t* keylen;
+    const float* vec;
+    const float* cvec;
+    float scale;
+    int B, L;
+    float* p;
+    float* ds;
+    float* z;
+    float* zs;
+};
+constexpr int FSEQ_THREADS = 512, FSEQ_WAVES = FSEQ_THREADS / 64, FSEQ_MAX_L = 288, FSEQ_PF = 4;
+static_assert(FSEQ_PF == 4, "the ring holds two row pairs per wave");
+
+template <int H, bool BWD>
+__global__ __launch_bounds__(FSEQ_THREADS) void fold_seq_kernel(const FoldSeqParams p) {
+    using C = Cols<H>;
+    constexpr int D = 64 * H, HP = C::HP;
+    __shared__ __attribute__((aligned(16))) float sc[FSEQ_MAX_L][HP];
+    __shared__ float2 rs[FSEQ_MAX_L];
+    __shared__ float zbuf[H * D];
+    const int tid = threadIdx.x, lane = tid & 63, wave = tid >> 6;
+    const int b = blockIdx.x, L = p.L;
+    int n = L;
+    if (!BWD && p.keylen) {
+        n = p.keylen[b];
+        n = n < 1 ? 1 : (n > L ? L : n);
+    }
+    const size_t row0 = (size_t)b * L;
+    using Raw = RawV<C::VW>;
+    const bf16_t* abase[C::NT];
+#pragma unroll
+    for (int t = 0; t < C::NT; ++t) abase[t] = a_at(p.A, row0, C::col(t, lane));
+    const size_t arow = p.A.kb_rows ? 32 : (size_t)p.A.lda;
+    auto fetch = [&](int j, Raw (&r)[C::NT]) {
+#pragma unroll
+        for (int t = 0; t < C::NT; ++t) rawload(abase[t] + (size_t)j * arow, r[t]);
+    };
+    auto slot_row = [&](int u) { return 2 * wave + 2 * FSEQ_WAVES * (u >> 1) + (u & 1); };
+    auto unpack = [&](const Raw (&r)[C::NT], float (&x)[H]) {
+#pragma unroll
+        for (int t = 0; t < C::NT; ++t) rawcvt(r[t], &x[t * C::VW]);
+    };
+    constexpr int STRIDE = FSEQ_WAVES * FSEQ_PF;
+    Raw ring[FSEQ_PF][C::NT];
+    {
+        float vec[H][H];
+#pragma unroll
+        for (int h = 0; h < H; ++h)
+#pragma unroll
+            for (int t = 0; t < C::NT; ++t) loadvf<C::VW>(p.vec + ((size_t)b * H + h) * D + C::col(t, lane), &vec[h][t * C::VW]);
+        const float cv = (p.cvec && lane < H) ? p.cvec[(size_t)b * H + lane] : 0.f;
+#pragma unroll
+        for (int u = 0; u < FSEQ_PF; ++u)
+            if (slot_row(u) < n) fetch(slot_row(u), ring[u]);
+        for (int j0 = 0; j0 + 2 * wave < n; j0 += STRIDE) {
+#pragma unroll
+            for (int u = 0; u < FSEQ_PF; ++u) {
+                const int j = j0 + slot_row(u);
+                if (j < n) {
+                    float x[H];
+                    unpack(ring[u], x);
+                    if (j + STRIDE < n) fetch(j + STRIDE, ring[u]);
+                    const float2 st = fold_row_ln(p.sums, row0 + j, D, p.eps);
+                    float acc[H];
+#pragma unroll
+                    for (int h = 0; h < H; ++h) acc[h] = dot_n<H>(vec[h], x);
+                    const float tj = fmaf(wave_sum_pick<H>(acc, lane), st.x, st.y * cv);
+                    if (lane < H) sc[j][lane] = BWD ? tj : tj * p.scale;
+                    if (lane == 0) rs[j] = st;
+                }
+            }
+        }
+    }
+    __syncthreads();
+    for (int h = wave; h < H; h += FSEQ_WAVES) {
+        float* pg = p.p + ((size_t)b * H + h) * L;
+        float zs = 0.f;
+        if (!BWD) {
+            float m = -INFINITY;
+            for (int j = lane; j < n; j += 64) m = fmaxf(m, sc[j][h]);
+            m = wave_max(m);
+            float l = 0.f;
+            for (int j = lane; j < n; j += 64) {
+                const float e = __expf(sc[j][h] - m);
+                sc[j][h] = e;
+                l += e;
+            }
+            const float inv = 1.0f / wave_sum(l);
+            for (int j = lane; j < L; j += 64) {
+                float pj = 0.f;
+                if (j < n) {
+                    pj = sc[j][h] * inv;
+                    sc[j][h] = pj * rs[j].x;
+                    zs = fmaf(pj, rs[j].y, zs);
+                }
+                pg[j] = pj;
+            }
+        } else {
+            float dl = 0.f;
+            for (int j = lane; j < L; j += 64) dl = fmaf(pg[j], sc[j][h], dl);
+            const float delta = wave_sum(dl);
+            float* dsg = p.ds + ((size_t)b * H + h) * L;
+            for (int j = lane; j < L; j += 64) {
+                const float dsj = pg[j] * (sc[j][h] - delta);
+                dsg[j] = dsj;
+                sc[j][h] = dsj * rs[j].x;
+                zs = fmaf(dsj, rs[j].y, zs);
+            }
+        }
+        zs = wave_sum(zs);
+        if (lane == 0) p.zs[(size_t)b * H + h] = zs;
+    }
+    __syncthreads();
+    float acc[H][H];
+#pragma unroll
+    for (int h = 0; h < H; ++h)
+#pragma unroll
+        for (int i = 0; i < H; ++i) acc[h][i] = 0.f;
+#pragma unroll
+    for (int u = 0; u < FSEQ_PF; ++u)
+        if (slot_row(u) < n) fetch(slot_row(u), ring[u]);
+    for (int j0 = 0; j0 + 2 * wave < n; j0 += STRIDE) {
+#pragma unroll
+        for (int u = 0; u < FSEQ_PF; ++u) {
+            const int j = j0 + slot_row(u);
+            if (j < n) {
+                float x[H], c[HP];
+                unpack(ring[u], x);
+                if (j + STRIDE < n) fetch(j + STRIDE, ring[u]);
+#pragma unroll
+                for (int g = 0; g < HP / 4; ++g) {
+                    const f32x4 c4 = *(const f32x4*)&sc[j][4 * g];
+                    c[4 * g] = c4[0]; c[4 * g + 1] = c4[1]; c[4 * g + 2] = c4[2]; c[4 * g + 3] = c4[3];
+                }
+#pragma unroll
+                for (int h = 0; h < H; ++h) axpy_n<H>(c[h], x, acc[h]);
+            }
+        }
+    }
+    for (int w = 0; w < FSEQ_WAVES; ++w) {
+        if (wave == w) {
+#pragma unroll
+            for (int h = 0; h < H; ++h)
+#pragma unroll
+                for (int t = 0; t < C::NT; ++t)
+#pragma unroll
+                    for (int e = 0; e < C::VW; ++e) {
+                        const int col = C::col(t, lane) + e;
+                        const float v = acc[h][t * C::VW + e];
+                        if (w == 0) zbuf[h * D + col] = v;
+                        else if (w < FSEQ_WAVES - 1) zbuf[h * D + col] += v;
+                        else p.z[((size_t)b * H + h) * D + col] = zbuf[h * D + col] + v;
+                    }
+        }
+        __syncthreads();
+    }
+}
+
+struct FoldDyParams {
+    const float *qt, *vt, *qq;
+    const float *ds, *p;
+    float scale;
+    int B, L, rows_per_wg;
+    bf16_t* dh1; long ld;
+};
+constexpr int FDY_MAX_ROWS = 72;
+
+template <int H>
+__global__ __launch_bounds__(H * 16 < 64 ? 64 : H * 16) void fold_dy_kernel(const FoldDyParams p) {
+    constexpr int D = 64 * H, HP = Cols<H>::HP;
+    __shared__ __attribute__((aligned(16))) float cf[FDY_MAX_ROWS][2 * HP];
+    const int tid = threadIdx.x, b = blockIdx.x, L = p.L;
+    const int j0 = blockIdx.y * p.rows_per_wg, j1 = min(L, j0 + p.rows_per_wg);
+    for (int i = tid; i < (j1 - j0) * H; i += blockDim.x) {
+        const int h = i / (j1 - j0), jj = i - h * (j1 - j0);
+        const size_t g = ((size_t)b * H + h) * L + j0 + jj;
+        cf[jj][h] = p.ds[g] * p.scale;
+        cf[jj][HP + h] = p.p[g];
+    }
+    __syncthreads();
+    if (tid >= 16 * H) return;
+    const int c0 = 4 * tid;
+    float qt[H][4], vt[H][4];
+#pragma unroll
+    for (int h = 0; h < H; ++h) {
+        loadvf<4>(p.qt + ((size_t)b * H + h) * D + c0, qt[h]);
+        loadvf<4>(p.vt + ((size_t)b * H + h) * D + c0, vt[h]);
+    }
+    for (int j = j0; j < j1; ++j) {
+        float c[2 * HP];
+#pragma unroll
+        for (int g = 0; g < 2 * HP / 4; ++g) {
+            const f32x4 c4 = *(const f32x4*)&cf[j - j0][4 * g];
+            c[4 * g] = c4[0]; c[4 * g + 1] = c4[1]; c[4 * g + 2] = c4[2]; c[4 * g + 3] = c4[3];
+        }
+        float r[4] = {0.f, 0.f, 0.f, 0.f};
+#pragma unroll
+        for (int h = 0; h < H; ++h) {
+            axpy_n<4>(c[h], qt[h], r);
+            axpy_n<4>(c[HP + h], vt[h], r);
+        }
+        if (j == 0) {
+            for (int h = 0; h < H; ++h) {
+                float q4[4];
+                loadvf<4>(p.qq + ((size_t)b * H + h) * D + c0, q4);
+#pragma unroll
+                for (int e = 0; e < 4; ++e) r[e] += q4[e];
+            }
+        }
+        const f32x4 rv = {r[0], r[1], r[2], r[3]};
+        store4(p.dh1 + ((size_t)b * L + j) * p.ld + c0, rv);
+    }
+}
+
+template <int H> void launch_dot(hipStream_t s, const FoldDotParams& p) {
+    hipLaunchKernelGGL(fold_dot_kernel<H>, dim3(2 * H, (p.B + FDOT_BCHUNK - 1) / FDOT_BCHUNK), dim3(256), 0, s, p);
+}
+template <int H> void launch_headT(hipStream_t s, const FoldHeadTParams& p0, const FoldHeadTParams* p1 = nullptr, const FoldHeadTParams* p2 = nullptr) {
+    FoldHeadTBatch b{};
+    b.p[0] = p0;
+    if (p1) b.p[1] = *p1;
+    if (p2) b.p[2] = *p2;
+    hipLaunchKernelGGL(fold_headT_kernel<H>, dim3(H, (p0.B + FHT_BT - 1) / FHT_BT, p2 ? 3 : (p1 ? 2 : 1)), dim3(H * 16 < 64 ? 64 : H * 16), 0, s, b);
+}
+template <int H, bool BWD> void launch_seq(hipStream_t s, const FoldSeqParams& p) {
+    hipLaunchKernelGGL((fold_seq_kernel<H, BWD>), dim3(p.B), dim3(FSEQ_THREADS), 0, s, p);
+}
+template <int H> void launch_dy(hipStream_t s, const FoldDyParams& p) {
+    hipLaunchKernelGGL(fold_dy_kernel<H>, dim3(p.B, (p.L + p.rows_per_wg - 1) / p.rows_per_wg), dim3(H * 16 < 64 ? 64 : H * 16), 0, s, p);
+}
+#define FOLD_DISPATCH(H, call)          \
+    switch (H) {                        \
+        case 1: call(1); break;         \
+        case 2: call(2); break;         \
+        case 4: call(4); break;         \
+        default: call(12); break;       \
+    }
+
+size_t align16(size_t n) { return (n + 15) & ~(size_t)15; }
+struct FoldWs {
+    size_t vec0, vec1, vec2, vec3, vec4, hs0, hs1, ds, dq, total;
+    FoldWs(int B, int H, int L) {
+        const size_t D = 64 * (size_t)H, bhd = align16((size_t)B * H * D * 4), bh = align16((size_t)B * H * 4);
+        vec0 = 0; vec1 = bhd; vec2 = 2 * bhd; vec3 = 3 * bhd; vec4 = 4 * bhd;
+        hs0 = 5 * bhd; hs1 = hs0 + bh;
+        ds = hs1 + bh;
+        dq = ds + align16((size_t)B * H * L * 4);
+        total = dq + align16((size_t)B * D * 4);
+    }
+};
+
+int fold_check(const uia_cls_fold_desc& d, bool bwd, const char* name) {
+    UIA_CHECK_ARG(d.B > 0 && d.L > 0 && d.L <= FSEQ_MAX_L && (d.H == 1 || d.H == 2 || d.H == 4 || d.H == 12), "%s: B=%d H=%d L=%d outside the supported range (H in {1, 2, 4, 12}, L <= 288)",
+                  name, d.B, d.H, d.L);
+    UIA_CHECK_ARG((int64_t)d.B * d.L <= 0x7FFFFFFF, "%s: %d sequences of %d rows exceed the 31-bit row index", name, d.B, d.L);
+    UIA_CHECK_ARG(d.scale > 0.f && d.scale < 3.0e38f, "%s: scale must be positive and finite, got %g", name, (double)d.scale);
+    UIA_CHECK_ARG(d.A && d.W && d.bias && d.q && d.p && d.ws, "%s: null tensor", name);
+    const int64_t D = 64 * (int64_t)d.H, M = (int64_t)d.B * d.L;
+    UIA_CHECK_ARG(d.a_kb_rows == 0 ? (d.lda >= D && d.lda % 8 == 0) : d.a_kb_rows >= M, "%s: A: row-major rows closer than D or not whole 16-byte units, or a K-blocked operand below B*L rows",
+                  name);
+    UIA_CHECK_ARG(d.ln_sums ? (d.ln_colsum && d.ln_eps > 0.f && d.ln_eps < 1.f) : !d.ln_colsum, "%s: a folded LayerNorm needs ln_sums, ln_colsum and 0 < ln_eps < 1 together", name);
+    UIA_CHECK_ARG(((uintptr_t)d.A | (uintptr_t)d.W | (uintptr_t)d.ws) % 16 == 0 && (uintptr_t)d.ln_sums % 8 == 0 &&
+                  ((uintptr_t)d.bias | (uintptr_t)d.q | (uintptr_t)d.p | (uintptr_t)d.ln_colsum | (uintptr_t)d.keylen) % 4 == 0, "%s: alignment", name);
+    UIA_CHECK_ARG(d.ws_bytes >= FoldWs(d.B, d.H, d.L).total, "%s: workspace of %llu bytes, uia_cls_fold_workspace_bytes says %llu", name, (unsigned long long)d.ws_bytes,
+                  (unsigned long long)FoldWs(d.B, d.H, d.L).total);
+    if (!bwd) {
+        UIA_CHECK_ARG(d.out && d.ldo >= D && d.ldo % 8 == 0 && (uintptr_t)d.out % 16 == 0, "%s: out: null, misaligned or rows closer than D", name);
+    } else {
+        UIA_CHECK_ARG(!d.keylen, "%s: the backward takes unmasked attention only", name);
+        UIA_CHECK_ARG(d.Wu && d.dout && d.dh1, "%s: null tensor", name);
+        UIA_CHECK_ARG(d.lddo >= D && d.lddo % 8 == 0 && d.ld_dh1 >= D && d.ld_dh1 % 8 == 0, "%s: dout / dh1 rows closer than D or not whole 16-byte units", name);
+        UIA_CHECK_ARG(((uintptr_t)d.Wu | (uintptr_t)d.dout | (uintptr_t)d.dh1) % 16 == 0, "%s: alignment", name);
+    }
+    return 0;
+}
+
+}
+
+size_t uia_cls_fold_ws_bytes(int B, int H, int L) {
+    if (B <= 0 || H <= 0 || L <= 0) return 0;
+    return FoldWs(B, H, L).total;
+}
+
+int uia_cls_fold_fwd_launch(hipStream_t stream, const uia_cls_fold_desc& d) {
+    if (fold_check(d, false, "uia_cls_fold_fwd")) return -1;
+    const int B = d.B, H = d.H, L = d.L, D = 64 * H;
+    const FoldWs o(B, H, L);
+    char* ws = (char*)d.ws;
+    float *qt = (float*)(ws + o.vec0), *z = (float*)(ws + o.vec1), *cq = (float*)(ws + o.hs0), *zs = (float*)(ws + o.hs1);
+    const bf16_t* W = (const bf16_t*)d.W;
+    const FoldA A{(const bf16_t*)d.A, (long)d.lda, (long)d.a_kb_rows};
+    FoldDotParams pq{};
+    pq.W = W; pq.A = A; pq.sums = d.ln_sums; pq.eps = d.ln_eps; pq.colsum = d.ln_colsum; pq.bias = d.bias; pq.alpha = 1.f;
+    pq.B = B; pq.L = L; pq.src_a = 1; pq.out32 = d.q; pq.ldo = D;
+    FoldHeadTParams pt{};
+    pt.W = W + (size_t)D * D; pt.u32 = d.q; pt.colsum = d.ln_colsum ? d.ln_colsum + D : nullptr; pt.cout = d.ln_colsum ? cq : nullptr; pt.out = qt; pt.B = B;
+    FoldSeqParams ps{};
+    ps.A = A; ps.sums = d.ln_sums; ps.eps = d.ln_eps; ps.keylen = d.keylen; ps.vec = qt; ps.cvec = d.ln_colsum ? cq : nullptr; ps.scale = d.scale;
+    ps.B = B; ps.L = L; ps.p = d.p; ps.z = z; ps.zs = zs;
+    FoldDotParams po{};
+    po.W = W + 2 * (size_t)D * D; po.v = z; po.ms = d.ln_colsum ? zs : nullptr; po.colsum = d.ln_colsum ? d.ln_colsum + 2 * D : nullptr; po.bias = d.bias + 2 * D; po.alpha = 1.f;
+    po.B = B; po.L = L; po.outT = (bf16_t*)d.out; po.ldo = (long)d.ldo;
+#define FOLD_FWD(HH)                      \
+    launch_dot<HH>(stream, pq);           \
+    launch_headT<HH>(stream, pt);         \
+    launch_seq<HH, false>(stream, ps);    \
+    launch_dot<HH>(stream, po)
+    FOLD_DISPATCH(H, FOLD_FWD)
+#undef FOLD_FWD
+    UIA_CHECK_LAUNCH();
+    return 0;
+}
+
+int uia_cls_fold_bwd_launch(hipStream_t stream, const uia_cls_fold_desc& d) {
+    if (fold_check(d, true, "uia_cls_fold_bwd")) return -1;
+    const int B = d.B, H = d.H, L = d.L, D = 64 * H;
+    const FoldWs o(B, H, L);
+    char* ws = (char*)d.ws;
+    float *vtF = (float*)(ws + o.vec0), *vtU = (float*)(ws + o.vec1), *qtU = (float*)(ws + o.vec2), *g = (float*)(ws + o.vec3), *qq = (float*)(ws + o.vec4);
+    float *cv = (float*)(ws + o.hs0), *gs = (float*)(ws + o.hs1), *ds = (float*)(ws + o.ds), *dq = (float*)(ws + o.dq);
+    const bf16_t *W = (const bf16_t*)d.W, *Wu = (const bf16_t*)d.Wu;
+    const bool same_w = d.W == d.Wu;
+    const FoldA A{(const bf16_t*)d.A, (long)d.lda, (long)d.a_kb_rows};
+    FoldHeadTParams pv{};
+    pv.W = W + 2 * (size_t)D * D; pv.uT = (const bf16_t*)d.dout; pv.ldu = (long)d.lddo; pv.colsum = d.ln_colsum ? d.ln_colsum + 2 * D : nullptr; pv.cout = d.ln_colsum ? cv : nullptr;
+    pv.out = vtF; pv.B = B;
+    FoldHeadTParams pvu = pv;
+    pvu.W = Wu + 2 * (size_t)D * D; pvu.colsum = nullptr; pvu.cout = nullptr; pvu.out = vtU;
+    FoldHeadTParams pqu{};
+    pqu.W = Wu + (size_t)D * D; pqu.u32 = d.q; pqu.out = qtU; pqu.B = B;
+    FoldSeqParams ps{};
+    ps.A = A; ps.sums = d.ln_sums; ps.eps = d.ln_eps; ps.vec = vtF; ps.cvec = d.ln_colsum ? cv : nullptr; ps.scale = d.scale;
+    ps.B = B; ps.L = L; ps.p = d.p; ps.ds = ds; ps.z = g; ps.zs = gs;
+    FoldDotParams pd{};
+    pd.W = W + (size_t)D * D; pd.v = g; pd.ms = d.ln_colsum ? gs : nullptr; pd.colsum = d.ln_colsum ? d.ln_colsum + D : nullptr; pd.alpha = d.scale;
+    pd.B = B; pd.L = L; pd.out32 = dq; pd.ldo = D;
+    FoldHeadTParams pqq{};
+    pqq.W = Wu; pqq.u32 = dq; pqq.out = qq; pqq.B = B;
+    FoldDyParams py{};
+    py.qt = qtU; py.vt = same_w ? vtF : vtU; py.qq = qq; py.ds = ds; py.p = d.p; py.scale = d.scale; py.B = B; py.L = L;
+    py.rows_per_wg = (L + 3) / 4; py.dh1 = (bf16_t*)d.dh1; py.ld = (long)d.ld_dh1;
+#define FOLD_BWD(HH)                          \
+    launch_headT<HH>(stream, pv, &pqu, same_w ? nullptr : &pvu); \
+    launch_seq<HH, true>(stream, ps);         \
+    launch_dot<HH>(stream, pd);               \
+    launch_headT<HH>(stream, pqq);            \
+    launch_dy<HH>(stream, py)
+    FOLD_DISPATCH(H, FOLD_BWD)
+#undef FOLD_BWD
+    UIA_CHECK_LAUNCH();
+    return 0;
+}
diff --git a/nextgen-uia_amd/csrc/uia_kernels.h b/nextgen-uia_amd/csrc/uia_kernels.h
--- a/nextgen-uia_amd/csrc/uia_kernels.h
+++ b/nextgen-uia_amd/csrc/uia_kernels.h
@@ -23,6 +23,9 @@
                                       const float* gamma, float eps, const float* dres_rows, int period, float* dx32, void* dxT, int8_t* dx_lo);
 int uia_attn_bwd_cls_launch(hipStream_t stream, int dtype, const UiaAttnParams& p, bool compact = false);
 int uia_attn_fwd_cls_launch(hipStream_t stream, int dtype, const UiaAttnParams& p);
+size_t uia_cls_fold_ws_bytes(int B, int H, int L);
+int uia_cls_fold_fwd_launch(hipStream_t stream, const uia_cls_fold_desc& d);
+int uia_cls_fold_bwd_launch(hipStream_t stream, const uia_cls_fold_desc& d);
 int uia_mona_cls_fwd_launch(hipStream_t stream, int dtype, int B, int ntok, const void* t, long ldt, void* d, float p_drop, uint64_t seed, const uint8_t* keep_mask);
 int uia_rows3_to_f32_launch(hipStream_t stream, int rows, int D, long stride_rows, const void* hi, long ldhi, long hi_kb_rows, const int8_t* lo, long ldlo, float* dst);
 int uia_mona_cls_bwd_launch(hipStream_t stream, int dtype, int B, int ntok, const void* dd, const void* t, long ldt, void* dt, float p_drop, uint64_t seed,
diff --git a/nextgen-uia_amd/uia_hip/_lib.py b/nextgen-uia_amd/uia_hip/_lib.py
--- a/nextgen-uia_amd/uia_hip/_lib.py
+++ b/nextgen-uia_amd/uia_hip/_lib.py
@@ -39,6 +39,12 @@
                 ("B", i32), ("H", i32), ("L", i32), ("dh", i32), ("mask_kind", i32), ("scale", f32),
                 ("dout", vp), ("lddo", i64), ("dq", vp), ("dk", vp), ("dv", vp), ("ld_dqkv", i64), ("cu_seqlens", vp),
                 ("out_kb_rows", i64), ("dqkv_kb_rows", i64)]
+
+
+class ClsFoldDesc(C.Structure):
+    _fields_ = [("A", vp), ("lda", i64), ("a_kb_rows", i64), ("W", vp), ("Wu", vp), ("bias", vp), ("ln_sums", vp), ("ln_colsum", vp), ("ln_eps", f32),
+                ("scale", f32), ("B", i32), ("H", i32), ("L", i32), ("reserved", i32), ("keylen", vp), ("out", vp), ("ldo", i64), ("q", vp), ("p", vp),
+                ("dout", vp), ("lddo", i64), ("dh1", vp), ("ld_dh1", i64), ("ws", vp), ("ws_bytes", C.c_uint64)]
 
 
 class MonaSpatialDesc(C.Structure):
@@ -199,6 +205,9 @@
     "uia_mona_cls_fwd": (C.c_int, [vp, C.c_int, C.c_int, C.c_int, vp, i64, vp, f32, C.c_uint64, vp]),
     "uia_rows3_to_f32": (C.c_int, [vp, C.c_int, C.c_int, i64, vp, i64, i64, vp, i64, vp]),
     "uia_layernorm_bwd_periodic": (C.c_int, [vp, C.c_int, C.c_int, C.c_int, vp, vp, vp, vp, i64, vp, f32, vp, C.c_int, vp, vp, vp]),
+    "uia_cls_fold_workspace_bytes": (sz, [C.c_int, C.c_int, C.c_int]),
+    "uia_cls_fold_fwd": (C.c_int, [vp, C.POINTER(ClsFoldDesc)]),
+    "uia_cls_fold_bwd": (C.c_int, [vp, C.POINTER(ClsFoldDesc)]),
 }
 
 _lib = None
diff --git a/nextgen-uia_amd/uia_hip/functional.py b/nextgen-uia_amd/uia_hip/functional.py
--- a/nextgen-uia_amd/uia_hip/functional.py
+++ b/nextgen-uia_amd/uia_hip/functional.py
@@ -10,7 +10,7 @@
 from ._lib import UiaError
 from .handoff import (ClsGrad, Resid3, _g3_partner_feeds, cls_grad_of, fwd3_of, grad3_decode, grad3_of, grad_resid3_enabled, hook_free, linear_chain,
                       publish_cls_grad, publish_fwd3, publish_grad3, publish_rows, publish_t_copy, set_cls_grad, set_grad_resid3, t_copy_of, take_rows, zero_sums,
-                      cls_only, set_cls_forward, take_cls_forward)
+                      cls_only, set_cls_forward, take_cls_forward, set_cls_fold)
 from .handoff import clear as clear_t_copies
 
 _STATE = {"dtype": torch.bfloat16, "seed": 0x5EED, "calls": 0, "fwd_resid3": os.environ.get("UIA_FWD_RESID3", "1") != "0"}
@@ -589,6 +589,11 @@
         self.ln1, self.qkv, self.proj, self.ln2, self.fc1, self.fc2 = ln1, qkv, proj, ln2, fc1, fc2
 
 
+def _cls_fold_ok(dt, heads, L, bias, like):
+    return (handoff.cls_fold_enabled() and dt == torch.bfloat16 and heads in ops.CLS_FOLD_HEADS and 1 < L <= ops.CLS_FOLD_MAX_L and bias is not None
+            and like.is_cuda)
+
+
 ATTN_SINGLE_PASS_MAX = 272
 
 
@@ -614,20 +619,28 @@
             rows = (x3.hi, x3.sums)
         else:
             rows = take_rows(x, dt) if fold else None
-        qkv = _empty((M, 3 * D), dt, like)
+        cls_last = handoff.take_last_block_cls() and spec.mask is None and 1 < N <= ATTN_SINGLE_PASS_MAX and D == 64 * spec.heads and like.is_cuda
+        cfold = None
+        qkv = None if cls_last and _cls_fold_ok(dt, spec.heads, N, spec.qkv[1], like) else _empty((M, 3 * D), dt, like)
         if rows is not None:
             wq, cq, bq = WEIGHTS.get_lnfold(spec.qkv[0], spec.qkv[1], spec.ln1[0], spec.ln1[1], dt)
             xin_t, sums0 = rows
             if not ops.is_kb(xin_t):
                 xin_t = xin_t.view(M, D)
-            ops.gemm(xin_t, wq, bias=bq, out_t=qkv, lnfold=(sums0, cq, D, spec.eps))
-            h1 = _act(M, D, dt, like, spec.fc1[0].shape[0]) if x3 is not None else xin_t
+            if qkv is None:
+                cfold, h1 = (xin_t, wq, bq, (sums0, cq, D, spec.eps)), None
+            else:
+                ops.gemm(xin_t, wq, bias=bq, out_t=qkv, lnfold=(sums0, cq, D, spec.eps))
+                h1 = _act(M, D, dt, like, spec.fc1[0].shape[0]) if x3 is not None else xin_t
         else:
             h1 = _empty((M, D), dt, x)
             ops.layernorm_fwd(x2d, spec.ln1[0], spec.ln1[1], spec.eps, y_t=h1)
-            ops.gemm(h1, WEIGHTS.get(spec.qkv[0], dt), bias=spec.qkv[1], out_t=qkv)
-        if handoff.take_last_block_cls() and spec.mask is None and 1 < N <= ATTN_SINGLE_PASS_MAX and D == 64 * spec.heads and like.is_cuda:
-            return VitBlockFn._forward_cls(ctx, x, x3, qkv, spec, (B, N, D), dt, train)
+            if qkv is None:
+                cfold = (h1, WEIGHTS.get(spec.qkv[0], dt), spec.qkv[1], None)
+            else:
+                ops.gemm(h1, WEIGHTS.get(spec.qkv[0], dt), bias=spec.qkv[1], out_t=qkv)
+        if cls_last:
+            return VitBlockFn._forward_cls(ctx, x, x3, qkv, spec, (B, N, D), dt, train, like, cfold)
         if N > ATTN_SINGLE_PASS_MAX:
             a = _empty((M, D), dt, like)
             ops.attn_fwd_long(qkv[:, :D], qkv[:, D:2 * D], qkv[:, 2 * D:], a, B, spec.heads, N)
@@ -673,12 +686,18 @@
         return x2
 
     @staticmethod
-    def _forward_cls(ctx, x, x3, qkv, spec, shape, dt, train):
+    def _forward_cls(ctx, x, x3, qkv, spec, shape, dt, train, like, cfold=None):
         B, N, D = shape
-        like = qkv
         a = _empty((B, D), dt, like)
-        lse = torch.empty(B, spec.heads, device=like.device, dtype=torch.float32) if train else None
-        ops.attn_fwd_cls(qkv[:, :D], qkv[:, D:2 * D], qkv[:, 2 * D:], a, B, spec.heads, N, lse=lse)
+        if cfold is not None:
+            aop, wf, bf, lnf = cfold
+            q = torch.empty(B, D, device=like.device, dtype=torch.float32)
+            p = torch.empty(B, spec.heads, N, device=like.device, dtype=torch.float32)
+            ops.cls_fold_fwd(aop, wf, bf, B, spec.heads, N, a, q, p, ops.cls_fold_workspace(B, spec.heads, N, like.device), lnfold=lnf)
+            lse = None
+        else:
+            lse = torch.empty(B, spec.heads, device=like.device, dtype=torch.float32) if train else None
+            ops.attn_fwd_cls(qkv[:, :D], qkv[:, D:2 * D], qkv[:, 2 * D:], a, B, spec.heads, N, lse=lse)
         x_cls = torch.empty(B, D, device=like.device, dtype=torch.float32)
         if x3 is not None:
             ops.rows3_to_f32(x3.hi, x3.lo, N, x_cls)
@@ -698,8 +717,14 @@
         x2 = torch.empty(B, 1, D, device=like.device, dtype=torch.float32)
         ops.gemm(f, w2, bias=spec.fc2[1], resid=x1, out32=x2.view(B, D), tile_cfg=_rows_tile_cfg(M, w2, like, dt, out32=True, resid=True))
         if train:
-            saved, ctx.layout = handoff.save_layout(x3.resid3 if x3 is not None else x, qkv, a, lse, x1, pre)
+            if cfold is not None:
+                saved, ctx.layout = handoff.save_layout(x3.resid3 if x3 is not None else x, aop, a, q, x1, pre)
+                saved = [p, lnf[0] if lnf is not None else p] + saved
+            else:
+                saved, ctx.layout = handoff.save_layout(x3.resid3 if x3 is not None else x, qkv, a, lse, x1, pre)
             ctx.save_for_backward(*saved)
+            ctx.cls_fold = cfold is not None
+            ctx.cls_fold_ln = cfold is not None and lnf is not None
             ctx.xshape = (B, N, D)
             ctx.spec = spec
             ctx.g3_out = dt == torch.bfloat16 and _g3_partner_feeds(x)
@@ -711,7 +736,8 @@
     @staticmethod
     def backward_cls(ctx, cg):
         compact = getattr(ctx, "cls_fwd", False)
-        xin, qkv, a, lse, x1, pre = handoff.restore_layout(ctx.saved_tensors, ctx.layout)
+        cfold = getattr(ctx, "cls_fold", False)
+        xin, qkv, a, lse, x1, pre = handoff.restore_layout(ctx.saved_tensors[2:] if cfold else ctx.saved_tensors, ctx.layout)
         x3_in = isinstance(xin, Resid3)
         x = xin.lo if x3_in else xin
         spec = ctx.spec
@@ -731,13 +757,22 @@
         ops.layernorm_bwd(dh, x1_cls, spec.ln2[0], spec.eps, dres=dy, dx32=dx1, dx_t=dx1_t if dt != torch.float32 else None)
         da = dh
         ops.gemm(dx1_t, WEIGHTS.get(spec.proj[0], dt, transpose=True), out_t=da)
-        dqkv = _attn_act(M, 3 * D, dt, x, D)
-        if ops.is_kb(dqkv):
-            ops.attn_bwd_cls(qkv[:, :D], qkv[:, D:2 * D], qkv[:, 2 * D:], a, da, lse, dqkv, None, None, B, spec.heads, N, rows=compact)
-        else:
-            ops.attn_bwd_cls(qkv[:, :D], qkv[:, D:2 * D], qkv[:, 2 * D:], a, da, lse, dqkv[:, :D], dqkv[:, D:2 * D], dqkv[:, 2 * D:], B, spec.heads, N, rows=compact)
         dh1 = _empty((M, D), dt, x)
-        ops.gemm(dqkv, WEIGHTS.get(spec.qkv[0], dt, transpose=True), out_t=dh1)
+        if cfold:
+            p_att, sums0 = ctx.saved_tensors[:2]
+            wu = WEIGHTS.get(spec.qkv[0], dt)
+            if ctx.cls_fold_ln:
+                wq, cq, bq = WEIGHTS.get_lnfold(spec.qkv[0], spec.qkv[1], spec.ln1[0], spec.ln1[1], dt)
+                ops.cls_fold_bwd(qkv, wq, wu, bq, B, spec.heads, N, lse, p_att, da, dh1, ops.cls_fold_workspace(B, spec.heads, N, x.device), lnfold=(sums0, cq, D, spec.eps))
+            else:
+                ops.cls_fold_bwd(qkv, wu, wu, spec.qkv[1], B, spec.heads, N, lse, p_att, da, dh1, ops.cls_fold_workspace(B, spec.heads, N, x.device))
+        else:
+            dqkv = _attn_act(M, 3 * D, dt, x, D)
+            if ops.is_kb(dqkv):
+                ops.attn_bwd_cls(qkv[:, :D], qkv[:, D:2 * D], qkv[:, 2 * D:], a, da, lse, dqkv, None, None, B, spec.heads, N, rows=compact)
+            else:
+                ops.attn_bwd_cls(qkv[:, :D], qkv[:, D:2 * D], qkv[:, 2 * D:], a, da, lse, dqkv[:, :D], dqkv[:, D:2 * D], dqkv[:, 2 * D:], B, spec.heads, N, rows=compact)
+            ops.gemm(dqkv, WEIGHTS.get(spec.qkv[0], dt, transpose=True), out_t=dh1)
         xrows = xin if x3_in else x.view(M, D)
         if getattr(ctx, "g3_out", False):
             dx_t = _empty((M, D), dt, x)
@@ -869,9 +904,17 @@
     return cu_seqlens is None and D == 64 * heads and 1 < L <= 288 and x_t.is_cuda and not (x_t.dtype != torch.float32 and _STATE.get("text_resid_t", False))
 
 
-def _post_ln_layer_cls(res, qkv, L, B, heads, P, keylen, eps, D, dt):
-    a = _empty((B, D), dt, qkv)
-    ops.attn_fwd_cls(qkv[:, :D], qkv[:, D:2 * D], qkv[:, 2 * D:], a, B, heads, L, mask="keypad", keylen=keylen)
+def _post_ln_layer_cls(res, qkv, L, B, heads, P, keylen, eps, D, dt, cfold=None):
+    if cfold is not None:
+        aop, wf, bf, lnf = cfold
+        qkv = aop.t if ops.is_kb(aop) else aop
+        a = _empty((B, D), dt, qkv)
+        q = torch.empty(B, D, device=qkv.device, dtype=torch.float32)
+        p = torch.empty(B, heads, L, device=qkv.device, dtype=torch.float32)
+        ops.cls_fold_fwd(aop, wf, bf, B, heads, L, a, q, p, ops.cls_fold_workspace(B, heads, L, qkv.device), keylen=keylen, lnfold=lnf)
+    else:
+        a = _empty((B, D), dt, qkv)
+        ops.attn_fwd_cls(qkv[:, :D], qkv[:, D:2 * D], qkv[:, 2 * D:], a, B, heads, L, mask="keypad", keylen=keylen)
     r = _res_cls_rows(res, L, B, D, eps)
     s_a = torch.empty(B, D, device=qkv.device, dtype=torch.float32)
     M = B * L
@@ -894,6 +937,13 @@
     dt = x_t.dtype
     t_resid = dt != torch.float32 and _STATE.get("text_resid_t", False)
     fold = fold_sums is not None and ln_fold_enabled(dt, M) and not t_resid
+    if cls_only and _cls_fold_ok(dt, heads, L, P["_qkv_b"], x_t):
+        if res.dim is not None:
+            wq, cq, bq = WEIGHTS.get_lnfold(P["_qkv_raw"][0], P["_qkv_raw"][1], res.w, res.b, dt)
+            cfold = (x_t, wq, bq, (res.stats, cq, D, res.eps))
+        else:
+            cfold = (x_t, P["_qkv_w"](dt), P["_qkv_b"], None)
+        return _post_ln_layer_cls(res, None, L, B, heads, P, keylen, eps, D, dt, cfold)
     qkv = _empty((M, 3 * D), dt, x_t)
     if res.dim is not None:
         wq, cq, bq = WEIGHTS.get_lnfold(P["_qkv_raw"][0], P["_qkv_raw"][1], res.w, res.b, dt)
diff --git a/nextgen-uia_amd/uia_hip/handoff.py b/nextgen-uia_amd/uia_hip/handoff.py
--- a/nextgen-uia_amd/uia_hip/handoff.py
+++ b/nextgen-uia_amd/uia_hip/handoff.py
@@ -5,7 +5,7 @@
 from . import ops
 
 _STATE = {"chain_depth": 0, "fwd3_next_plain": False, "grad_resid3": False, "cls_grad": True,
-          "cls_forward": True, "cls_decl": False, "cls_last": False, "cls_rows": False}
+          "cls_forward": True, "cls_fold": True, "cls_decl": False, "cls_last": False, "cls_rows": False}
 
 
 class Resid3(NamedTuple):
@@ -204,6 +204,14 @@
 
 def set_cls_forward(flag):
     _STATE["cls_forward"] = bool(flag)
+
+
+def set_cls_fold(flag):
+    _STATE["cls_fold"] = bool(flag)
+
+
+def cls_fold_enabled():
+    return _STATE["cls_fold"]
 
 
 def hook_free(*modules):
diff --git a/nextgen-uia_amd/uia_hip/ops.py b/nextgen-uia_amd/uia_hip/ops.py
--- a/nextgen-uia_amd/uia_hip/ops.py
+++ b/nextgen-uia_amd/uia_hip/ops.py
@@ -872,6 +872,64 @@
     check(lib().uia_attn_fwd_cls(_stream(), _code(q.dtype), C.byref(d)), "uia_attn_fwd_cls")
 
 
+CLS_FOLD_HEADS = (1, 2, 4, 12)
+CLS_FOLD_MAX_L = 288
+
+
+def cls_fold_workspace(B, H, L, device):
+    return torch.empty(lib().uia_cls_fold_workspace_bytes(B, H, L), device=device, dtype=torch.uint8)
+
+
+def _cls_fold_desc(name, a, w, bias, B, H, L, q, p, ws, lnfold, scale):
+    D = 64 * H
+    d = _lib.ClsFoldDesc()
+    if is_kb(a):
+        rows, cols, plane = _kb_dims(a, f"{name}: A")
+        _require(a.dtype == torch.bfloat16 and rows >= B * L and cols == D, f"{name}: K-blocked A {tuple(a.t.shape)} does not hold bf16 [{B * L}, {D}]")
+        d.A, d.lda, d.a_kb_rows = _p(a.t), 0, plane
+    else:
+        _require(isinstance(a, torch.Tensor) and a.dtype == torch.bfloat16 and a.dim() == 2 and a.shape[0] >= B * L and a.shape[1] == D and a.stride(1) == 1,
+                 f"{name}: A must be bf16 [{B * L}, {D}] rows (row-major or KBlocked), got {tuple(getattr(a, 'shape', ()))} {getattr(a, 'dtype', type(a).__name__)}")
+        d.A, d.lda, d.a_kb_rows = _p(a), a.stride(0), 0
+    wrow = w.row if isinstance(w, PackedW) else w
+    _dense(wrow, f"{name}: W", (torch.bfloat16,), 3 * D * D, align=16)
+    _dense(bias, f"{name}: bias", _F32, 3 * D, align=4)
+    _dense(q, f"{name}: q", _F32, B * D, align=16)
+    _dense(p, f"{name}: p", _F32, B * H * L, align=4)
+    _dense(ws, f"{name}: ws", (torch.uint8,), align=16)
+    d.W, d.bias, d.q, d.p, d.ws, d.ws_bytes = _p(wrow), _p(bias), _p(q), _p(p), _p(ws), ws.numel()
+    if lnfold is not None:
+        sums, colsum, dim, eps = lnfold
+        _require(dim == D and sums.numel() >= 2 * B * L and sums.is_contiguous(), f"{name}: lnfold sums must hold (Σ, Σ²) of {B * L} rows of {D}")
+        _dense(colsum, f"{name}: lnfold colsum", _F32, 3 * D, align=4)
+        d.ln_sums, d.ln_colsum, d.ln_eps = _p(sums), _p(colsum), float(eps)
+    d.B, d.H, d.L, d.scale = B, H, L, float(scale) if scale is not None else 0.125
+    return d
+
+
+def cls_fold_fwd(a, w, bias, B, H, L, out, q, p, ws, keylen=None, lnfold=None, scale=None):
+    d = _cls_fold_desc("cls_fold_fwd", a, w, bias, B, H, L, q, p, ws, lnfold, scale)
+    _require(not is_kb(out) and out.dim() == 2 and tuple(out.shape) == (B, 64 * H) and out.stride(1) == 1 and out.dtype == torch.bfloat16,
+             f"cls_fold_fwd: out must be bf16 [{B}, {64 * H}] rows (one per sequence)")
+    if keylen is not None:
+        _dense(keylen, "cls_fold_fwd: keylen", (torch.int32,), B, align=4)
+        d.keylen = _p(keylen)
+    d.out, d.ldo = _p(out), out.stride(0)
+    check(lib().uia_cls_fold_fwd(_stream(), C.byref(d)), "uia_cls_fold_fwd")
+
+
+def cls_fold_bwd(a, w, wu, bias, B, H, L, q, p, dout, dh1, ws, lnfold=None, scale=None):
+    d = _cls_fold_desc("cls_fold_bwd", a, w, bias, B, H, L, q, p, ws, lnfold, scale)
+    D = 64 * H
+    wurow = wu.row if isinstance(wu, PackedW) else wu
+    _dense(wurow, "cls_fold_bwd: Wu", (torch.bfloat16,), 3 * D * D, align=16)
+    _require(dout.dim() == 2 and tuple(dout.shape) == (B, D) and dout.stride(1) == 1 and dout.dtype == torch.bfloat16, f"cls_fold_bwd: dout must be bf16 [{B}, {D}] rows")
+    _require(not is_kb(dh1) and dh1.dim() == 2 and tuple(dh1.shape) == (B * L, D) and dh1.stride(1) == 1 and dh1.dtype == torch.bfloat16,
+             f"cls_fold_bwd: dh1 must be bf16 [{B * L}, {D}] row-major rows")
+    d.Wu, d.dout, d.lddo, d.dh1, d.ld_dh1 = _p(wurow), _p(dout), dout.stride(0), _p(dh1), dh1.stride(0)
+    check(lib().uia_cls_fold_bwd(_stream(), C.byref(d)), "uia_cls_fold_bwd")
+
+
 def rows3_to_f32(hi, lo, stride_rows, dst):
     rows, D = dst.shape
     if dst.dtype != torch.float32 or not dst.is_contiguous() or lo.dtype != torch.int8 or lo.dim() != 2 or lo.stride(1) != 1 or lo.shape[1] != D:
```

Result: no change. 6747 (median of 6 runs) (+0.8%).
